# peabody124/PosePipeline

Measured on AMD Instinct MI355X. Metric: frames/sec (whole node), detect->2D->3D cascade on 1080p; MPJPE vs reference, higher is better.
Workload: dtype f32; eligible float32 convolutions are evaluated as 2-term float16 splits (22 significand bits under per-channel / per-sample power-of-two scales, 3 products per term) on the 16-bit matrix cores with float32 accumulation (float32-accurate at any input magnitude, not bit-identical: tests/test_gpu_spl

## Files before the change

posepipeline_amd/csrc/api_core.hip:

```cpp
#include <dlfcn.h>

#include <algorithm>
#include <memory>

#include "pp_internal.h"
#include "pp_amax.h"

#include <atomic>
extern std::atomic<int> g_decode_generic, g_split_gemm_epi;

static thread_local std::string g_last_error;

void pp_set_error(const char* fmt, ...) {
    char buf[1024];
    va_list ap;
    va_start(ap, fmt);
    vsnprintf(buf, sizeof(buf), fmt, ap);
    va_end(ap);
    g_last_error = buf;
}

namespace {
struct Roctx {
    int (*push)(const char*) = nullptr;
// ... 83 lines not shown
    PP_HIP_CHECK(hipStreamCreateWithFlags(&c->copy_stream, hipStreamNonBlocking));
    PP_HIP_CHECK(hipEventCreateWithFlags(&c->ev_upload, hipEventDisableTiming));
    PP_HIP_CHECK(hipEventCreateWithFlags(&c->ev_consumed, hipEventDisableTiming));
    *out = c.release();
    return PP_OK;
}

void pp_ctx_destroy(pp_ctx* ctx) {
    if (!ctx) return;
    (void)hipSetDevice(ctx->device);
    if (ctx->stream) (void)hipStreamSynchronize(ctx->stream);
    if (ctx->scratch) (void)hipFree(ctx->scratch);
    if (ctx->ev_start) (void)hipEventDestroy(ctx->ev_start);
    if (ctx->ev_stop) (void)hipEventDestroy(ctx->ev_stop);
    if (ctx->copy_stream) {
        (void)hipStreamSynchronize(ctx->copy_stream);
        (void)hipStreamDestroy(ctx->copy_stream);
    }
    if (ctx->ev_upload) (void)hipEventDestroy(ctx->ev_upload);
    if (ctx->ev_consumed) (void)hipEventDestroy(ctx->ev_consumed);
    if (ctx->own_stream && ctx->stream) (void)hipStreamDestroy(ctx->stream);
    delete ctx;
}

int pp_ctx_set_stream(pp_ctx* ctx, void* hip_stream) {
    PP_REQUIRE(ctx, "pp_ctx_set_stream: ctx is NULL");
    PP_HIP_CHECK(hipStreamSynchronize(ctx->stream));
    if (ctx->own_stream && ctx->stream) PP_HIP_CHECK(hipStreamDestroy(ctx->stream));
    ctx->stream = static_cast<hipStream_t>(hip_stream);
    ctx->own_stream = false;
    return PP_OK;
}

int pp_ctx_synchronize(pp_ctx* ctx) {
    PP_REQUIRE(ctx, "pp_ctx_synchronize: ctx is NULL");
    PP_HIP_CHECK(hipStreamSynchronize(ctx->stream));
    return PP_OK;
}

int pp_timer_start(pp_ctx* ctx) {
    PP_REQUIRE(ctx, "pp_timer_start: ctx is NULL");
    PP_HIP_CHECK(hipEventRecord(ctx->ev_start, ctx->stream));
    return PP_OK;
}

int pp_timer_stop(pp_ctx* ctx, float* elapsed_ms) {
    PP_REQUIRE(ctx && elapsed_ms, "pp_timer_stop: NULL argument");
    PP_HIP_CHECK(hipEventRecord(ctx->ev_stop, ctx->stream));
    PP_HIP_CHECK(hipEventSynchronize(ctx->ev_stop));
    PP_HIP_CHECK(hipEventElapsedTime(elapsed_ms, ctx->ev_start, ctx->ev_stop));
    return PP_OK;
}

int pp_malloc(pp_ctx* ctx, size_t bytes, void** dptr) {
    PP_REQUIRE(ctx && dptr, "pp_malloc: NULL argument");
    PP_HIP_CHECK(hipSetDevice(ctx->device));
    PP_HIP_CHECK(hipMalloc(dptr, bytes ? bytes : 1));
    return PP_OK;
}

int pp_free(pp_ctx* ctx, void* dptr) {
    PP_REQUIRE(ctx, "pp_free: ctx is NULL");
    if (!dptr) return PP_OK;
    PP_HIP_CHECK(hipStreamSynchronize(ctx->stream));
    PP_HIP_CHECK(hipFree(dptr));
    return PP_OK;
}

int pp_memcpy_h2d(pp_ctx* ctx, void* dst, const void* src, size_t bytes) {
    PP_REQUIRE(ctx && (bytes == 0 || (dst && src)), "pp_memcpy_h2d: NULL argument");
    PP_HIP_CHECK(hipMemcpyAsync(dst, src, bytes, hipMemcpyHostToDevice, ctx->stream));
    PP_HIP_CHECK(hipStreamSynchronize(ctx->stream));
    return PP_OK;
}

int pp_host_alloc(pp_ctx* ctx, size_t bytes, void** out) {
    PP_REQUIRE(ctx && out, "pp_host_alloc: NULL argument");
    *out = nullptr;
    PP_HIP_CHECK(hipSetDevice(ctx->device));
    PP_HIP_CHECK(hipHostMalloc(out, bytes ? bytes : 1, hipHostMallocDefault));
    return PP_OK;
}

int pp_host_free(pp_ctx* ctx, void* p) {
    PP_REQUIRE(ctx != nullptr, "pp_host_free: ctx is NULL");
    if (p) PP_HIP_CHECK(hipHostFree(p));
    return PP_OK;
}

int pp_upload_begin(pp_ctx* ctx, void* dst, const void* src, size_t bytes) {
    PP_REQUIRE(ctx && (bytes == 0 || (dst && src)), "pp_upload_begin: NULL argument");
    PP_HIP_CHECK(hipStreamWaitEvent(ctx->copy_stream, ctx->ev_consumed, 0));
    PP_HIP_CHECK(hipMemcpyAsync(dst, src, bytes, hipMemcpyHostToDevice, ctx->copy_stream));
    PP_HIP_CHECK(hipEventRecord(ctx->ev_upload, ctx->copy_stream));
    return PP_OK;
}

int pp_upload_begin_nv12(pp_ctx* ctx, void* dst_bgr, void* tmp_nv12, const void* src_host, int frames, int height, int width) {
    PP_REQUIRE(ctx && (frames == 0 || (dst_bgr && tmp_nv12 && src_host)), "pp_upload_begin_nv12: NULL argument");
    PP_REQUIRE(frames >= 0 && height > 0 && width > 0, "pp_upload_begin_nv12: bad shape");
    PP_HIP_CHECK(hipStreamWaitEvent(ctx->copy_stream, ctx->ev_consumed, 0));
    const size_t bytes = (size_t)frames * height * width * 3 / 2;
    if (bytes) PP_HIP_CHECK(hipMemcpyAsync(tmp_nv12, src_host, bytes, hipMemcpyHostToDevice, ctx->copy_stream));
    const int r = pp_launch_nv12_to_bgr((const unsigned char*)tmp_nv12, (unsigned char*)dst_bgr, frames, height, width, ctx->copy_stream);
    if (r != PP_OK) return r;
    PP_HIP_CHECK(hipEventRecord(ctx->ev_upload, ctx->copy_stream));
    return PP_OK;
}

int pp_nv12_to_bgr(pp_ctx* ctx, const uint8_t* nv12, int frames, int height, int width, uint8_t* bgr) {
    PP_REQUIRE(ctx && (frames == 0 || (nv12 && bgr)), "pp_nv12_to_bgr: NULL argument");
    return pp_launch_nv12_to_bgr(nv12, bgr, frames, height, width, ctx->stream);
}

int pp_upload_wait(pp_ctx* ctx, int host_sync) {
    PP_REQUIRE(ctx != nullptr, "pp_upload_wait: ctx is NULL");
    PP_HIP_CHECK(hipStreamWaitEvent(ctx->stream, ctx->ev_upload, 0));
    if (host_sync) PP_HIP_CHECK(hipEventSynchronize(ctx->ev_upload));
    return PP_OK;
}

int pp_upload_release(pp_ctx* ctx) {
    PP_REQUIRE(ctx != nullptr, "pp_upload_release: ctx is NULL");
    PP_HIP_CHECK(hipEventRecord(ctx->ev_consumed, ctx->stream));
    return PP_OK;
}

int pp_memcpy_d2h(pp_ctx* ctx, void* dst, const void* src, size_t bytes) {
    PP_REQUIRE(ctx && (bytes == 0 || (dst && src)), "pp_memcpy_d2h: NULL argument");
    PP_HIP_CHECK(hipMemcpyAsync(dst, src, bytes, hipMemcpyDeviceToHost, ctx->stream));
    PP_HIP_CHECK(hipStreamSynchronize(ctx->stream));
    return PP_OK;
}

int pp_memcpy_d2d(pp_ctx* ctx, void* dst, const void* src, size_t bytes) {
    PP_REQUIRE(ctx && (bytes == 0 || (dst && src)), "pp_memcpy_d2d: NULL argument");
    PP_HIP_CHECK(hipMemcpyAsync(dst, src, bytes, hipMemcpyDeviceToDevice, ctx->stream));
    return PP_OK;
}

}


struct pp_net {
    pp_ctx* ctx = nullptr;
    std::vector<pp_op> ops;
    std::vector<pp_buf> bufs;
    std::vector<size_t> buf_off;
    std::vector<size_t> buf_elems;
    float* weights = nullptr;
    size_t n_weights = 0;
    unsigned char* wsplit = nullptr;
    std::vector<SplitPlan> split_plan;
    int numerics = PP_NET_NUMERICS_EXACT;
    int split_f16 = 0;
    unsigned* amax = nullptr;
    std::vector<int> op_x_slot, op_y_slot, op_post_slot, slot_owner;
    std::vector<int> slot_first, slot_last;
    struct ExtAmax { int buf, slot, first_reader, last_reader; bool provided; };
    std::vector<ExtAmax> ext;
    float* arena = nullptr;
    size_t arena_floats = 0;
    int max_batch = 0;
    hipGraphExec_t graph_exec = nullptr;
    int graph_batch = 0;
    bool use_lanes = true;
    std::vector<hipStream_t> lanes;
    std::vector<int> op_lane;
    std::vector<std::vector<int>> op_waits;
    std::vector<char> op_needs_event;
    std::vector<hipEvent_t> op_done;
    hipEvent_t fork_ev = nullptr;
    std::vector<hipEvent_t> join_ev;
    std::vector<pp_vit_encoder*> vits;
    std::vector<pp_deconv_bf16*> deconvs;

    float* buf_ptr(int b) const { return arena + buf_off[b]; }
    unsigned* amax_slot(int slot) const { return slot >= 0 ? amax + (size_t)slot * max_batch : nullptr; }
};

static ConvArgs net_conv_args(pp_net* net, const pp_op& op, int batch);
static int net_make_lanes(pp_net* net, int n_lanes);

static void net_plan_amax(pp_net* net) {
    const int n = (int)net->ops.size(), nb = (int)net->bufs.size();
    net->op_x_slot.assign(n, -1);
    net->op_y_slot.assign(n, -1);
    net->op_post_slot.assign(n, -1);
    net->slot_owner.clear();
    net->ext.clear();
    if (net->numerics != PP_NET_NUMERICS_SPLIT || !net->split_f16) return;
    auto is_h = [&](int i) { return net->ops[i].type == PP_OP_CONV && net->split_plan[i].kernel != SPLIT_NONE; };
    auto tracks = [&](int i) {
        const pp_op& op = net->ops[i];
        if (op.type == PP_OP_UPSAMPLE_ADD) return true;
        return op.type == PP_OP_CONV && pp_conv_tracks_amax(net_conv_args(net, op, 1), is_h(i));
    };
    {
        std::vector<char> written(nb, 0);
        for (int i = 0; i < n; ++i) {
            const pp_op& op = net->ops[i];
            if (is_h(i) && !written[op.in]) {
                pp_net::ExtAmax* e = nullptr;
                for (auto& x : net->ext)
                    if (x.buf == op.in) e = &x;
                if (!e) {
                    net->ext.push_back({op.in, (int)net->slot_owner.size(), i, i, false});
                    net->slot_owner.push_back(-1);
                    e = &net->ext.back();
                }
                e->last_reader = i;
                net->op_x_slot[i] = e->slot;
            }
            written[op.out] = 1;
        }
    }
    struct Tensor { int slot; std::vector<int> producers; bool wanted; };
    std::vector<Tensor> tensors;
    std::vector<int> cur(nb, -1);
    std::vector<char> read_since(nb, 1);
    std::vector<std::pair<int, int>> readers;
    for (int i = 0; i < n; ++i) {
        const pp_op& op = net->ops[i];
        if (is_h(i) && cur[op.in] >= 0) {
            tensors[cur[op.in]].wanted = true;
            readers.push_back({i, cur[op.in]});
        }
        for (int b : {op.in, op.res1, op.res2, op.in2, op.in3})
            if (b >= 0) read_since[b] = 1;
        if (cur[op.out] < 0 || read_since[op.out]) {
            cur[op.out] = (int)tensors.size();
            tensors.push_back({(int)net->slot_owner.size(), {}, false});
            net->slot_owner.push_back(i);
        }
        tensors[cur[op.out]].producers.push_back(i);
        read_since[op.out] = 0;
    }
    net->slot_first.assign(net->slot_owner.size(), -1);
    net->slot_last.assign(net->slot_owner.size(), -1);
    for (const Tensor& t : tensors) {
        if (!t.wanted) continue;
        net->slot_first[t.slot] = t.producers.front();
        net->slot_last[t.slot] = t.producers.back();
        bool fused = true;
        for (int p : t.producers) fused = fused && tracks(p);
        {
            int covered = 0;
            const int out_b = net->ops[t.producers.front()].out;
            for (int p : t.producers) covered += net->ops[p].type == PP_OP_CONV ? net->ops[p].cout : net->bufs[out_b].c;
            if (covered < net->bufs[out_b].c) fused = false;
        }
        if (fused)
            for (int p : t.producers) net->op_y_slot[p] = t.slot;
        else
            net->op_post_slot[t.producers.back()] = t.slot;
    }
    for (const auto& r : readers) net->op_x_slot[r.first] = tensors[r.second].slot;
}

static int net_reset_amax(pp_net* net, int first, int last, int batch, hipStream_t s) {
    if (!net->amax) return PP_OK;
    int s0 = -1, s1 = -1;
    for (int k = 0; k < (int)net->slot_first.size(); ++k) {
        const int a = net->slot_first[k], b = net->slot_last[k];
        if (a < 0 || b < first || a >= last) continue;
        PP_REQUIRE(a >= first && b < last, "pp_net_run: op range [%d, %d) splits the producers (ops %d .. %d) of a tensor whose per-sample maxima are tracked",
                   first, last, a, b);
    }
    for (int k = 0; k < (int)net->slot_owner.size(); ++k)
        if (net->slot_owner[k] >= first && net->slot_owner[k] < last) {
            if (s0 < 0) s0 = k;
            s1 = k + 1;
        }
    if (s0 >= 0) PP_HIP_CHECK(hipMemsetAsync(net->amax_slot(s0), 0, (size_t)(s1 - s0) * net->max_batch * sizeof(unsigned), s));
    for (auto& e : net->ext) {
        if (e.last_reader < first || e.first_reader >= last) continue;
        if (e.provided) {
            e.provided = false;
            continue;
        }
        PP_HIP_CHECK(hipMemsetAsync(net->amax_slot(e.slot), 0, (size_t)batch * sizeof(unsigned), s));
        int rc = pp_launch_amax(net->buf_ptr(e.buf), batch, net->buf_elems[e.buf], net->amax_slot(e.slot), s);
        if (rc != PP_OK) return rc;
    }
    return PP_OK;
}

static void net_plan_lanes(pp_net* net, int n_lanes) {
    const int n = (int)net->ops.size(), nb = (int)net->bufs.size();
    net->op_lane.assign(n, 0);
    net->op_waits.assign(n, {});
    net->op_needs_event.assign(n, 0);
    std::vector<int> last_writer(nb, -1);
    std::vector<std::vector<int>> readers(nb);
    std::vector<int> lane_tail(n_lanes, -1);
    for (int i = 0; i < n; ++i) {
        const pp_op& op = net->ops[i];
        std::vector<int> deps;
        auto add = [&](int d) {
            if (d >= 0 && std::find(deps.begin(), deps.end(), d) == deps.end()) deps.push_back(d);
        };
        for (int b : {op.in, op.res1, op.res2, op.in2, op.in3})
            if (b >= 0) add(last_writer[b]);
        add(last_writer[op.out]);
        for (int r : readers[op.out]) add(r);
        int lane = -1, best = -1;
        for (int l = 0; l < n_lanes; ++l)
            if (lane_tail[l] >= 0 && lane_tail[l] > best && std::find(deps.begin(), deps.end(), lane_tail[l]) != deps.end()) {
                best = lane_tail[l];
                lane = l;
            }
        if (lane < 0) {
            lane = 0;
            for (int l = 1; l < n_lanes; ++l)
                if (lane_tail[l] < lane_tail[lane]) lane = l;
        }
        net->op_lane[i] = lane;
        for (int d : deps)
            if (net->op_lane[d] != lane) {
                net->op_waits[i].push_back(d);
                net->op_needs_event[d] = 1;
            }
        lane_tail[lane] = i;
        for (int b : {op.in, op.res1, op.res2, op.in2, op.in3})
            if (b >= 0 && b != op.out) readers[b].push_back(i);
        last_writer[op.out] = i;
        readers[op.out].clear();
    }
}

static int net_check_op(const pp_net& net, const pp_op& op, int idx) {
    const int nb = (int)net.bufs.size();
    PP_REQUIRE(op.in >= 0 && op.in < nb && op.out >= 0 && op.out < nb, "op %d: buffer id out of range", idx);
    PP_REQUIRE(op.res1 < nb && op.res2 < nb, "op %d: residual buffer id out of range", idx);
    PP_REQUIRE(op.in2 < nb && op.in3 < nb && (op.type == PP_OP_UPSAMPLE_ADD || (op.in2 < 0 && op.in3 < 0)),
               "op %d: in2 / in3 are inputs of PP_OP_UPSAMPLE_ADD only (-1 elsewhere)", idx);
    const pp_buf& bi = net.bufs[op.in];
    const pp_buf& bo = net.bufs[op.out];
    const int eh = op.pad_end & 1, ew = (op.pad_end >> 1) & 1;
    PP_REQUIRE(op.out_c_off >= 0 && op.in_c_off >= 0 && (op.out_c_off & 3) == 0 && (op.in_c_off & 3) == 0,
               "op %d: channel offsets must be non-negative multiples of 4", idx);
    if (op.type != PP_OP_CONV) {
        for (int b : {op.in, op.out, op.res1, op.res2, op.in2, op.in3})
            PP_REQUIRE(b < 0 || net.bufs[b].pad == 0, "op %d: only convolutions may touch a buffer with a zero halo (buffer %d)", idx, b);
    } else {
        PP_REQUIRE(bo.pad == 0 || (!op.out_nchw && op.out_c_off == 0 && bo.c == op.cout && (op.cout & 3) == 0),
                   "op %d: a halo output buffer must be a plain NHWC tensor of the op's own channels", idx);
    }
    if (op.type == PP_OP_CONV) {
        PP_REQUIRE(bi.c == op.cin && op.in_c_off == 0, "op %d: in buffer has %d channels, op.cin=%d", idx, bi.c, op.cin);
        PP_REQUIRE(op.out_c_off + op.cout <= bo.c && (op.out_c_off == 0 ? true : !op.out_nchw),
                   "op %d: channels [%d, %d) do not fit the out buffer (%d channels)", idx, op.out_c_off,
                   op.out_c_off + op.cout, bo.c);
        PP_REQUIRE(bo.c == op.cout || ((bo.c & 3) == 0 && !op.out_nchw), "op %d: a sliced out buffer needs c %% 4 == 0", idx);
        PP_REQUIRE(op.relu >= PP_RELU_NONE && op.relu <= PP_ACT_SWISH, "op %d: unknown activation %d", idx, op.relu);
        const int ho = pp_conv_out_dim(bi.h + eh, op.kh, op.stride, op.pad_h, op.dil_h) - ((op.pad_end >> 2) & 1);
        const int wo = pp_conv_out_dim(bi.w + ew, op.kw, op.stride, op.pad_w, op.dil_w) - ((op.pad_end >> 3) & 1);
        PP_REQUIRE((ho << op.up_log2) == bo.h && (wo << op.up_log2) == bo.w,
                   "op %d: conv output %dx%d (<<%d) does not match out buffer %dx%d", idx, ho, wo, op.up_log2,
                   bo.h, bo.w);
        const size_t kpad = ((size_t)op.kh * op.kw * op.cin + 31) / 32 * 32;
        const size_t cpad = ((size_t)op.cout + 15) / 16 * 16;
        PP_REQUIRE(op.w_off >= 0 && (size_t)op.w_off + kpad * cpad <= net.n_weights, "op %d: weights out of blob", idx);
        PP_REQUIRE(op.b_off >= 0 && (size_t)op.b_off + cpad <= net.n_weights, "op %d: bias out of blob", idx);
        PP_REQUIRE((op.w_off % 4) == 0 && (op.b_off % 4) == 0, "op %d: blob offsets must be 16-byte aligned", idx);
        if (op.res1 >= 0) PP_REQUIRE(net.bufs[op.res1].c == op.cout, "op %d: res1 channel mismatch", idx);
        if (op.res2 >= 0)
            PP_REQUIRE(net.bufs[op.res2].c == op.cout && net.bufs[op.res2].h == bo.h && net.bufs[op.res2].w == bo.w,
                       "op %d: res2 shape mismatch", idx);
    } else if (op.type == PP_OP_MAXPOOL) {
        PP_REQUIRE(op.cin == op.cout && (op.cin & 3) == 0 && op.in_c_off + op.cin <= bi.c && op.out_c_off + op.cout <= bo.c &&
                       (bi.c & 3) == 0 && (bo.c & 3) == 0,
                   "op %d: maxpool channel slices do not fit", idx);
        PP_REQUIRE(pp_conv_out_dim(bi.h + eh, op.kh, op.stride, op.pad_h, 1) == bo.h &&
                       pp_conv_out_dim(bi.w + ew, op.kw, op.stride, op.pad_w, 1) == bo.w,
                   "op %d: maxpool output dims mismatch", idx);
    } else if (op.type == PP_OP_AVGPOOL) {
        PP_REQUIRE(op.cin == op.cout && (op.cin & 3) == 0 && bi.c == op.cin && bo.c == op.cin && op.in != op.out && op.kh > 0 &&
                       op.kw > 0 && op.stride > 0 && bi.h >= op.kh && bi.w >= op.kw && (bi.h - op.kh) / op.stride + 1 == bo.h &&
                       (bi.w - op.kw) / op.stride + 1 == bo.w,
                   "op %d: avgpool needs in [h][w][c] and out [(h - kh) / s + 1][(w - kw) / s + 1][c], c %% 4 == 0", idx);
    } else if (op.type == PP_OP_COPY) {
        PP_REQUIRE(bi.c == bo.c && bi.h == bo.h && bi.w == bo.w, "op %d: copy shape mismatch", idx);
    } else if (op.type == PP_OP_DEPTH_TO_SPACE) {
        PP_REQUIRE(op.cout > 0 && (op.cout & 3) == 0 && bi.c == 4 * op.cout && bo.c == op.cout && bo.h == 2 * bi.h && bo.w == 2 * bi.w,
                   "op %d: depth_to_space needs in [h][w][4*cout] and out [2h][2w][cout]", idx);
    } else if (op.type == PP_OP_DECONV_BF16) {
        PP_REQUIRE(bi.c == op.cin && bo.c == op.cout && bo.h == 2 * bi.h && bo.w == 2 * bi.w && op.in != op.out,
                   "op %d: deconv_bf16 needs in [h][w][cin] and out [2h][2w][cout]", idx);
        PP_REQUIRE(op.cin % 64 == 0 && (op.cout & 7) == 0, "op %d: deconv_bf16 needs cin %% 64 == 0 and cout %% 8 == 0", idx);
        PP_REQUIRE(op.relu == PP_RELU_NONE || op.relu == PP_RELU_LAST, "op %d: deconv_bf16 supports PP_RELU_NONE / PP_RELU_LAST", idx);
        PP_REQUIRE(op.w_off >= 0 && (op.w_off % 4) == 0 && (size_t)op.w_off + (size_t)16 * op.cout * op.cin <= net.n_weights &&
                       op.b_off >= 0 && (op.b_off % 4) == 0 && (size_t)op.b_off + op.cout <= net.n_weights,
                   "op %d: deconv_bf16 parameters out of blob", idx);
    } else if (op.type == PP_OP_UPSAMPLE_ADD) {
        PP_REQUIRE(op.cin == op.cout && (op.cout & 3) == 0 && bi.c == op.cout && bo.c == op.cout && op.up_log2 >= 0 &&
                       (bi.h << op.up_log2) == bo.h && (bi.w << op.up_log2) == bo.w && op.in != op.out,
                   "op %d: upsample_add needs in [h][w][c] and out [h << up][w << up][c]", idx);
        PP_REQUIRE(op.relu == PP_RELU_NONE || op.relu == PP_RELU_LAST, "op %d: upsample_add supports PP_RELU_NONE / PP_RELU_LAST", idx);
        for (int r : {op.res1, op.res2})
            if (r >= 0)
                PP_REQUIRE(net.bufs[r].c == bo.c && net.bufs[r].h == bo.h && net.bufs[r].w == bo.w, "op %d: residual shape mismatch", idx);
        PP_REQUIRE(op.in3 < 0 || op.in2 >= 0, "op %d: in3 without in2", idx);
        for (int k = 0; k < 2; ++k) {
            const int b = k ? op.in3 : op.in2, u = k ? op.up3_log2 : op.up2_log2;
            if (b >= 0)
                PP_REQUIRE(u >= 0 && u <= 5 && net.bufs[b].c == bo.c && (net.bufs[b].h << u) == bo.h && (net.bufs[b].w << u) == bo.w &&
                               b != op.out, "op %d: in%d must be [h >> up][w >> up][c] of the out buffer", idx, k + 2);
        }
    } else if (op.type == PP_OP_VIT_ENCODER) {
        PP_REQUIRE(op.cin == op.cout && bi.c == op.cin && bo.c == op.cin && bi.h == bo.h && bi.w == bo.w && op.in != op.out,
                   "op %d: vit encoder needs distinct in / out buffers of [h][w][dim]", idx);
        PP_REQUIRE(op.kh > 0 && op.kw > 0 && op.stride > 0, "op %d: vit encoder needs depth (kh), heads (kw), mlp ratio (stride)", idx);
        PP_REQUIRE(op.w_off >= 0 && (op.w_off % 4) == 0 &&
                       (size_t)op.w_off + pp_vit_param_floats(bi.h * bi.w, op.cin, op.kh, op.cin * op.stride) <= net.n_weights,
                   "op %d: vit encoder parameters out of blob", idx);
    } else {
        pp_set_error("op %d: unsupported op type %d", idx, op.type);
        return PP_ERR_UNSUPPORTED;
    }
    return PP_OK;
}

static ConvArgs net_conv_args(pp_net* net, const pp_op& op, int batch) {
    const pp_buf& bi = net->bufs[op.in];
    const pp_buf& bo = net->bufs[op.out];
    ConvArgs a{};
    a.x = net->buf_ptr(op.in);
    a.y = net->buf_ptr(op.out);
    a.w = net->weights + op.w_off;
    a.bias = net->weights + op.b_off;
    a.res1 = op.res1 >= 0 ? net->buf_ptr(op.res1) : nullptr;
    a.res2 = op.res2 >= 0 ? net->buf_ptr(op.res2) : nullptr;
    a.N = batch; a.Hin = bi.h; a.Win = bi.w; a.Cin = op.cin;
    a.Hout = bo.h >> op.up_log2; a.Wout = bo.w >> op.up_log2;
    a.Cout = op.cout; a.CoutPad = (op.cout + 15) / 16 * 16;
    a.KH = op.kh; a.KW = op.kw; a.stride = op.stride; a.pad_h = op.pad_h; a.pad_w = op.pad_w;
    a.dil_h = op.dil_h; a.dil_w = op.dil_w;
    a.K = op.kh * op.kw * op.cin; a.Kpad = (a.K + 31) / 32 * 32;
    a.HWout = a.Hout * a.Wout; a.M = batch * a.HWout;
    a.relu = op.relu; a.up_log2 = op.up_log2; a.out_nchw = op.out_nchw;
    a.res1_shift = op.res1_shift; a.res1_off_w = op.res1_off_w;
    a.res1_H = op.res1 >= 0 ? net->bufs[op.res1].h : 0;
    a.res1_W = op.res1 >= 0 ? net->bufs[op.res1].w : 0;
    a.y_stride = bo.c; a.y_coff = op.out_c_off;
    a.x_pad = bi.pad; a.y_pad = bo.pad;
    a.r1_pad = op.res1 >= 0 ? net->bufs[op.res1].pad : 0;
    a.r2_pad = op.res2 >= 0 ? net->bufs[op.res2].pad : 0;
    const size_t idx = &op - net->ops.data();
    a.wsplit = (net->wsplit && idx < net->split_plan.size() && net->split_plan[idx].off >= 0) ? net->wsplit + net->split_plan[idx].off : nullptr;
    a.numerics = net->numerics;
    a.split_f16 = net->split_f16;
    if (idx < net->op_x_slot.size()) {
        a.x_amax = net->amax_slot(net->op_x_slot[idx]);
        a.y_amax = net->amax_slot(net->op_y_slot[idx]);
    }
    return a;
}

static int net_launch_op_body(pp_net* net, const pp_op& op, int batch, hipStream_t s);

static int net_launch_op(pp_net* net, const pp_op& op, int batch, hipStream_t s) {
    const size_t idx = &op - net->ops.data();
    int rc = net_launch_op_body(net, op, batch, s);
    if (rc == PP_OK && net->amax && net->op_post_slot[idx] >= 0)
        rc = pp_launch_amax(net->buf_ptr(op.out), batch, net->buf_elems[op.out], net->amax_slot(net->op_post_slot[idx]), s);
    return rc;
}

static int net_launch_op_body(pp_net* net, const pp_op& op, int batch, hipStream_t s) {
    const pp_buf& bi = net->bufs[op.in];
    const pp_buf& bo = net->bufs[op.out];
    if (op.type == PP_OP_CONV) {
        const ConvArgs a = net_conv_args(net, op, batch);
        return pp_launch_conv(a, &net->split_plan[&op - net->ops.data()], s);
    } else if (op.type == PP_OP_MAXPOOL) {
        PoolArgs p{};
        p.x = net->buf_ptr(op.in); p.y = net->buf_ptr(op.out);
        p.N = batch; p.Hin = bi.h; p.Win = bi.w; p.C = op.cin; p.Hout = bo.h; p.Wout = bo.w;
        p.x_stride = bi.c; p.x_coff = op.in_c_off; p.y_stride = bo.c; p.y_coff = op.out_c_off;
        p.KH = op.kh; p.KW = op.kw; p.stride = op.stride; p.pad_h = op.pad_h; p.pad_w = op.pad_w;
        return pp_launch_maxpool(p, s);
    } else if (op.type == PP_OP_AVGPOOL) {
        return pp_launch_avgpool(net->buf_ptr(op.in), net->buf_ptr(op.out), batch, bi.h, bi.w, op.cin, op.kh, op.kw, op.stride, s);
    } else if (op.type == PP_OP_COPY) {
        PP_HIP_CHECK(hipMemcpyAsync(net->buf_ptr(op.out), net->buf_ptr(op.in),
                                    (size_t)batch * net->buf_elems[op.in] * sizeof(float),
                                    hipMemcpyDeviceToDevice, s));
        return PP_OK;
    } else if (op.type == PP_OP_DEPTH_TO_SPACE) {
        return pp_launch_depth_to_space(net->buf_ptr(op.in), net->buf_ptr(op.out), batch, bi.h, bi.w, op.cout, s);
    } else if (op.type == PP_OP_DECONV_BF16) {
        return pp_deconv_bf16_run(net->deconvs[&op - net->ops.data()], net->buf_ptr(op.in), net->buf_ptr(op.out), batch,
                                  op.relu == PP_RELU_LAST, s);
    } else if (op.type == PP_OP_UPSAMPLE_ADD) {
        return pp_launch_upsample_add(net->buf_ptr(op.in), op.res1 >= 0 ? net->buf_ptr(op.res1) : nullptr,
                                      op.res2 >= 0 ? net->buf_ptr(op.res2) : nullptr, net->buf_ptr(op.out), batch, bo.h, bo.w,
                                      bo.c, op.up_log2, op.relu == PP_RELU_LAST, s, op.in2 >= 0 ? net->buf_ptr(op.in2) : nullptr,
                                      op.up2_log2, op.in3 >= 0 ? net->buf_ptr(op.in3) : nullptr, op.up3_log2,
                                      net->amax && net->op_y_slot[&op - net->ops.data()] >= 0 ? net->amax_slot(net->op_y_slot[&op - net->ops.data()]) : nullptr);
    } else if (op.type == PP_OP_VIT_ENCODER) {
        pp_vit_encoder* enc = net->vits[&op - net->ops.data()];
        return pp_vit_encoder_run(enc, net->buf_ptr(op.in), net->buf_ptr(op.out), batch, s);
    }
    return PP_ERR_UNSUPPORTED;
}

int pp_net_dims(pp_net* net, int buf, int* h, int* w, int* c) {
    if (!net || buf < 0 || buf >= (int)net->bufs.size()) return PP_ERR_ARG;
    *h = net->bufs[buf].h; *w = net->bufs[buf].w; *c = net->bufs[buf].c;
    return PP_OK;
}
int pp_net_max_batch(pp_net* net) { return net ? net->max_batch : 0; }
pp_ctx* pp_net_ctx(pp_net* net) { return net ? net->ctx : nullptr; }

void pp_net_void_input_amax(pp_net* net, int buf) {
    if (!net) return;
    for (auto& e : net->ext)
        if (e.buf == buf) e.provided = false;
}

unsigned* pp_net_input_amax_slot(pp_net* net, int buf) {
    if (!net || !net->amax) return nullptr;
    for (auto& e : net->ext)
        if (e.buf == buf) return net->amax_slot(e.slot);
    return nullptr;
}

extern "C" {

int pp_net_create(pp_ctx* ctx, const pp_op* ops, int n_ops, const pp_buf* bufs, int n_bufs,
                  const float* weights, size_t n_weights, int max_batch, pp_net** out) {
    return pp_net_create_mem(ctx, ops, n_ops, bufs, n_bufs, weights, n_weights, PP_MEM_HOST, max_batch, out);
}

int pp_net_create_mem(pp_ctx* ctx, const pp_op* ops, int n_ops, const pp_buf* bufs, int n_bufs,
                      const float* weights, size_t n_weights, int weights_mem, int max_batch, pp_net** out) {
    return pp_net_create_ex(ctx, ops, n_ops, bufs, n_bufs, weights, n_weights, weights_mem, max_batch, PP_NET_NUMERICS_DEFAULT, out);
}

int pp_net_numerics(pp_net* net) { return net ? net->numerics : PP_ERR_ARG; }
int pp_net_split_kind(pp_net* net) {
    if (!net) return PP_ERR_ARG;
    return net->numerics != PP_NET_NUMERICS_SPLIT ? PP_NET_NUMERICS_EXACT : net->split_f16 ? PP_NET_NUMERICS_SPLIT_F16 : PP_NET_NUMERICS_SPLIT_BF16;
}

int pp_net_create_ex(pp_ctx* ctx, const pp_op* ops, int n_ops, const pp_buf* bufs, int n_bufs,
                     const float* weights, size_t n_weights, int weights_mem, int max_batch, int numerics, pp_net** out) {
    PP_REQUIRE(ctx && ops && bufs && weights && out, "pp_net_create: NULL argument");
    PP_REQUIRE(numerics >= PP_NET_NUMERICS_DEFAULT && numerics <= PP_NET_NUMERICS_SPLIT_F16, "pp_net_create_ex: bad numerics %d", numerics);
    PP_REQUIRE(weights_mem == PP_MEM_HOST || weights_mem == PP_MEM_DEVICE, "pp_net_create: bad weights_mem %d", weights_mem);
    PP_REQUIRE(n_ops > 0 && n_bufs > 0 && max_batch > 0, "pp_net_create: empty program");
    *out = nullptr;
    std::unique_ptr<pp_net> net(new pp_net());
    net->ctx = ctx;
    net->ops.assign(ops, ops + n_ops);
    net->bufs.assign(bufs, bufs + n_bufs);
    net->max_batch = max_batch;
    net->n_weights = n_weights;
    net->numerics = numerics != PP_NET_NUMERICS_DEFAULT ? numerics : (pp_conv_split_enabled() ? PP_NET_NUMERICS_SPLIT : PP_NET_NUMERICS_EXACT);
    if (net->numerics >= PP_NET_NUMERICS_SPLIT) {
        net->split_f16 = net->numerics == PP_NET_NUMERICS_SPLIT ? pp_conv_split_f16_default() : net->numerics == PP_NET_NUMERICS_SPLIT_F16;
        net->numerics = PP_NET_NUMERICS_SPLIT;
    }
    size_t off = 0;
    for (int b = 0; b < n_bufs; ++b) {
        PP_REQUIRE(bufs[b].h > 0 && bufs[b].w > 0 && bufs[b].c > 0 && bufs[b].pad >= 0 && bufs[b].pad <= 8, "buffer %d has an empty dim / bad halo", b);
        const size_t e = (size_t)(bufs[b].h + bufs[b].pad) * (bufs[b].w + bufs[b].pad) * bufs[b].c;
        net->buf_elems.push_back(e);
        net->buf_off.push_back(off);
        off += (e * max_batch + 63) / 64 * 64;
    }
    net->arena_floats = off;
    for (int i = 0; i < n_ops; ++i) {
        int rc = net_check_op(*net, net->ops[i], i);
        if (rc != PP_OK) return rc;
    }
    PP_HIP_CHECK(hipSetDevice(ctx->device));
    PP_HIP_CHECK(hipMalloc((void**)&net->weights, n_weights * sizeof(float)));
    PP_HIP_CHECK(hipMemcpyAsync(net->weights, weights, n_weights * sizeof(float),
                                weights_mem == PP_MEM_HOST ? hipMemcpyHostToDevice : hipMemcpyDeviceToDevice, ctx->stream));
    PP_HIP_CHECK(hipMalloc((void**)&net->arena, net->arena_floats * sizeof(float)));
    PP_HIP_CHECK(hipMemsetAsync(net->arena, 0, net->arena_floats * sizeof(float), ctx->stream));
    net->vits.assign(n_ops, nullptr);
    net->deconvs.assign(n_ops, nullptr);
    for (int i = 0; i < n_ops; ++i) {
        const pp_op& op = net->ops[i];
        if (op.type == PP_OP_DECONV_BF16) {
            const pp_buf& bi = net->bufs[op.in];
            int rc = pp_deconv_bf16_create(net->weights + op.w_off, net->weights + op.b_off, bi.h, bi.w, op.cin, op.cout,
                                           max_batch, ctx->stream, &net->deconvs[i]);
            if (rc != PP_OK) {
                pp_net_destroy(net.release());
                return rc;
            }
        }
        if (op.type != PP_OP_VIT_ENCODER) continue;
        const pp_buf& bi = net->bufs[op.in];
        int rc = pp_vit_encoder_create(net->weights + op.w_off, bi.h * bi.w, op.cin, op.kh, op.kw, op.cin * op.stride,
                                       max_batch, ctx->stream, &net->vits[i]);
        if (rc != PP_OK) {
            pp_net_destroy(net.release());
            return rc;
        }
    }
    net->split_plan.assign(n_ops, SplitPlan());
    if (net->numerics == PP_NET_NUMERICS_SPLIT) {
        size_t bytes = 0;
        for (int i = 0; i < n_ops; ++i) {
            if (net->ops[i].type != PP_OP_CONV) continue;
            SplitPlan p = pp_conv_split_plan(net_conv_args(net.get(), net->ops[i], 1));
            if (p.kernel == SPLIT_NONE) continue;
            p.off = (long long)bytes;
            bytes += (p.bytes + 255) / 256 * 256;
            net->split_plan[i] = p;
        }
        net_plan_amax(net.get());
        if (!net->slot_owner.empty()) {
            const size_t ab = net->slot_owner.size() * (size_t)max_batch * sizeof(unsigned);
            PP_HIP_CHECK(hipMalloc((void**)&net->amax, ab));
            PP_HIP_CHECK(hipMemsetAsync(net->amax, 0, ab, ctx->stream));
        }
        if (bytes) {
            PP_HIP_CHECK(hipMalloc((void**)&net->wsplit, bytes));
            for (int i = 0; i < n_ops; ++i) {
                const SplitPlan& p = net->split_plan[i];
                if (p.kernel == SPLIT_NONE) continue;
                int rc = pp_conv_split_weights(p, net_conv_args(net.get(), net->ops[i], 1), net->wsplit + p.off, ctx->stream);
                if (rc != PP_OK) return rc;
            }
        }
    }
    PP_HIP_CHECK(hipStreamSynchronize(ctx->stream));
    for (int i = 0; i < n_ops; ++i)
        if (net->ops[i].type == PP_OP_CONV) {
            int rc = pp_conv_prepare(net_conv_args(net.get(), net->ops[i], 1));
            if (rc != PP_OK) return rc;
        }
    const char* env_lanes = getenv("POSEPIPE_NET_LANES");
    const int n_lanes = env_lanes ? atoi(env_lanes) : 4;
    int rc_l = net_make_lanes(net.get(), n_lanes);
    if (rc_l != PP_OK) return rc_l;
    *out = net.release();
    return PP_OK;
}

static int net_make_lanes(pp_net* net, int n_lanes) {
    for (auto l : net->lanes) (void)hipStreamDestroy(l);
    net->lanes.clear();
    for (auto e : net->op_done)
        if (e) (void)hipEventDestroy(e);
    net->op_done.clear();
    for (auto e : net->join_ev)
        if (e) (void)hipEventDestroy(e);
    net->join_ev.clear();
    if (net->fork_ev) (void)hipEventDestroy(net->fork_ev);
    net->fork_ev = nullptr;
    const int n_ops = (int)net->ops.size();
    if (n_lanes > 1 && n_ops >= 8) {
        net_plan_lanes(net, n_lanes);
        net->lanes.resize(n_lanes);
        for (auto& l : net->lanes) PP_HIP_CHECK(hipStreamCreateWithFlags(&l, hipStreamNonBlocking));
        net->op_done.assign(n_ops, nullptr);
        for (int i = 0; i < n_ops; ++i)
            if (net->op_needs_event[i]) PP_HIP_CHECK(hipEventCreateWithFlags(&net->op_done[i], hipEventDisableTiming));
        PP_HIP_CHECK(hipEventCreateWithFlags(&net->fork_ev, hipEventDisableTiming));
        net->join_ev.resize(n_lanes);
        for (auto& e : net->join_ev) PP_HIP_CHECK(hipEventCreateWithFlags(&e, hipEventDisableTiming));
    }
    return PP_OK;
}

int pp_net_input_amax(pp_net* net, int buf, void** dptr) {
    PP_REQUIRE(net && dptr && buf >= 0 && buf < (int)net->bufs.size(), "pp_net_input_amax: bad argument");
    *dptr = nullptr;
    for (auto& e : net->ext)
        if (e.buf == buf && net->amax) {
            e.provided = true;
            *dptr = net->amax_slot(e.slot);
        }
    return PP_OK;
}

int pp_net_conv_kinds(pp_net* net, int* kinds) {
    PP_REQUIRE(net && kinds, "pp_net_conv_kinds: NULL argument");
    for (size_t i = 0; i < net->ops.size(); ++i) {
        if (net->ops[i].type != PP_OP_CONV) {
            kinds[i] = 0;
            continue;
        }
        kinds[i] = net->split_plan[i].kernel != SPLIT_NONE ? 2 : 1;
    }
    return PP_OK;
}

void pp_net_destroy(pp_net* net) {
    if (!net) return;
    if (net->ctx && net->ctx->stream) (void)hipStreamSynchronize(net->ctx->stream);
    for (auto l : net->lanes) {
        (void)hipStreamSynchronize(l);
        (void)hipStreamDestroy(l);
    }
    for (auto e : net->op_done)
        if (e) (void)hipEventDestroy(e);
    for (auto e : net->join_ev)
        if (e) (void)hipEventDestroy(e);
    if (net->fork_ev) (void)hipEventDestroy(net->fork_ev);
    if (net->graph_exec) (void)hipGraphExecDestroy(net->graph_exec);
    for (auto* v : net->vits) pp_vit_encoder_destroy(v);
    for (auto* d : net->deconvs) pp_deconv_bf16_destroy(d);
    if (net->weights) (void)hipFree(net->weights);
    if (net->wsplit) (void)hipFree(net->wsplit);
    if (net->amax) (void)hipFree(net->amax);
    if (net->arena) (void)hipFree(net->arena);
    delete net;
}

int pp_net_buffer(pp_net* net, int buf, void** dptr, size_t* bytes_per_sample) {
    PP_REQUIRE(net && buf >= 0 && buf < (int)net->bufs.size(), "pp_net_buffer: bad buffer id");
    PP_REQUIRE(net->bufs[buf].pad == 0, "pp_net_buffer: buffer %d has a zero halo (conv-internal layout); expose dense buffers only", buf);
    if (dptr) *dptr = net->buf_ptr(buf);
    if (bytes_per_sample) *bytes_per_sample = net->buf_elems[buf] * sizeof(float);
    return PP_OK;
}

int pp_net_run(pp_net* net, int batch, int first_op, int last_op) {
    PP_REQUIRE(net, "pp_net_run: net is NULL");
    PP_REQUIRE(batch > 0 && batch <= net->max_batch, "pp_net_run: batch %d not in (0,%d]", batch, net->max_batch);
    if (last_op < 0) last_op = (int)net->ops.size();
    PP_REQUIRE(first_op >= 0 && last_op <= (int)net->ops.size() && first_op <= last_op, "pp_net_run: bad op range");
    if (net->graph_exec && batch == net->graph_batch && first_op == 0 && last_op == (int)net->ops.size()) {
        PP_HIP_CHECK(hipGraphLaunch(net->graph_exec, net->ctx->stream));
        return PP_OK;
    }
    hipStream_t main = net->ctx->stream;
    PpRange range("pp_net_run");
    {
        int rc = net_reset_amax(net, first_op, last_op, batch, main);
        if (rc != PP_OK) return rc;
    }
    if (net->lanes.empty() || !net->use_lanes || last_op - first_op < 8) {
        for (int i = first_op; i < last_op; ++i) {
            int rc = net_launch_op(net, net->ops[i], batch, main);
            if (rc != PP_OK) return rc;
        }
        return PP_OK;
    }
    PP_HIP_CHECK(hipEventRecord(net->fork_ev, main));
    for (hipStream_t l : net->lanes) PP_HIP_CHECK(hipStreamWaitEvent(l, net->fork_ev, 0));
    for (int i = first_op; i < last_op; ++i) {
        hipStream_t s = net->lanes[net->op_lane[i]];
        for (int d : net->op_waits[i])
            if (d >= first_op) PP_HIP_CHECK(hipStreamWaitEvent(s, net->op_done[d], 0));
        int rc = net_launch_op(net, net->ops[i], batch, s);
        if (rc != PP_OK) return rc;
        if (net->op_needs_event[i]) PP_HIP_CHECK(hipEventRecord(net->op_done[i], s));
    }
    for (size_t l = 0; l < net->lanes.size(); ++l) {
        PP_HIP_CHECK(hipEventRecord(net->join_ev[l], net->lanes[l]));
        PP_HIP_CHECK(hipStreamWaitEvent(main, net->join_ev[l], 0));
    }
    return PP_OK;
}

int pp_net_vit_timing(pp_net* net, int enable, float* ms3, int* n_gemm) {
    PP_REQUIRE(net, "pp_net_vit_timing: net is NULL");
    for (auto* v : net->vits) {
        if (!v) continue;
        if (ms3) {
            PP_HIP_CHECK(hipStreamSynchronize(net->ctx->stream));
            int rc = pp_vit_encoder_get_timing(v, ms3, n_gemm);
            if (rc != PP_OK) return rc;
        }
        pp_vit_encoder_set_timing(v, enable);
        return PP_OK;
    }
    pp_set_error("pp_net_vit_timing: the program has no PP_OP_VIT_ENCODER");
    return PP_ERR_STATE;
}

int pp_net_set_lane_count(pp_net* net, int n_lanes) {
    PP_REQUIRE(net && n_lanes >= 1 && n_lanes <= 16, "pp_net_set_lane_count: net is NULL or n_lanes not in [1, 16]");
    PP_HIP_CHECK(hipStreamSynchronize(net->ctx->stream));
    for (auto l : net->lanes) PP_HIP_CHECK(hipStreamSynchronize(l));
    if (net->graph_exec) {
        PP_HIP_CHECK(hipGraphExecDestroy(net->graph_exec));
        net->graph_exec = nullptr;
    }
    return net_make_lanes(net, n_lanes);
}

int pp_net_set_lanes(pp_net* net, int enable) {
    PP_REQUIRE(net, "pp_net_set_lanes: net is NULL");
    PP_HIP_CHECK(hipStreamSynchronize(net->ctx->stream));
    net->use_lanes = enable != 0;
    return PP_OK;
}

int pp_net_capture(pp_net* net, int batch) {
    PP_REQUIRE(net, "pp_net_capture: net is NULL");
    PP_REQUIRE(batch > 0 && batch <= net->max_batch, "pp_net_capture: bad batch");
    if (net->graph_exec) {
        PP_HIP_CHECK(hipGraphExecDestroy(net->graph_exec));
        net->graph_exec = nullptr;
    }
    hipStream_t s = net->ctx->stream;
    PP_HIP_CHECK(hipStreamSynchronize(s));
    hipGraph_t graph = nullptr;
    PP_HIP_CHECK(hipStreamBeginCapture(s, hipStreamCaptureModeThreadLocal));
    int rc = net_reset_amax(net, 0, (int)net->ops.size(), batch, s);
    for (size_t i = 0; i < net->ops.size() && rc == PP_OK; ++i) rc = net_launch_op(net, net->ops[i], batch, s);
    hipError_t e = hipStreamEndCapture(s, &graph);
    if (rc != PP_OK) {
        if (graph) (void)hipGraphDestroy(graph);
        return rc;
    }
    PP_HIP_CHECK(e);
    PP_HIP_CHECK(hipGraphInstantiate(&net->graph_exec, graph, nullptr, nullptr, 0));
    PP_HIP_CHECK(hipGraphDestroy(graph));
    net->graph_batch = batch;
    return PP_OK;
}

int pp_net_forward(pp_net* net, int batch, int in_buf, const float* in, int out_buf, float* out, int mem) {
    PP_REQUIRE(net && in && out, "pp_net_forward: NULL argument");
    PP_REQUIRE(in_buf >= 0 && in_buf < (int)net->bufs.size() && out_buf >= 0 && out_buf < (int)net->bufs.size(),
               "pp_net_forward: bad buffer id");
    PP_REQUIRE(batch > 0 && batch <= net->max_batch, "pp_net_forward: batch %d not in (0,%d]", batch, net->max_batch);
    PP_REQUIRE(net->bufs[in_buf].pad == 0 && net->bufs[out_buf].pad == 0, "pp_net_forward: input / output buffers must be dense (pad 0)");
    hipStream_t s = net->ctx->stream;
    const hipMemcpyKind kin = mem == PP_MEM_HOST ? hipMemcpyHostToDevice : hipMemcpyDeviceToDevice;
    const hipMemcpyKind kout = mem == PP_MEM_HOST ? hipMemcpyDeviceToHost : hipMemcpyDeviceToDevice;
    PP_HIP_CHECK(hipMemcpyAsync(net->buf_ptr(in_buf), in, (size_t)batch * net->buf_elems[in_buf] * sizeof(float), kin, s));
    pp_net_void_input_amax(net, in_buf);
    int rc = pp_net_run(net, batch, 0, (int)net->ops.size());
    if (rc != PP_OK) return rc;
    PP_HIP_CHECK(hipMemcpyAsync(out, net->buf_ptr(out_buf), (size_t)batch * net->buf_elems[out_buf] * sizeof(float), kout, s));
    PP_HIP_CHECK(hipStreamSynchronize(s));
    return PP_OK;
}

int pp_net_profile(pp_net* net, int batch, float* ms_per_op) {
    PP_REQUIRE(net, "pp_net_profile: net is NULL");
    PP_REQUIRE(batch > 0 && batch <= net->max_batch, "pp_net_profile: bad batch");
    hipStream_t s = net->ctx->stream;
    const size_t n = net->ops.size();
    std::vector<hipEvent_t> ev(n + 1);
    for (auto& e : ev) PP_HIP_CHECK(hipEventCreate(&e));
    int rc = net_reset_amax(net, 0, (int)n, batch, s);
    PP_HIP_CHECK(hipEventRecord(ev[0], s));
    for (size_t i = 0; i < n && rc == PP_OK; ++i) {
        rc = net_launch_op(net, net->ops[i], batch, s);
        if (rc == PP_OK && hipEventRecord(ev[i + 1], s) != hipSuccess) rc = PP_ERR_HIP;
    }
    if (rc == PP_OK && hipStreamSynchronize(s) != hipSuccess) rc = PP_ERR_HIP;
    if (rc == PP_OK && ms_per_op) {
        for (size_t i = 0; i < n; ++i) {
            float ms = 0.f;
            (void)hipEventElapsedTime(&ms, ev[i], ev[i + 1]);
            ms_per_op[i] = ms;
        }
    }
    for (auto& e : ev) (void)hipEventDestroy(e);
    return rc;
}

int pp_conv2d(pp_ctx* ctx, const pp_op* op, int n, int hin, int win, const float* x, const float* w,
              const float* bias, const float* res1, const float* res2, float* y, int res1_h, int res1_w,
              int mem) {
    PP_REQUIRE(ctx && op && x && w && bias && y, "pp_conv2d: NULL argument");
    PP_REQUIRE(op->type == PP_OP_CONV, "pp_conv2d: op is not a conv");
    PP_REQUIRE(n > 0 && hin > 0 && win > 0, "pp_conv2d: empty input");
    ConvArgs a{};
    a.N = n; a.Hin = hin; a.Win = win; a.Cin = op->cin;
    a.Hout = pp_conv_out_dim(hin + (op->pad_end & 1), op->kh, op->stride, op->pad_h, op->dil_h) - ((op->pad_end >> 2) & 1);
    a.Wout = pp_conv_out_dim(win + ((op->pad_end >> 1) & 1), op->kw, op->stride, op->pad_w, op->dil_w) - ((op->pad_end >> 3) & 1);
    PP_REQUIRE(a.Hout > 0 && a.Wout > 0, "pp_conv2d: empty output");
    a.Cout = op->cout; a.CoutPad = (op->cout + 15) / 16 * 16;
    a.KH = op->kh; a.KW = op->kw; a.stride = op->stride; a.pad_h = op->pad_h; a.pad_w = op->pad_w;
    a.dil_h = op->dil_h; a.dil_w = op->dil_w;
    a.K = op->kh * op->kw * op->cin; a.Kpad = (a.K + 31) / 32 * 32;
    a.HWout = a.Hout * a.Wout; a.M = n * a.HWout;
    a.relu = op->relu; a.up_log2 = op->up_log2; a.out_nchw = op->out_nchw;
    a.res1_shift = op->res1_shift; a.res1_off_w = op->res1_off_w;
    const int Ho2 = a.Hout << op->up_log2, Wo2 = a.Wout << op->up_log2;
    a.res1_H = res1 ? (res1_h > 0 ? res1_h : Ho2) : 0;
    a.res1_W = res1 ? (res1_w > 0 ? res1_w : Wo2) : 0;
    a.y_stride = op->cout; a.y_coff = 0;
    PP_REQUIRE(op->out_c_off == 0 && op->in_c_off == 0, "pp_conv2d: channel slices need a layer program");
    const size_t x_e = (size_t)n * hin * win * op->cin;
    const size_t w_e = (size_t)a.Kpad * a.CoutPad;
    const size_t b_e = a.CoutPad;
    const size_t y_e = (size_t)n * Ho2 * Wo2 * op->cout;
    const size_t r1_e = res1 ? (size_t)n * a.res1_H * a.res1_W * op->cout : 0;
    const size_t r2_e = res2 ? y_e : 0;
    if (mem == PP_MEM_DEVICE) {
        a.x = x; a.w = w; a.bias = bias; a.res1 = res1; a.res2 = res2; a.y = y;
        return pp_launch_conv(a, nullptr, ctx->stream);
    }
    size_t total = 0;
    for (size_t e : {x_e, w_e, b_e, y_e, r1_e, r2_e}) total += ScratchCursor::align(e * sizeof(float));
    int rc = ctx->ensure_scratch(total);
    if (rc != PP_OK) return rc;
    ScratchCursor cur(ctx);
    float* dx = cur.take<float>(x_e);
    float* dw = cur.take<float>(w_e);
    float* db = cur.take<float>(b_e);
    float* dy = cur.take<float>(y_e);
    float* dr1 = cur.take<float>(r1_e);
    float* dr2 = cur.take<float>(r2_e);
    hipStream_t s = ctx->stream;
    PP_HIP_CHECK(hipMemcpyAsync(dx, x, x_e * 4, hipMemcpyHostToDevice, s));
    PP_HIP_CHECK(hipMemcpyAsync(dw, w, w_e * 4, hipMemcpyHostToDevice, s));
    PP_HIP_CHECK(hipMemcpyAsync(db, bias, b_e * 4, hipMemcpyHostToDevice, s));
    if (res1) PP_HIP_CHECK(hipMemcpyAsync(dr1, res1, r1_e * 4, hipMemcpyHostToDevice, s));
    if (res2) PP_HIP_CHECK(hipMemcpyAsync(dr2, res2, r2_e * 4, hipMemcpyHostToDevice, s));
    a.x = dx; a.w = dw; a.bias = db; a.res1 = res1 ? dr1 : nullptr; a.res2 = res2 ? dr2 : nullptr; a.y = dy;
    rc = pp_launch_conv(a, nullptr, s);
    if (rc != PP_OK) return rc;
    PP_HIP_CHECK(hipMemcpyAsync(y, dy, y_e * 4, hipMemcpyDeviceToHost, s));
    PP_HIP_CHECK(hipStreamSynchronize(s));
    return PP_OK;
}

}
```

posepipeline_amd/csrc/conv_igemm.hip:

```cpp
#include <dlfcn.h>

#include <algorithm>
#include <atomic>
#include <cstdlib>
#include <map>
#include <mutex>
#include <vector>

#include "pp_internal.h"
#include "pp_amax.h"

typedef float f32x4 __attribute__((ext_vector_type(4)));

namespace {

constexpr int BK = 32;

__device__ __forceinline__ int swz(int j) {
    return ((j >> 1) & 1) | ((j & 1) << 1) | ((((j >> 1) ^ (j >> 2)) & 1) << 2);
}

__device__ __forceinline__ unsigned udiv(unsigned n, unsigned m, unsigned s1, unsigned s2) {
    const unsigned t = __umulhi(m, n);
    return (t + ((n - t) >> s1)) >> s2;
// ... 466 lines not shown
};
struct TapKey {
    int dev, cin, kh, kw, dil_h, dil_w, win, k;
    bool operator<(const TapKey& o) const { return memcmp(this, &o, sizeof(TapKey)) < 0; }
};
std::mutex g_tap_mutex;
std::map<TapKey, uint2*> g_tap_tables;

const uint2* tap_table_for(const ConvArgs& a, bool create) {
    TapKey key;
    memset(&key, 0, sizeof(key));
    if (hipGetDevice(&key.dev) != hipSuccess) return nullptr;
    const int pitch = a.Win + a.x_pad;
    key.cin = a.Cin; key.kh = a.KH; key.kw = a.KW; key.dil_h = a.dil_h; key.dil_w = a.dil_w; key.win = pitch; key.k = a.K;
    std::lock_guard<std::mutex> lock(g_tap_mutex);
    auto it = g_tap_tables.find(key);
    if (it != g_tap_tables.end()) return it->second;
    if (!create) return nullptr;
    const int nsteps = (a.K + 15) / 16;
    std::vector<uint2> h((size_t)(nsteps + 1) * 4);
    for (int s = 0; s <= nsteps; ++s)
        for (int q = 0; q < 4; ++q) {
            const int k = 16 * s + 4 * q;
            uint2 e = make_uint2(0x7fff7fffu, 0x80000000u);
            if (k < a.K) {
                const int tap = k / a.Cin, c = k - tap * a.Cin;
                const int kh = tap / a.KW, kw = tap - kh * a.KW;
                e.x = ((unsigned)(kh * a.dil_h) << 16) | (unsigned)(kw * a.dil_w);
                e.y = (unsigned)(((kh * a.dil_h * pitch + kw * a.dil_w) * a.Cin + c) * 4);
            }
            h[(size_t)s * 4 + q] = e;
        }
    uint2* d = nullptr;
    if (hipMalloc((void**)&d, h.size() * sizeof(uint2)) != hipSuccess) return nullptr;
    if (hipMemcpy(d, h.data(), h.size() * sizeof(uint2), hipMemcpyHostToDevice) != hipSuccess) {
        (void)hipFree(d);
        return nullptr;
    }
    g_tap_tables[key] = d;
    return d;
}

int g_force_ct = 0, g_force_pt = 0;
int g_variant = -1;

}

extern "C" int pp_conv_variant(int variant) {
    if (variant < -1 || variant > 4) {
        pp_set_error("pp_conv_variant: -1 (default), 0 (two-barrier kernel), 1 (three-stage pipelined kernel), 3 (pipelined + tap table: "
                     "the bit-exact default) or 4 (bf16-split kernel where eligible)");
        return PP_ERR_ARG;
    }
    g_variant = variant;
    return PP_OK;
}

extern "C" int pp_conv_force(int ct, int pt) {
    if (ct < 0 || ct > 4 || (pt != 0 && pt != 1 && pt != 2)) {
        pp_set_error("pp_conv_force: ct in 0..4, pt in {0, 1, 2} (0 = automatic)");
        return PP_ERR_ARG;
    }
    g_force_ct = ct;
    g_force_pt = pt;
    return PP_OK;
}

int pp_conv_out_dim(int in, int k, int stride, int pad, int dil) {
    return (in + 2 * pad - dil * (k - 1) - 1) / stride + 1;
}

static void magic_u32(unsigned d, unsigned* m, unsigned* s1, unsigned* s2) {
    unsigned l = 0;
    while ((1ull << l) < d) ++l;
    *m = (unsigned)((((1ull << l) - d) << 32) / d + 1);
    *s1 = l < 1 ? l : 1;
    *s2 = l > 0 ? l - 1 : 0;
}

std::atomic<int> g_exact{-1};
bool pp_conv_split_enabled() {
    static const int env_exact = env_int("POSEPIPE_CONV_EXACT", 0);
    static const int env_variant = env_int("POSEPIPE_CONV_VARIANT", -1);
    const int v = g_variant >= 0 ? g_variant : env_variant;
    const int ge = g_exact.load(std::memory_order_relaxed);
    const int exact = ge >= 0 ? ge : env_exact;
    return v == 4 || (v < 0 && !exact);
}

std::atomic<int> g_split_f16{-1};
bool pp_conv_split_f16_default() {
    static const int env_f16 = env_int("POSEPIPE_SPLIT_F16", 1);
    const int g = g_split_f16.load(std::memory_order_relaxed);
    return (g >= 0 ? g : env_f16) != 0;
}

extern "C" int pp_conv_split_kind(int f16) {
    if (f16 < -1 || f16 > 1) {
        pp_set_error("pp_conv_split_kind: 1 (two float16 terms, three products), 0 (three bfloat16 terms, six products) or -1 (POSEPIPE_SPLIT_F16)");
        return PP_ERR_ARG;
    }
    g_split_f16.store(f16, std::memory_order_relaxed);
    return PP_OK;
}

extern "C" int pp_conv_exact(int exact) {
    if (exact < -1 || exact > 1) {
        pp_set_error("pp_conv_exact: 1 (bit-exact fp32 MFMA kernels), 0 (bf16-split kernels where eligible) or -1 (POSEPIPE_CONV_EXACT)");
        return PP_ERR_ARG;
    }
    g_exact.store(exact, std::memory_order_relaxed);
    return PP_OK;
}

bool pp_conv_tracks_amax(const ConvArgs& a, bool split) {
    if (a.HWout < 64) return false;
    if (split) return true;
    const int Ho2 = a.Hout << a.up_log2, Wo2 = a.Wout << a.up_log2;
    const bool res1_plain = a.res1_shift == 0 && a.res1_off_w == 0 && a.res1_H == Ho2 && a.res1_W == Wo2;
    return a.up_log2 == 0 && (a.Cout & 3) == 0 && !a.out_nchw && (!a.res1 || res1_plain) && a.relu <= PP_RELU_FIRST &&
           (a.y_stride == 0 || a.y_stride == a.Cout);
}

int pp_conv_prepare(const ConvArgs& a) {
    if (a.Cin % 4 != 0 || a.K <= 0) return PP_OK;
    return tap_table_for(a, true) ? PP_OK : PP_ERR_HIP;
}

int pp_launch_conv(const ConvArgs& a_in, const SplitPlan* plan, hipStream_t stream) {
    ConvArgs a = a_in;
    a.tap_table = nullptr;
    magic_u32((unsigned)a.HWout, &a.div_hw_m, &a.div_hw_s1, &a.div_hw_s2);
    magic_u32((unsigned)a.Wout, &a.div_w_m, &a.div_w_s1, &a.div_w_s2);
    magic_u32((unsigned)a.Cin, &a.div_c_m, &a.div_c_s1, &a.div_c_s2);
    magic_u32((unsigned)a.KW, &a.div_kw_m, &a.div_kw_s1, &a.div_kw_s2);
    static const int xcd_remap = env_int("POSEPIPE_CONV_XCD", 1);
    a.xcd_remap = xcd_remap;
    if (a.Cin % 4 != 0) {
        pp_set_error("conv: Cin=%d must be a multiple of 4 (pad the input channels)", a.Cin);
        return PP_ERR_ARG;
    }
    if (a.Hin + a.pad_h >= 32768 || a.Win + a.pad_w >= 32768) {
        pp_set_error("conv: spatial dims must be < 32768");
        return PP_ERR_ARG;
    }
    if (a.M <= 0) return PP_OK;
    const size_t img_bytes = (size_t)(a.Hin + a.x_pad) * (a.Win + a.x_pad) * a.Cin * sizeof(float);
    static const size_t max_bytes_env = (size_t)env_int("POSEPIPE_CONV_MAX_MB", 0) << 20;
    const size_t max_bytes = max_bytes_env ? max_bytes_env : 0xfffffff0u;
    if (img_bytes > max_bytes) {
        pp_set_error("conv: one input image of %zu bytes exceeds the 4 GiB buffer range", img_bytes);
        return PP_ERR_ARG;
    }
    if ((size_t)a.N * img_bytes > max_bytes) {
        const int per = (int)(max_bytes / img_bytes);
        const size_t y_img = (size_t)((a.Hout << a.up_log2) + a.y_pad) * ((a.Wout << a.up_log2) + a.y_pad) * (a.y_stride ? a.y_stride : a.Cout);
        const size_t r1_img = (size_t)(a.res1_H + a.r1_pad) * (a.res1_W + a.r1_pad) * a.Cout;
        const size_t r2_img = (size_t)((a.Hout << a.up_log2) + a.r2_pad) * ((a.Wout << a.up_log2) + a.r2_pad) * a.Cout;
        for (int n0 = 0; n0 < a.N; n0 += per) {
            ConvArgs p = a_in;
            p.N = std::min(per, a.N - n0);
            p.M = p.N * a.HWout;
            p.x = a.x + (size_t)n0 * (img_bytes / sizeof(float));
            p.y = a.y + (size_t)n0 * y_img;
            if (a.res1) p.res1 = a.res1 + (size_t)n0 * r1_img;
            if (a.res2) p.res2 = a.res2 + (size_t)n0 * r2_img;
            if (a.x_amax) p.x_amax = a.x_amax + n0;
            if (a.y_amax) p.y_amax = a.y_amax + n0;
            const int rc = pp_launch_conv(p, plan, stream);
            if (rc != PP_OK) return rc;
        }
        return PP_OK;
    }
    a.x_bytes = (unsigned)((size_t)a.N * img_bytes);
    if (a.y_stride == 0) a.y_stride = a.Cout;
    if (plan && plan->kernel != SPLIT_NONE) return pp_launch_conv_split(*plan, a, stream);
    if (!plan && a.numerics == 0 && pp_conv_split_enabled()) {
        a.split_f16 = pp_conv_split_f16_default();
        const SplitPlan p = pp_conv_split_plan(a);
        if (p.kernel != SPLIT_NONE) {
            void* tmp = nullptr;
            const size_t wbytes = (p.bytes + 255) / 256 * 256;
            PP_HIP_CHECK(hipMalloc(&tmp, wbytes + (p.f16 ? (size_t)a.N * sizeof(unsigned) : 0)));
            a.wsplit = tmp;
            int rc = pp_conv_split_weights(p, a, tmp, stream);
            if (rc == PP_OK && p.f16) {
                unsigned* am = reinterpret_cast<unsigned*>(static_cast<unsigned char*>(tmp) + wbytes);
                if (hipMemsetAsync(am, 0, (size_t)a.N * sizeof(unsigned), stream) != hipSuccess) rc = PP_ERR_HIP;
                if (rc == PP_OK) rc = pp_launch_amax(a.x, a.N, img_bytes / sizeof(float), am, stream);
                a.x_amax = am;
            }
            if (rc == PP_OK) rc = pp_launch_conv_split(p, a, stream);
            (void)hipStreamSynchronize(stream);
            (void)hipFree(tmp);
            return rc;
        }
    }
    if (a.y_amax && !pp_conv_tracks_amax(a, false)) {
        pp_set_error("conv: this layer's epilogue does not track the output maximum (ConvArgs::y_amax; see pp_conv_tracks_amax)");
        return PP_ERR_STATE;
    }
    static const int force_ct = env_int("POSEPIPE_CONV_CT", 0), force_pt = env_int("POSEPIPE_CONV_PT", 0),
                     min_blocks = env_int("POSEPIPE_CONV_MIN_BLOCKS", 512);
    const int tiles = a.CoutPad / 16;
    int best_ct = 1, best_waste = 1 << 30;
    for (int ct = 4; ct >= 1; --ct) {
        const int waste = ((tiles + ct - 1) / ct) * ct - tiles;
        if (waste < best_waste) {
            best_waste = waste;
            best_ct = ct;
        }
    }
    static const TuneTable tuning;
    static const int env_variant = env_int("POSEPIPE_CONV_VARIANT", -1);
    int tuned_pt = 0, variant = 0;
    if (!tuning.best.empty()) {
        TuneKey k;
        memset(&k, 0, sizeof(k));
        k.cin = a.Cin; k.cout = a.Cout; k.kh = a.KH; k.kw = a.KW; k.stride = a.stride; k.dil_h = a.dil_h; k.dil_w = a.dil_w;
        if (const TuneTable::Choice* c = tuning.find(k, a.M)) {
            best_ct = c->ct;
            tuned_pt = c->pt;
            if (c->variant >= 0) variant = c->variant;
        }
    }
    if (env_variant >= 0) variant = env_variant;
    if (g_variant >= 0) variant = g_variant;
    if (variant == 4) variant = 0;
    if (force_ct) best_ct = force_ct;
    if (g_force_ct) best_ct = g_force_ct;
    const int cblocks = (tiles + best_ct - 1) / best_ct;
    int pt = 2;
    while (pt > 1 && (long)((a.M + 64 * pt - 1) / (64 * pt)) * cblocks < min_blocks) pt >>= 1;
    if (tuned_pt) pt = tuned_pt;
    if (force_pt) pt = force_pt;
    if (g_force_pt) pt = g_force_pt;
    {
        static const int pt_by_ct[5] = {0, env_int("POSEPIPE_CONV_PT_CT1", 0), env_int("POSEPIPE_CONV_PT_CT2", 0),
                                        env_int("POSEPIPE_CONV_PT_CT3", 0), env_int("POSEPIPE_CONV_PT_CT4", 0)};
        if (pt_by_ct[best_ct] && (long)((a.M + 64 * pt_by_ct[best_ct] - 1) / (64 * pt_by_ct[best_ct])) * cblocks >= min_blocks)
            pt = pt_by_ct[best_ct];
    }
    a.no_bounds = 0;
    const bool halo = (a.x_pad | a.y_pad | a.r1_pad | a.r2_pad) != 0;
    if (halo) variant = 3;
    if (variant == 3) {
        a.no_bounds = a.pad_h <= a.x_pad && a.pad_w <= a.x_pad &&
                      (a.Hout - 1) * a.stride - a.pad_h + (a.KH - 1) * a.dil_h <= a.Hin - 1 + a.x_pad &&
                      (a.Wout - 1) * a.stride - a.pad_w + (a.KW - 1) * a.dil_w <= a.Win - 1 + a.x_pad && a.x_bytes < 0x7fffff00u;
        a.tap_table = tap_table_for(a, true);
        if (!a.tap_table) {
            pp_set_error("conv: could not build the tap table");
            return PP_ERR_HIP;
        }
    }
    if (variant >= 1) return pp_launch_conv_p3(a, best_ct, pt, stream, variant == 2);
    switch (best_ct) {
        case 4: return launch_ct<4>(a, pt, stream);
        case 3: return launch_ct<3>(a, pt, stream);
        case 2: return launch_ct<2>(a, pt, stream);
        default: return launch_ct<1>(a, pt, stream);
    }
}

int pp_launch_maxpool(const PoolArgs& a, hipStream_t stream) {
    if (a.C % 4 != 0) {
        pp_set_error("maxpool: C=%d must be a multiple of 4", a.C);
        return PP_ERR_ARG;
    }
    const size_t total = (size_t)a.N * a.Hout * a.Wout * (a.C / 4);
    if (total == 0) return PP_OK;
    const int blocks = (int)std::min<size_t>((total + 255) / 256, 256 * 8);
    hipLaunchKernelGGL(maxpool_kernel, dim3(blocks), dim3(256), 0, stream, a);
    hipError_t e = hipGetLastError();
    if (e != hipSuccess) {
        pp_set_error("maxpool launch failed: %s", hipGetErrorString(e));
        return PP_ERR_HIP;
    }
    return PP_OK;
}
```

posepipeline_amd/csrc/conv_split.hip:

```cpp
#include <algorithm>
#include <atomic>
#include <map>
#include <mutex>
#include <type_traits>
#include <vector>
#include <cstring>
#include <cstdio>

#include "pp_internal.h"
#include "pp_amax.h"

#ifndef PP_SPLIT_ABLATE
#define PP_SPLIT_ABLATE 0
#endif

typedef __attribute__((ext_vector_type(8))) __bf16 bf16x8;
typedef __attribute__((ext_vector_type(8))) _Float16 f16x8;
typedef __attribute__((ext_vector_type(16))) float f32x16;

std::atomic<int> g_split_gemm_epi{-1};

namespace {


struct SplitArgs {
    const float* x;
    const uint4* w;
    const float* bias;
    const float* res1;
    const float* res2;
    float* y;
    int N, H, W, Cin, Cout, ncb;
    int xp_h, xp_w;
    int y_pad, r1_pad, r2_pad, relu;
    int nchunks;
    int tiles_x, tiles_y, TH, TW, bw_log2, gx_log2;
    int PWp;
    int NP, NPp;
    int mode, stride;
    int r1_shift, r1_H, r1_W;
    int ktaps, KW, pad, Hin, Win;
    long long S;
    unsigned x_bytes;
    int xcd_remap;
    int SP;
    int gx, gy;
    int col_major;
    int epi_lds;
    unsigned dv_per[2], dv_row[2];
    unsigned dv_tx[2], dv_ty[2], dv_pw[2];
    unsigned dv_ncol[2], dv_run0[2], dv_run1[2];
    unsigned dv_ktaps[2], dv_kw[2];
    const float* wscale;
    const unsigned* x_amax;
    unsigned* y_amax;
#ifdef PP_SPLIT_TIMELINE
    unsigned long long* dbg;
#endif
};

#ifdef PP_SPLIT_TIMELINE
#define PP_TL_DECL unsigned long long tl_t[10] = {0, 0, 0, 0, 0, 0, 0, 0, 0, 0}
#define PP_TL_MARK(i) do { if (a.dbg) tl_t[i] = __builtin_amdgcn_s_memtime(); } while (0)
#define PP_TL_FLUSH()                                                                                                    \
    do {                                                                                                                 \
        if (a.dbg && threadIdx.x == 0) {                                                                                 \
            unsigned hw, xcc;                                                                                            \
            asm volatile("s_getreg_b32 %0, hwreg(HW_REG_HW_ID)" : "=s"(hw));                                            \
            asm volatile("s_getreg_b32 %0, hwreg(HW_REG_XCC_ID)" : "=s"(xcc));                                          \
            unsigned long long* r = a.dbg + (size_t)blockIdx.x * 16;                                                     \
            r[0] = blockIdx.x; r[1] = ((unsigned long long)xcc << 32) | hw;                                              \
            r[2] = tl_t[0]; r[3] = tl_t[1]; r[4] = tl_t[2]; r[5] = tl_t[3]; r[6] = L; r[7] = col;                       \
            for (int i_ = 4; i_ < 10; ++i_) r[4 + i_] = tl_t[i_];                                                        \
        }                                                                                                                \
    } while (0)
#else
#define PP_TL_DECL
#define PP_TL_MARK(i)
#define PP_TL_FLUSH()
#endif

__device__ __forceinline__ unsigned pp_udiv(unsigned n, const unsigned (&dv)[2]) {
    const unsigned t = __umulhi(n, dv[0]);
    const unsigned q = (t + ((n - t) >> 1)) >> (dv[1] & 31u);
    return dv[1] >= 32u ? n : q;
}

__device__ __forceinline__ bool xcd_tile_column(unsigned L, const SplitArgs& a, unsigned& tile, unsigned& col) {
    const unsigned ntiles = (unsigned)a.gx, ncol = (unsigned)a.gy;
    const unsigned xcd = L & 7u, j = L >> 3;
    const unsigned q = ntiles >> 3, r = ntiles & 7u;
    const unsigned run = xcd < r ? q + 1 : q;
    unsigned tj;
    if (a.col_major) {
        if (run == 0) return false;
        col = xcd < r ? pp_udiv(j, a.dv_run1) : pp_udiv(j, a.dv_run0);
        tj = j - col * run;
        if (col >= ncol) return false;
    } else {
        tj = pp_udiv(j, a.dv_ncol);
        col = j - tj * ncol;
        if (tj >= run) return false;
    }
    tile = (xcd < r ? xcd * (q + 1) : r * (q + 1) + (xcd - r) * q) + tj;
    return true;
}

typedef __attribute__((ext_vector_type(2))) __bf16 bf16x2_t;
typedef __attribute__((ext_vector_type(2))) float f32x2_t;
__device__ __forceinline__ void split4(const float4 v, uint2& p0, uint2& p1, uint2& p2) {
    const f32x2_t a = {v.x, v.y}, b = {v.z, v.w};
    const bf16x2_t a0 = __builtin_convertvector(a, bf16x2_t), b0 = __builtin_convertvector(b, bf16x2_t);
    const f32x2_t ra = a - __builtin_convertvector(a0, f32x2_t), rb = b - __builtin_convertvector(b0, f32x2_t);
    const bf16x2_t a1 = __builtin_convertvector(ra, bf16x2_t), b1 = __builtin_convertvector(rb, bf16x2_t);
    const f32x2_t sa = ra - __builtin_convertvector(a1, f32x2_t), sb = rb - __builtin_convertvector(b1, f32x2_t);
    const bf16x2_t a2 = __builtin_convertvector(sa, bf16x2_t), b2 = __builtin_convertvector(sb, bf16x2_t);
    p0 = make_uint2(__builtin_bit_cast(unsigned, a0), __builtin_bit_cast(unsigned, b0));
    p1 = make_uint2(__builtin_bit_cast(unsigned, a1), __builtin_bit_cast(unsigned, b1));
    p2 = make_uint2(__builtin_bit_cast(unsigned, a2), __builtin_bit_cast(unsigned, b2));
}

typedef __attribute__((ext_vector_type(2))) _Float16 f16x2_t;
__device__ __forceinline__ void split2h(const float x0, const float x1, const float s, unsigned& h0, unsigned& h1) {
    unsigned d, e;
    asm("v_fma_mixlo_f16 %0, %1, %2, 0" : "=v"(d) : "v"(x0), "v"(s));
    asm("v_fma_mixhi_f16 %0, %1, %2, 0" : "+v"(d) : "v"(x1), "v"(s));
    asm("v_fma_mixlo_f16 %0, %1, %2, -%3 op_sel_hi:[0,0,1]" : "=v"(e) : "v"(x0), "v"(s), "v"(d));
    asm("v_fma_mixhi_f16 %0, %1, %2, -%3 op_sel:[0,0,1] op_sel_hi:[0,0,1]" : "+v"(e) : "v"(x1), "v"(s), "v"(d));
    h0 = d;
    h1 = e;
}
__device__ __forceinline__ void split4h(const float4 v, const float s, uint2& p0, uint2& p1) {
    split2h(v.x, v.y, s, p0.x, p1.x);
    split2h(v.z, v.w, s, p0.y, p1.y);
}

__device__ __forceinline__ float split_activate(float x, int act) {
    if (act == PP_ACT_LEAKY) return x >= 0.f ? x : 0.1f * x;
    if (act == PP_ACT_MISH) {
        if (x > 20.f) return x;
        const double n = exp((double)x);
        const double t = n * (n + 2.0);
        return x * (float)(t / (t + 2.0));
    }
    if (act == PP_ACT_ELU) return x > 0.f ? x : (float)expm1((double)x);
    if (act == PP_ACT_SWISH) return x * (float)(1.0 / (1.0 + exp(-(double)x)));
    return x;
}

__device__ __forceinline__ int lane_q(int r) {
    const int g1 = ((r >= 4 && r < 12) || (r >= 16 && r < 20) || r >= 28) ? 1 : 0;
    int idx;
    if (!g1) idx = r < 4 ? r : r < 16 ? r - 8 : r - 12;
    else idx = r < 12 ? r - 4 : r < 20 ? r - 8 : r - 16;
    return g1 * 16 + idx;
}
__device__ __forceinline__ void block_pixel(int r, int bw_log2, int& iy, int& ix) {
    if (bw_log2 == 0) {
        iy = 0;
        ix = r;
        return;
    }
    const int q = lane_q(r);
    if (bw_log2 == 1) {
        iy = q >> 4;
        ix = q & 15;
    } else {
        iy = ((q >> 3) & 1) * 2 + (q >> 4);
        ix = q & 7;
    }
}

enum { MODE_TILE = 0, MODE_STREAM = 1, MODE_GEMM = 2 };

template <int T, int NSLOT, int COB, int PXB = 2, int NW = 4, bool RING4 = false, bool H = false, bool S2 = false>
__global__ __launch_bounds__(64 * NW, NW == 4 ? 2 : 1) void conv_split_kernel(SplitArgs a) {
    static_assert(!S2 || (T == 9 && RING4 && H && PXB == 1), "S2 is the 4-wave fp16 ring form with one pixel block per wave");
    constexpr int NT = 64 * NW;
    constexpr int XP = H ? 2 : 3;
    constexpr int WPL = H ? 2 : 3;
    constexpr bool WLDS = NW == 8 || RING4;
    static_assert(!RING4 || (NW == 4 && T == 9), "RING4 is the 4-wave 3x3 form");
    extern __shared__ __attribute__((aligned(16))) unsigned char smem[];
    const int tid = threadIdx.x;
    const int lane = tid & 63;
    const int wave = tid >> 6;
    unsigned L = blockIdx.x, col = blockIdx.y;
    PP_TL_DECL;
    PP_TL_MARK(0);
    if (a.xcd_remap) {
        if (!xcd_tile_column(blockIdx.x, a, L, col)) return;
    }
    const int cb0 = (int)col * COB;
    const int plane_bytes = 2 * a.NPp * 16;
    const int buf_bytes = XP * plane_bytes;

    int n = 0, x0 = 0, y0 = 0;
    unsigned s0 = 0;
    if (a.mode == MODE_TILE) {
        const unsigned L2 = pp_udiv(L, a.dv_tx);
        const int tx = (int)(L - L2 * (unsigned)a.tiles_x);
        n = (int)pp_udiv(L2, a.dv_ty);
        const int ty = (int)(L2 - (unsigned)n * (unsigned)a.tiles_y);
        x0 = tx * a.TW;
        y0 = ty * a.TH;
    } else {
        s0 = L * (unsigned)(32 * PXB * NW);
    }
// ... 833 lines not shown
    }
    size_t ypix[SB], r1pix[SB], r2pix[SB];
    bool ook[SB];
    int onn[SB];
    float xinv[H ? SB : 1];
#pragma unroll
    for (int sb = 0; sb < SB; ++sb) {
        int aof_, on_, oy_, ox_;
        sub_block(sb, aof_, on_, oy_, ox_, ook[sb]);
        onn[sb] = on_;
        if constexpr (H) xinv[sb] = pp_act_unscale(oam[sb]);
        const int n_ = ook[sb] ? on_ : 0, y_ = ook[sb] ? oy_ : 0, x_ = ook[sb] ? ox_ : 0;
        ypix[sb] = ((size_t)n_ * (a.H + a.y_pad) + y_) * (a.W + a.y_pad) + x_;
        r1pix[sb] = ((size_t)n_ * (a.r1_H + a.r1_pad) + (y_ >> a.r1_shift)) * (a.r1_W + a.r1_pad) + (x_ >> a.r1_shift);
        r2pix[sb] = ((size_t)n_ * (a.H + a.r2_pad) + y_) * (a.W + a.r2_pad) + x_;
    }
    float4 rv[SB][CB];
    if (a.res1) {
#pragma unroll
        for (int sb = 0; sb < SB; ++sb)
#pragma unroll
            for (int cb = 0; cb < CB; ++cb) rv[sb][cb] = *reinterpret_cast<const float4*>(a.res1 + r1pix[sb] * a.Cout + cos[cb]);
    }
#pragma unroll
    for (int sb = 0; sb < SB; ++sb)
#pragma unroll
        for (int cb = 0; cb < CB; ++cb) {
            const f32x4 cc = acc[cb][sb];
            const float4 b = b4[cb];
            float4 v;
            if constexpr (H) v = make_float4(__builtin_fmaf(cc[0], sc4[cb].x * xinv[sb], b.x), __builtin_fmaf(cc[1], sc4[cb].y * xinv[sb], b.y),
                                             __builtin_fmaf(cc[2], sc4[cb].z * xinv[sb], b.z), __builtin_fmaf(cc[3], sc4[cb].w * xinv[sb], b.w));
            else v = make_float4(cc[0] + b.x, cc[1] + b.y, cc[2] + b.z, cc[3] + b.w);
            if (a.relu == PP_RELU_FIRST) { v.x = fmaxf(v.x, 0.f); v.y = fmaxf(v.y, 0.f); v.z = fmaxf(v.z, 0.f); v.w = fmaxf(v.w, 0.f); }
            else if (a.relu >= PP_ACT_LEAKY) { v.x = split_activate(v.x, a.relu); v.y = split_activate(v.y, a.relu); v.z = split_activate(v.z, a.relu); v.w = split_activate(v.w, a.relu); }
            if (a.res1) { v.x += rv[sb][cb].x; v.y += rv[sb][cb].y; v.z += rv[sb][cb].z; v.w += rv[sb][cb].w; }
            rv[sb][cb] = v;
        }
    PP_TL_MARK(6);
    if (a.res2) {
#pragma unroll
        for (int sb = 0; sb < SB; ++sb)
#pragma unroll
            for (int cb = 0; cb < CB; ++cb) {
                const float4 r = *reinterpret_cast<const float4*>(a.res2 + r2pix[sb] * a.Cout + cos[cb]);
                rv[sb][cb].x += r.x; rv[sb][cb].y += r.y; rv[sb][cb].z += r.z; rv[sb][cb].w += r.w;
            }
    }
    float ymax[SB];
#pragma unroll
    for (int sb = 0; sb < SB; ++sb) {
        ymax[sb] = 0.f;
#pragma unroll
        for (int cb = 0; cb < CB; ++cb) {
            float4 v = rv[sb][cb];
            if (a.relu == PP_RELU_LAST) { v.x = fmaxf(v.x, 0.f); v.y = fmaxf(v.y, 0.f); v.z = fmaxf(v.z, 0.f); v.w = fmaxf(v.w, 0.f); }
            if (ook[sb] && cok[cb]) {
                *reinterpret_cast<float4*>(a.y + ypix[sb] * a.Cout + cos[cb]) = v;
                ymax[sb] = fmaxf(ymax[sb], pp_abs4max(v));
            }
        }
    }
    if (a.y_amax) {
        int wg_first = n, wg_last = n;
        if (a.mode != MODE_TILE) {
            const unsigned last = (unsigned)min((long long)s0 + 255, a.S - 1);
            wg_first = (int)pp_udiv(min(s0, last), a.dv_per);
            wg_last = (int)pp_udiv(last, a.dv_per);
        }
        pp_amax_commit_wg<4, SB>(a.y_amax, onn, ymax, wg_first, wg_last, reinterpret_cast<float*>(smem));
    }
    PP_TL_MARK(3);
#ifdef PP_SPLIT_TIMELINE
    asm volatile("s_waitcnt vmcnt(0)" ::: "memory");
    PP_TL_MARK(7);
#endif
    PP_TL_FLUSH();
}

__device__ __forceinline__ float channel_scale(float cmax) {
    if (!(cmax > 0.f) || !(cmax < 3.0e38f)) return 1.f;
    int e;
    (void)frexpf(cmax, &e);
    return ldexpf(1.f, 15 - e);
}
__device__ __forceinline__ void split_weight_h(float v, float c, unsigned short& q0, unsigned short& q1, unsigned short& q2) {
    const float vs = v * c;
    const _Float16 g0 = (_Float16)vs;
    const float r = vs - (float)g0;
    const _Float16 g1 = (_Float16)r;
    q0 = __builtin_bit_cast(unsigned short, g0);
    q1 = __builtin_bit_cast(unsigned short, g1);
    q2 = 0;
}
__global__ __launch_bounds__(64) void weight_channel_max_kernel(const float* w, int kchunks, int CoutPad, int nout, float* cmax, float* inv_scale) {
    const int cout = blockIdx.x, lane = threadIdx.x;
    float m = 0.f;
    if (cout < CoutPad)
        for (int c = lane >> 5; c < kchunks; c += 2) m = fmaxf(m, fabsf(w[((size_t)c * CoutPad + cout) * 32 + (lane & 31)]));
#pragma unroll
    for (int o = 32; o > 0; o >>= 1) m = fmaxf(m, __shfl_xor(m, o));
    if (lane == 0 && cout < nout) {
        cmax[cout] = m;
        inv_scale[cout] = 1.f / channel_scale(m);
    }
}

template <bool H>
__global__ __launch_bounds__(256) void split_weights48_kernel(const float* w, uint4* out, int Cin, int CoutPad, int ncb16, size_t total, const float* cmax) {
    const size_t i = blockIdx.x * (size_t)256 + threadIdx.x;
    if (i >= total) return;
    const int lane = (int)(i & 63);
    size_t r = i >> 6;
    const int cb = (int)(r % ncb16);
    r /= ncb16;
    const int pair = (int)(r % 5);
    const int c = (int)(r / 5);
    const int g = lane >> 4;
    const int t = 2 * pair + (g >> 1);
    const int cout = cb * 16 + (lane & 15);
    unsigned short h[3][8];
#pragma unroll
    for (int j = 0; j < 8; ++j) {
        const int cin = c * 16 + (g & 1) * 8 + j;
        const int k = t * Cin + cin;
        float v = 0.f;
        if (t < 9 && cout < CoutPad) v = w[((size_t)(k >> 5) * CoutPad + cout) * 32 + 8 * (k & 3) + ((k & 31) >> 2)];
        if constexpr (H) {
            split_weight_h(v, channel_scale(cmax[cout]), h[0][j], h[1][j], h[2][j]);
            continue;
        }
        const __bf16 q0 = (__bf16)v;
        const float r1 = v - (float)q0;
        const __bf16 q1 = (__bf16)r1;
        const float r2 = r1 - (float)q1;
        const __bf16 q2 = (__bf16)r2;
        h[0][j] = __builtin_bit_cast(unsigned short, q0);
        h[1][j] = __builtin_bit_cast(unsigned short, q1);
        h[2][j] = __builtin_bit_cast(unsigned short, q2);
    }
    constexpr int WPL = H ? 2 : 3;
    const size_t frag = (i >> 6) * WPL;
#pragma unroll
    for (int pl = 0; pl < WPL; ++pl) {
        uint4 o;
        o.x = h[pl][0] | ((unsigned)h[pl][1] << 16);
        o.y = h[pl][2] | ((unsigned)h[pl][3] << 16);
        o.z = h[pl][4] | ((unsigned)h[pl][5] << 16);
        o.w = h[pl][6] | ((unsigned)h[pl][7] << 16);
        out[(frag + pl) * 64 + lane] = o;
    }
}

template <int WM, int WN, bool H = false>
__global__ __launch_bounds__(64 * WM * WN, 512 / (64 * WM * WN)) void conv_split_gemm_kernel(SplitArgs a) {
    constexpr int XP = H ? 2 : 3;
    constexpr int WPL = H ? 2 : 3;
    constexpr int NT = 64 * WM * WN, NWAVE = WM * WN;
    constexpr int BM = 128 * WM, BN = 64 * WN;
    constexpr int XS = BM * 4 / NT;
    constexpr int WU = BN * 2 * WPL;
    constexpr int NPp = BM + 4;
    constexpr int XPLANE = 2 * NPp * 16;
    constexpr int XBYTES = XP * XPLANE, STAGE = XBYTES + WU * 16;
    extern __shared__ __attribute__((aligned(16))) unsigned char smem[];
    const int tid = threadIdx.x;
    const int lane = tid & 63;
    const int wave = tid >> 6;
    const int wm = wave / WN, wn = wave % WN;
    unsigned bx = blockIdx.x, by = blockIdx.y;
    PP_TL_DECL;
    PP_TL_MARK(0);
    if (a.xcd_remap) {
        if (!xcd_tile_column(blockIdx.x, a, bx, by)) return;
    }
    const unsigned L = bx, col = by;
    (void)L; (void)col;
    const long long m0 = (long long)bx * BM;
    const int cbB = by * (BN / 32);
    const int cb0 = cbB + wn * 2;

    const unsigned mfirst = (unsigned)min(m0 + wm * 128, a.S - 1), mlast = (unsigned)min(m0 + wm * 128 + 127, a.S - 1);
    const int img_first = __builtin_amdgcn_readfirstlane((int)pp_udiv(mfirst, a.dv_per)), img_last = __builtin_amdgcn_readfirstlane((int)pp_udiv(mlast, a.dv_per));
    unsigned oam_first = 0;
    if constexpr (H) oam_first = a.x_amax[img_first];
    const unsigned lds_base0 = (unsigned)(size_t)(__attribute__((address_space(3))) unsigned char*)smem;
    const size_t wstep0 = (size_t)a.ncb * (WPL * 64);
    f32x16 acc[2][4];
    if constexpr (H) {
    constexpr int XR = 3, XSTG = BM * 64, WR = 3, WBYTES = WU * 16;
    constexpr int NXD = BM / 16 / NWAVE;
    constexpr int NWD = WU / 64 / NWAVE;
    static_assert(BM / 16 % NWAVE == 0 && WU / 64 % NWAVE == 0, "every wave issues the same number of DMAs (vmcnt arithmetic)");
    unsigned gx[NXD];
#pragma unroll
    for (int i = 0; i < NXD; ++i) {
        const int pl = (wave + NWAVE * i) * 16 + (lane >> 2);
        const unsigned m = (unsigned)min(m0 + pl, a.S - 1);
        const int img = (int)pp_udiv(m, a.dv_per), rem = (int)(m - (unsigned)img * (unsigned)(a.H * a.W));
        const int ho = (int)pp_udiv((unsigned)rem, a.dv_row), wo = rem - ho * a.W;
        gx[i] = (unsigned)(((img * a.xp_h + ho * a.stride) * a.xp_w + wo * a.stride) * a.Cin) * 4u + (unsigned)(((lane & 3) ^ ((pl >> 1) & 3)) * 16);
    }
    float xsc[4];
#pragma unroll
    for (int pb = 0; pb < 4; ++pb) xsc[pb] = pp_act_scale(oam_first);
    if (img_first != img_last) {
#pragma unroll
        for (int pb = 0; pb < 4; ++pb) {
            const unsigned mp = (unsigned)min(m0 + wm * 128 + pb * 32 + (lane & 31), a.S - 1);
            xsc[pb] = pp_act_scale(a.x_amax[pp_udiv(mp, a.dv_per)]);
        }
    }
    asm volatile("s_waitcnt vmcnt(0)" ::: "memory");
    const unsigned wlane16 = (unsigned)lane * 16u;
    auto issue = [&](int c) {
        const uint4* wsrc = a.w + (size_t)c * wstep0 + (size_t)cbB * (WPL * 64);
#pragma unroll
        for (int i = 0; i < NWD; ++i) {
            const int slab = i * NWAVE + wave;
            const unsigned dst = __builtin_amdgcn_readfirstlane(lds_base0 + (unsigned)(XR * XSTG + (c % WR) * WBYTES + slab * 1024));
            asm volatile("s_mov_b32 m0, %2\n\ts_nop 0\n\tglobal_load_lds_dwordx4 %0, %1" ::"v"(wlane16 + (unsigned)(slab * 1024)), "s"(wsrc), "s"(dst) : "memory", "m0");
        }
        const float* xsrc = a.x + (size_t)c * 16;
#pragma unroll
        for (int i = 0; i < NXD; ++i) {
            const unsigned dst = __builtin_amdgcn_readfirstlane(lds_base0 + (unsigned)((c % XR) * XSTG + (wave + NWAVE * i) * 1024));
            asm volatile("s_mov_b32 m0, %2\n\ts_nop 0\n\tglobal_load_lds_dwordx4 %0, %1" ::"v"(gx[i]), "s"(xsrc), "s"(dst) : "memory", "m0");
        }
    };
    const int fofs = (wm * 128 + (lane & 31)) * 64 + ((((lane >> 5) * 2) ^ ((lane >> 1) & 3)) * 16);
    const int wofs = XR * XSTG + ((wn * 2) * (WPL * 64) + lane) * 16;
    auto frag = [&](const unsigned char* sx_, int pb, uint4 (&h)[2]) {
        const float4 q0 = *reinterpret_cast<const float4*>(sx_ + (fofs + pb * 2048));
        const float4 q1 = *reinterpret_cast<const float4*>(sx_ + ((fofs + pb * 2048) ^ 16));
        const float sc = xsc[pb];
        unsigned a_[4], b_[4];
        split2h(q0.x, q0.y, sc, a_[0], b_[0]);
        split2h(q0.z, q0.w, sc, a_[1], b_[1]);
        split2h(q1.x, q1.y, sc, a_[2], b_[2]);
        split2h(q1.z, q1.w, sc, a_[3], b_[3]);
        h[0] = make_uint4(a_[0], a_[1], a_[2], a_[3]);
        h[1] = make_uint4(b_[0], b_[1], b_[2], b_[3]);
    };
    PP_TL_MARK(4);
    issue(0);
    if (a.nchunks > 1) issue(1);
    PP_TL_MARK(5);
    if (a.nchunks > 1) asm volatile("s_waitcnt vmcnt(%0)" ::"n"(NXD + NWD) : "memory");
    else asm volatile("s_waitcnt vmcnt(0)" ::: "memory");
    __builtin_amdgcn_s_barrier();
    PP_TL_MARK(1);
#pragma unroll
    for (int cb = 0; cb < 2; ++cb)
#pragma unroll
        for (int pb = 0; pb < 4; ++pb)
#pragma unroll
            for (int i = 0; i < 16; ++i) acc[cb][pb][i] = 0.f;
    for (int c = 0; c < a.nchunks; ++c) {
        const unsigned char* sxp = smem + (c % XR) * XSTG;
        const unsigned char* sw = smem + (c % WR) * WBYTES;
        uint4 wf[2][WPL], xh[2][2];
#pragma unroll
        for (int cb = 0; cb < 2; ++cb)
#pragma unroll
            for (int pl = 0; pl < WPL; ++pl) wf[cb][pl] = *reinterpret_cast<const uint4*>(sw + wofs + (cb * WPL + pl) * 1024);
        frag(sxp, 0, xh[0]);
        if (c + 2 < a.nchunks) issue(c + 2);
#pragma unroll
        for (int pb = 0; pb < 4; ++pb) {
            __builtin_amdgcn_sched_barrier(0);
            constexpr int WI[3] = {1, 0, 0}, XI[3] = {0, 1, 0};
#pragma unroll
            for (int p = 0; p < 3; ++p)
#pragma unroll
                for (int cb = 0; cb < 2; ++cb)
                    acc[cb][pb] = __builtin_amdgcn_mfma_f32_32x32x16_f16(__builtin_bit_cast(f16x8, wf[cb][WI[p]]),
                                                                         __builtin_bit_cast(f16x8, xh[pb & 1][XI[p]]), acc[cb][pb], 0, 0, 0);
            if (pb < 3) frag(sxp, pb + 1, xh[(pb + 1) & 1]);
            __builtin_amdgcn_sched_barrier(0);
        }
        if (c + 2 < a.nchunks) asm volatile("s_waitcnt vmcnt(%0) lgkmcnt(0)" ::"n"(NXD + NWD) : "memory");
        else asm volatile("s_waitcnt vmcnt(0) lgkmcnt(0)" ::: "memory");
        __builtin_amdgcn_s_barrier();
    }
    } else {
    unsigned goff[XS];
    int simg[H ? XS : 1];
#pragma unroll
    for (int j = 0; j < XS; ++j) {
        const int u = tid + NT * j;
        const long long m = m0 + (u >> 2);
        unsigned off = 0xffffffffu;
        if constexpr (H) simg[j] = 0;
        if (m < a.S) {
            const int img = (int)pp_udiv((unsigned)m, a.dv_per), rem = (int)((unsigned)m - (unsigned)img * (unsigned)(a.H * a.W));
            if constexpr (H) simg[j] = img;
            const int ho = (int)pp_udiv((unsigned)rem, a.dv_row), wo = rem - ho * a.W;
            off = (unsigned)(((img * a.xp_h + ho * a.stride) * a.xp_w + wo * a.stride) * a.Cin) * 4u + (unsigned)(u & 3) * 16u;
        }
        goff[j] = off;
    }
    const int woff0 = ((((tid & 3) >> 1) * NPp + (tid >> 2)) * 16 + (tid & 1) * 8);
    const __amdgpu_buffer_rsrc_t xrsrc = __builtin_amdgcn_make_buffer_rsrc((void*)a.x, 0, (int)a.x_bytes, 0x00020000);
    const size_t wstep = (size_t)a.ncb * (WPL * 64);
    float4 xr[XS];
    auto load_x = [&](int c) {
#pragma unroll
        for (int j = 0; j < XS; ++j) {
            const unsigned off = goff[j] == 0xffffffffu ? 0xffffffffu : goff[j] + (unsigned)c * 64u;
            xr[j] = __builtin_bit_cast(float4, __builtin_amdgcn_raw_buffer_load_b128(xrsrc, (int)off, 0, 0));
        }
    };
    float sx[H ? XS : 1];
    auto store_x = [&](int buf) {
        unsigned char* base = smem + buf * STAGE;
#pragma unroll
        for (int j = 0; j < XS; ++j) {
            uint2 p0, p1, p2;
            if constexpr (H) split4h(xr[j], sx[j], p0, p1);
            else split4(xr[j], p0, p1, p2);
            unsigned char* d = base + woff0 + (NT / 4) * 16 * j;
            *reinterpret_cast<uint2*>(d) = p0;
            *reinterpret_cast<uint2*>(d + XPLANE) = p1;
            if constexpr (!H) *reinterpret_cast<uint2*>(d + 2 * XPLANE) = p2;
        }
    };
    constexpr int NSLAB = WU / 64;
    const unsigned lds_base = (unsigned)(size_t)(__attribute__((address_space(3))) unsigned char*)smem;
    auto issue_w = [&](int c, int buf) {
        const uint4* src = a.w + (size_t)c * wstep + (size_t)cbB * (WPL * 64) + lane;
#pragma unroll
        for (int i = 0; i < (NSLAB + NWAVE - 1) / NWAVE; ++i) {
            const int slab = i * NWAVE + wave;
            if (NSLAB % NWAVE == 0 || slab < NSLAB)
            {
                const unsigned dst = __builtin_amdgcn_readfirstlane(lds_base + (unsigned)(buf * STAGE + XBYTES + slab * 1024));
                const uint4* g = src + slab * 64;
                asm volatile("s_mov_b32 m0, %1\n\ts_nop 0\n\tglobal_load_lds_dwordx4 %0, off" ::"v"(g), "s"(dst) : "memory", "m0");
            }
        }
    };

    const int xofs = ((lane >> 5) * NPp + wm * 128 + (lane & 31)) * 16;
    const int wofs = XBYTES + ((wn * 2) * (WPL * 64) + lane) * 16;


    PP_TL_MARK(4);
    issue_w(0, 0);
    load_x(0);
    store_x(0);
    PP_TL_MARK(5);
    if (a.nchunks > 1) load_x(1);
    asm volatile("s_waitcnt vmcnt(%0) lgkmcnt(0)" ::"n"(XS) : "memory");
    if (a.nchunks <= 1) asm volatile("s_waitcnt vmcnt(0)" ::: "memory");
    __builtin_amdgcn_s_barrier();
    PP_TL_MARK(1);

#pragma unroll
    for (int cb = 0; cb < 2; ++cb)
#pragma unroll
        for (int pb = 0; pb < 4; ++pb)
#pragma unroll
            for (int i = 0; i < 16; ++i) acc[cb][pb][i] = 0.f;
    for (int c = 0; c < a.nchunks; ++c) {
        const unsigned char* sb = smem + (c & 1) * STAGE;
        uint4 wf[2][WPL], xf[2][XP];
#pragma unroll
        for (int cb = 0; cb < 2; ++cb)
#pragma unroll
            for (int pl = 0; pl < WPL; ++pl) wf[cb][pl] = *reinterpret_cast<const uint4*>(sb + wofs + (cb * WPL + pl) * 1024);
#pragma unroll
        for (int pl = 0; pl < XP; ++pl) xf[0][pl] = *reinterpret_cast<const uint4*>(sb + xofs + pl * XPLANE);
#pragma unroll
        for (int pb = 0; pb < 4; ++pb) {
            if (pb < 3) {
#pragma unroll
                for (int pl = 0; pl < XP; ++pl) xf[(pb + 1) & 1][pl] = *reinterpret_cast<const uint4*>(sb + xofs + pl * XPLANE + (pb + 1) * 512);
            }
            __builtin_amdgcn_sched_barrier(0);
            if (pb == 1 && c + 1 < a.nchunks) {
                store_x((c + 1) & 1);
                issue_w(c + 1, (c + 1) & 1);
                if (c + 2 < a.nchunks) load_x(c + 2);
            }
            if constexpr (H) {
                constexpr int WI[3] = {1, 0, 0}, XI[3] = {0, 1, 0};
#pragma unroll
                for (int p = 0; p < 3; ++p)
#pragma unroll
                    for (int cb = 0; cb < 2; ++cb)
                        acc[cb][pb] = __builtin_amdgcn_mfma_f32_32x32x16_f16(__builtin_bit_cast(f16x8, wf[cb][WI[p]]),
                                                                             __builtin_bit_cast(f16x8, xf[pb & 1][XI[p]]), acc[cb][pb], 0, 0, 0);
            } else {
            constexpr int WI[6] = {2, 1, 0, 1, 0, 0}, XI[6] = {0, 1, 2, 0, 1, 0};
#pragma unroll
            for (int p = 0; p < 6; ++p)
#pragma unroll
                for (int cb = 0; cb < 2; ++cb)
                    acc[cb][pb] = __builtin_amdgcn_mfma_f32_32x32x16_bf16(__builtin_bit_cast(bf16x8, wf[cb][WI[p]]),
                                                                          __builtin_bit_cast(bf16x8, xf[pb & 1][XI[p]]), acc[cb][pb], 0, 0, 0);
            }
            __builtin_amdgcn_sched_barrier(0);
        }
        if (c + 2 < a.nchunks)
            asm volatile("s_waitcnt vmcnt(%0) lgkmcnt(0)" ::"n"(XS) : "memory");
        else
            asm volatile("s_waitcnt vmcnt(0) lgkmcnt(0)" ::: "memory");
        __builtin_amdgcn_s_barrier();
    }

    }

    PP_TL_MARK(2);
    PP_TL_MARK(6);
    if (a.epi_lds) {
        unsigned char* stg = smem + wave * (16384 + 2048);
        uint4* tab = reinterpret_cast<uint4*>(stg + 16384);
#pragma unroll
        for (int i = 0; i < 2; ++i) {
            const int p = lane + 64 * i;
            const long long m = m0 + wm * 128 + p;
            uint4 t = make_uint4(0u, 0u, 0u, 0u);
            if (m < a.S) {
                const int img = (int)pp_udiv((unsigned)m, a.dv_per), rem = (int)((unsigned)m - (unsigned)img * (unsigned)(a.H * a.W));
                const int oy = (int)pp_udiv((unsigned)rem, a.dv_row), ox = rem - oy * a.W;
                t.x = (unsigned)(((size_t)img * (a.H + a.y_pad) + oy) * (a.W + a.y_pad) + ox);
                t.y = (unsigned)(((size_t)img * (a.r1_H + a.r1_pad) + (oy >> a.r1_shift)) * (a.r1_W + a.r1_pad) + (ox >> a.r1_shift));
                t.z = (unsigned)(((size_t)img * (a.H + a.r2_pad) + oy) * (a.W + a.r2_pad) + ox);
                t.w = (unsigned)img + 1u;
            }
            tab[p] = t;
        }
        const int rdrow = lane >> 3, rdpos = lane & 7, rdchunk = rdpos ^ rdrow;
        float xinv[H ? 4 : 1];
        if constexpr (H) {
#pragma unroll
            for (int pb = 0; pb < 4; ++pb) xinv[pb] = pp_act_unscale(oam_first);
            if (img_first != img_last) {
#pragma unroll
                for (int pb = 0; pb < 4; ++pb) {
                    const unsigned mp = (unsigned)min(m0 + wm * 128 + pb * 32 + (lane & 31), a.S - 1);
                    xinv[pb] = pp_act_unscale(a.x_amax[pp_udiv(mp, a.dv_per)]);
                }
            }
        }
        float ymax = 0.f, ymax1 = 0.f;
#pragma unroll
        for (int cb = 0; cb < 2; ++cb) {
#pragma unroll
            for (int pb = 0; pb < 4; ++pb)
#pragma unroll
                for (int g = 0; g < 4; ++g) {
                    const int co = (cb0 + cb) * 32 + 8 * g + 4 * (lane >> 5);
                    const float4 b4 = *reinterpret_cast<const float4*>(a.bias + co);
                    const f32x16 cc = acc[cb][pb];
                    float4 v;
                    if constexpr (H) {
                        const float4 sc = *reinterpret_cast<const float4*>(a.wscale + co);
                        const float xi = xinv[pb];
                        v = make_float4(__builtin_fmaf(cc[4 * g + 0], sc.x * xi, b4.x), __builtin_fmaf(cc[4 * g + 1], sc.y * xi, b4.y),
                                        __builtin_fmaf(cc[4 * g + 2], sc.z * xi, b4.z), __builtin_fmaf(cc[4 * g + 3], sc.w * xi, b4.w));
                    } else {
                        v = make_float4(cc[4 * g + 0] + b4.x, cc[4 * g + 1] + b4.y, cc[4 * g + 2] + b4.z, cc[4 * g + 3] + b4.w);
                    }
                    if (a.relu == PP_RELU_FIRST) { v.x = fmaxf(v.x, 0.f); v.y = fmaxf(v.y, 0.f); v.z = fmaxf(v.z, 0.f); v.w = fmaxf(v.w, 0.f); }
                    else if (a.relu >= PP_ACT_LEAKY) { v.x = split_activate(v.x, a.relu); v.y = split_activate(v.y, a.relu); v.z = split_activate(v.z, a.relu); v.w = split_activate(v.w, a.relu); }
                    *reinterpret_cast<float4*>(stg + (pb * 32 + (lane & 31)) * 128 + (((2 * g + (lane >> 5)) ^ (lane & 7)) << 4)) = v;
                }
            const int co = (cb0 + cb) * 32 + rdchunk * 4;
            const unsigned* tabw = reinterpret_cast<const unsigned*>(tab);
#pragma unroll
            for (int h8 = 0; h8 < 2; ++h8) {
            float4 vv[8];
#pragma unroll
            for (int i8 = 0; i8 < 8; ++i8) vv[i8] = *reinterpret_cast<const float4*>(stg + ((h8 * 8 + i8) * 8 + rdrow) * 128 + rdpos * 16);
            if (a.res1) {
                float4 rv[8];
#pragma unroll
                for (int i8 = 0; i8 < 8; ++i8) rv[i8] = *reinterpret_cast<const float4*>(a.res1 + (size_t)tabw[((h8 * 8 + i8) * 8 + rdrow) * 4 + 1] * a.Cout + co);
#pragma unroll
                for (int i8 = 0; i8 < 8; ++i8) { vv[i8].x += rv[i8].x; vv[i8].y += rv[i8].y; vv[i8].z += rv[i8].z; vv[i8].w += rv[i8].w; }
            }
            if (a.res2) {
                float4 rv[8];
#pragma unroll
                for (int i8 = 0; i8 < 8; ++i8) rv[i8] = *reinterpret_cast<const float4*>(a.res2 + (size_t)tabw[((h8 * 8 + i8) * 8 + rdrow) * 4 + 2] * a.Cout + co);
#pragma unroll
                for (int i8 = 0; i8 < 8; ++i8) { vv[i8].x += rv[i8].x; vv[i8].y += rv[i8].y; vv[i8].z += rv[i8].z; vv[i8].w += rv[i8].w; }
            }
#pragma unroll
            for (int i8 = 0; i8 < 8; ++i8) {
                const int it = h8 * 8 + i8;
                float4 v = vv[i8];
                if (a.relu == PP_RELU_LAST) { v.x = fmaxf(v.x, 0.f); v.y = fmaxf(v.y, 0.f); v.z = fmaxf(v.z, 0.f); v.w = fmaxf(v.w, 0.f); }
                const uint2 t = *reinterpret_cast<const uint2*>(tabw + (it * 8 + rdrow) * 4);
                const unsigned tw = tabw[(it * 8 + rdrow) * 4 + 3];
                if (tw) *reinterpret_cast<float4*>(a.y + (size_t)t.x * a.Cout + co) = v;
                if (a.y_amax) {
                    const float m = tw ? pp_abs4max(v) : 0.f;
                    if (img_last - img_first <= 1) {
                        if ((int)tw - 1 == img_first) ymax = fmaxf(ymax, m);
                        else ymax1 = fmaxf(ymax1, m);
                    } else {
                        float m8 = fmaxf(m, __shfl_xor(m, 1));
                        m8 = fmaxf(m8, __shfl_xor(m8, 2));
                        m8 = fmaxf(m8, __shfl_xor(m8, 4));
                        if (rdpos == 0 && m8 > 0.f) atomicMax(a.y_amax + (tw - 1u), __float_as_uint(m8));
                    }
                }
            }
            }
        }
        if (a.y_amax) {
            const unsigned wlast = (unsigned)min(m0 + BM - 1, a.S - 1);
            const int im[2] = {img_first, img_last};
            const float ym[2] = {ymax, ymax1};
            pp_amax_commit_wg<NWAVE, 2>(a.y_amax, im, ym, (int)pp_udiv((unsigned)min(m0, (long long)wlast), a.dv_per), (int)pp_udiv(wlast, a.dv_per),
                                        reinterpret_cast<float*>(smem));
        }
        PP_TL_MARK(3);
#ifdef PP_SPLIT_TIMELINE
        asm volatile("s_waitcnt vmcnt(0)" ::: "memory");
        PP_TL_MARK(7);
#endif
        PP_TL_FLUSH();
        return;
    }

    int rimg[4];
    float rmax[4];
#pragma unroll
    for (int pb = 0; pb < 4; ++pb) {
        const long long mt = m0 + wm * 128 + pb * 32 + (lane & 31);
        const bool pok = mt < a.S;
        const long long m = pok ? mt : a.S - 1;
        const int img = (int)pp_udiv((unsigned)m, a.dv_per), rem = (int)((unsigned)m - (unsigned)img * (unsigned)(a.H * a.W));
        float xi = 1.f, ymax = 0.f;
        if constexpr (H) xi = pp_act_unscale(a.x_amax[img]);
        rimg[pb] = img;
        const int oy = (int)pp_udiv((unsigned)rem, a.dv_row), ox = rem - oy * a.W;
        const size_t ypix = ((size_t)img * (a.H + a.y_pad) + oy) * (a.W + a.y_pad) + ox;
        const size_t r1pix = ((size_t)img * (a.r1_H + a.r1_pad) + (oy >> a.r1_shift)) * (a.r1_W + a.r1_pad) + (ox >> a.r1_shift);
        const size_t r2pix = ((size_t)img * (a.H + a.r2_pad) + oy) * (a.W + a.r2_pad) + ox;
#pragma unroll
        for (int cb = 0; cb < 2; ++cb) {
#pragma unroll
            for (int g = 0; g < 4; ++g) {
                const int co = (cb0 + cb) * 32 + 8 * g + 4 * (lane >> 5);
                if (co >= a.Cout || !pok) continue;
                const float4 b4 = *reinterpret_cast<const float4*>(a.bias + co);
                const f32x16 cc = acc[cb][pb];
                float4 v;
                if constexpr (H) {
                    const float4 sc = *reinterpret_cast<const float4*>(a.wscale + co);
                    v = make_float4(__builtin_fmaf(cc[4 * g + 0], sc.x * xi, b4.x), __builtin_fmaf(cc[4 * g + 1], sc.y * xi, b4.y),
                                    __builtin_fmaf(cc[4 * g + 2], sc.z * xi, b4.z), __builtin_fmaf(cc[4 * g + 3], sc.w * xi, b4.w));
                } else {
                    v = make_float4(cc[4 * g + 0] + b4.x, cc[4 * g + 1] + b4.y, cc[4 * g + 2] + b4.z, cc[4 * g + 3] + b4.w);
                }
                if (a.relu == PP_RELU_FIRST) { v.x = fmaxf(v.x, 0.f); v.y = fmaxf(v.y, 0.f); v.z = fmaxf(v.z, 0.f); v.w = fmaxf(v.w, 0.f); }
                else if (a.relu >= PP_ACT_LEAKY) { v.x = split_activate(v.x, a.relu); v.y = split_activate(v.y, a.relu); v.z = split_activate(v.z, a.relu); v.w = split_activate(v.w, a.relu); }
                if (a.res1) {
                    const float4 r = *reinterpret_cast<const float4*>(a.res1 + r1pix * a.Cout + co);
                    v.x += r.x; v.y += r.y; v.z += r.z; v.w += r.w;
                }
                if (a.res2) {
                    const float4 r = *reinterpret_cast<const float4*>(a.res2 + r2pix * a.Cout + co);
                    v.x += r.x; v.y += r.y; v.z += r.z; v.w += r.w;
                }
                if (a.relu == PP_RELU_LAST) { v.x = fmaxf(v.x, 0.f); v.y = fmaxf(v.y, 0.f); v.z = fmaxf(v.z, 0.f); v.w = fmaxf(v.w, 0.f); }
                *reinterpret_cast<float4*>(a.y + ypix * a.Cout + co) = v;
                ymax = fmaxf(ymax, pp_abs4max(v));
            }
        }
        rmax[pb] = ymax;
    }
    if (a.y_amax) {
        const unsigned wlast = (unsigned)min(m0 + BM - 1, a.S - 1);
        pp_amax_commit_wg<NWAVE, 4>(a.y_amax, rimg, rmax, (int)pp_udiv((unsigned)min(m0, (long long)wlast), a.dv_per), (int)pp_udiv(wlast, a.dv_per),
                                    reinterpret_cast<float*>(smem));
    }
}

template <bool H>
__global__ __launch_bounds__(256) void split_weights_kernel(const float* w, uint4* out, int Cin, int taps, int CoutPad, int ncb,
                                                            size_t total, const float* cmax) {
    const size_t i = blockIdx.x * (size_t)256 + threadIdx.x;
    if (i >= total) return;
    const int lane = (int)(i & 63);
    size_t r = i >> 6;
    const int cb = (int)(r % ncb);
    r /= ncb;
    const int t = (int)(r % taps);
    const int c = (int)(r / taps);
    const int cout = cb * 32 + (lane & 31);
    unsigned short h[3][8];
#pragma unroll
    for (int j = 0; j < 8; ++j) {
        const int cin = c * 16 + (lane >> 5) * 8 + j;
        const int k = t * Cin + cin;
        float v = 0.f;
        if (cout < CoutPad) v = w[((size_t)(k >> 5) * CoutPad + cout) * 32 + 8 * (k & 3) + ((k & 31) >> 2)];
        if constexpr (H) {
            split_weight_h(v, channel_scale(cmax[cout]), h[0][j], h[1][j], h[2][j]);
            continue;
        }
        const __bf16 q0 = (__bf16)v;
        const float r1 = v - (float)q0;
        const __bf16 q1 = (__bf16)r1;
        const float r2 = r1 - (float)q1;
        const __bf16 q2 = (__bf16)r2;
        h[0][j] = __builtin_bit_cast(unsigned short, q0);
        h[1][j] = __builtin_bit_cast(unsigned short, q1);
        h[2][j] = __builtin_bit_cast(unsigned short, q2);
    }
    constexpr int WPL = H ? 2 : 3;
    const size_t frag = (i >> 6) * WPL;
#pragma unroll
    for (int pl = 0; pl < WPL; ++pl) {
        uint4 o;
        o.x = h[pl][0] | ((unsigned)h[pl][1] << 16);
        o.y = h[pl][2] | ((unsigned)h[pl][3] << 16);
        o.z = h[pl][4] | ((unsigned)h[pl][5] << 16);
        o.w = h[pl][6] | ((unsigned)h[pl][7] << 16);
        out[(frag + pl) * 64 + lane] = o;
    }
}

void make_magic(unsigned d, unsigned (&dv)[2]) {
    if (d <= 1) { dv[0] = 0; dv[1] = 32; return; }
    unsigned k = 0;
    while ((1ull << k) < d) ++k;
    dv[0] = (unsigned)((((1ull << k) - d) << 32) / d + 1);
    dv[1] = k - 1;
}

int env_int(const char* name, int dflt) {
    const char* v = getenv(name);
    return v ? atoi(v) : dflt;
}

TileGeom pick_tile(int H, int W, int max_np, int pxb) {
    static const int force = env_int("POSEPIPE_SPLIT_TILE", -1);
    TileGeom best{};
    best.eff = -1.0;
    const int cand[4][2] = {{0, 0}, {0, 1}, {1, 0}, {2, 0}};
    const int nblk = 4 * pxb;
    for (int i = 0; i < 4; ++i) {
        if (force >= 0 && i != force) continue;
        TileGeom g{};
        g.bw_log2 = cand[i][0];
        g.gx_log2 = cand[i][1];
        const int BW = 32 >> g.bw_log2, BH = 1 << g.bw_log2, GX = 1 << g.gx_log2, GY = nblk / GX;
        g.TW = GX * BW;
        g.TH = GY * BH;
        g.PWp = g.TW + 2;
        if (g.bw_log2 == 2)
            while (g.PWp % 8 != 4) ++g.PWp;
        g.NP = (g.TH + 2) * g.PWp;
        g.NPp = g.NP;
        while (g.NPp % 8 != 4) ++g.NPp;
        g.tiles_x = (W + g.TW - 1) / g.TW;
        g.tiles_y = (H + g.TH - 1) / g.TH;
        if (g.NP > max_np) continue;
        g.eff = (double)H * W / ((double)g.tiles_x * g.tiles_y * 128.0 * pxb) - 1e-4 * g.NP / 256.0;
        if (g.eff > best.eff) best = g;
    }
    return best;
}

TileGeom pick_tile_s2(int H, int W, int max_np) {
    static const int force = env_int("POSEPIPE_SPLIT_TILE_S2", -1);
    TileGeom best{};
    best.eff = -1.0;
    const int cand[4][2] = {{0, 0}, {1, 0}, {2, 0}, {1, 1}};
    for (int i = 0; i < 4; ++i) {
        if (force >= 0 && i != force) continue;
        TileGeom g{};
        g.bw_log2 = cand[i][0];
        g.gx_log2 = cand[i][1];
        const int BW = 32 >> g.bw_log2, BH = 1 << g.bw_log2, GX = 1 << g.gx_log2, GY = 4 / GX;
        g.TW = GX * BW;
        g.TH = GY * BH;
        g.PWp = g.TW + 1;
        if (g.bw_log2 == 2)
            while (g.PWp % 8 != 4) ++g.PWp;
        g.NP = 4 * (g.TH + 1) * g.PWp;
        g.NPp = g.NP;
        while (g.NPp % 8 != 4) ++g.NPp;
        g.tiles_x = (W + g.TW - 1) / g.TW;
        g.tiles_y = (H + g.TH - 1) / g.TH;
// ... 180 lines not shown
    const int i = blockIdx.x * 256 + threadIdx.x;
    if (i >= STEM_STEPS * 2 * 64) return;
    const int lane = i & 63, cb = (i >> 6) & 1, s = i >> 7;
    const int cout = cb * 32 + (lane & 31);
    unsigned short h[2][8];
#pragma unroll
    for (int j = 0; j < 8; ++j) {
        const int dy = s >> 1, dx = 4 * (s & 1) + 2 * (lane >> 5) + (j >> 2), c = j & 3;
        float v = 0.f;
        if (dx < 7) {
            const int k = (dy * 7 + dx) * 4 + c;
            v = w[((size_t)(k >> 5) * CoutPad + cout) * 32 + 8 * (k & 3) + ((k & 31) >> 2)];
        }
        unsigned short q2;
        split_weight_h(v, channel_scale(cmax[cout]), h[0][j], h[1][j], q2);
    }
#pragma unroll
    for (int pn = 0; pn < 2; ++pn) {
        uint4 o;
        o.x = h[pn][0] | ((unsigned)h[pn][1] << 16);
        o.y = h[pn][2] | ((unsigned)h[pn][3] << 16);
        o.z = h[pn][4] | ((unsigned)h[pn][5] << 16);
        o.w = h[pn][6] | ((unsigned)h[pn][7] << 16);
        out[(size_t)(((s * 2 + cb) * 2 + pn) * 64 + lane)] = o;
    }
}

}


static TileGeom tap_tiling(const ConvArgs& a, int nw, int stream_env) {
    const int max_np = nw == 8 ? 768 : 512, xp_h = a.Hin + a.x_pad, xp_w = a.Win + a.x_pad;
    TileGeom g = pick_tile(a.Hout, a.Wout, max_np, nw / 2);
    g.mode = MODE_TILE;
    const int snp = 64 * nw + 2 + 2 * xp_w;
    const double stream_eff = (double)a.Hout * a.Wout / ((double)xp_h * xp_w);
    bool use_stream = a.x_pad >= 1 && snp <= max_np && (g.eff < 0 || stream_eff > g.eff + 0.02);
    if (stream_env == 0 && g.eff >= 0) use_stream = false;
    if (stream_env == 1 && a.x_pad >= 1 && snp <= max_np) use_stream = true;
    if (use_stream) {
        g.mode = MODE_STREAM;
        g.PWp = xp_w;
        g.NP = g.NPp = snp;
        while (g.NPp % 8 != 4) ++g.NPp;
    }
    return g;
}

SplitPlan pp_conv_split_plan(const ConvArgs& a) {
    static const int stem7_on = env_int("POSEPIPE_SPLIT_STEM7", 1);
    static const int s2_on = env_int("POSEPIPE_SPLIT_S2", 1), s2p_on = env_int("POSEPIPE_SPLIT_S2P", 1);
    static const int gemm8_on = env_int("POSEPIPE_SPLIT_GEMM8", 1), gemm4_min_c = env_int("POSEPIPE_SPLIT_GEMM4_MIN_C", 64);
    static const int gemm_min_cin = env_int("POSEPIPE_SPLIT_GEMM_MIN_CIN", 1024);
    static const int c48_on = env_int("POSEPIPE_SPLIT_C48", 1), c48_mult = env_int("POSEPIPE_SPLIT_C48_MULT", 0);
    static const int stream_env = env_int("POSEPIPE_SPLIT_STREAM", -1);
    const char* s2_env = getenv("POSEPIPE_SPLIT_S2_MIN_CIN");
    SplitPlan p;
    p.f16 = a.split_f16 != 0;
    const size_t wpl = p.f16 ? 2 : 3;
    p.ncb = (a.Cout + 31) / 32;
    p.nout = p.ncb * 32;
    if (stem7_on && p.f16 && a.KH == 7 && a.KW == 7 && a.stride == 2 && a.pad_h == 3 && a.pad_w == 3 && a.dil_h == 1 && a.dil_w == 1 &&
        a.Cin == 4 && a.Cout == 64 && a.CoutPad >= 64 && a.up_log2 == 0 && !a.out_nchw && !a.res1 && !a.res2 &&
        (a.relu == PP_RELU_NONE || a.relu == PP_RELU_FIRST || a.relu == PP_RELU_LAST) && (a.y_stride == 0 || a.y_stride == a.Cout) &&
        a.y_coff == 0 && a.Hout == (a.Hin - 1) / 2 + 1 && a.Wout == (a.Win - 1) / 2 + 1) {
        p.kernel = SPLIT_STEM7;
        p.cin = a.Cin;
        p.frag_bytes = STEM_WBYTES;
        p.bytes = p.frag_bytes + (size_t)2 * p.nout * sizeof(float);
        return p;
    }
    const bool k3 = a.KH == 3 && a.KW == 3 && a.stride == 1 && a.pad_h == 1 && a.pad_w == 1 && a.dil_h == 1 && a.dil_w == 1 &&
                    a.Hout == a.Hin && a.Wout == a.Win;
    const bool k1 = a.KH == 1 && a.KW == 1 && a.pad_h == 0 && a.pad_w == 0;
    const bool full = a.KH == a.Hin && a.KW == a.Win && a.pad_h == 0 && a.pad_w == 0 && a.dil_h == 1 && a.dil_w == 1 &&
                      a.x_pad == 0 && a.Hout == 1 && a.Wout == 1 && !k1;
    const bool s2_pick = s2_env ? a.Cin >= atoi(s2_env) : p.f16 ? (a.Cin >= 96 || (a.Cin >= 48 && p.ncb >= 6)) : (a.Cin >= 128 && (p.ncb & 1) == 0);
    const bool s2_shape = a.KH == 3 && a.KW == 3 && a.stride == 2 && a.pad_h == 1 && a.pad_w == 1 && a.dil_h == 1 && a.dil_w == 1 && !full;
    const bool s2p_map = a.Hout * a.Wout >= 1500 || (a.Hout * a.Wout >= 400 && a.Cout >= 96);
    const bool s2p = s2p_on && p.f16 && s2_shape && s2p_map;
    const bool k3s2 = s2_on && s2_shape && (s2_pick || s2p);
    if (!(k3 || k1 || full || k3s2)) return p;
    p.taps = (k3 || k3s2) ? 9 : 1;
    p.cin = full ? a.K : a.Cin;
    const bool product = gemm8_on && p.taps == 1 && p.cin >= gemm4_min_c && a.Cout % 128 == 0;
    const bool one_column = p.f16 && p.cin >= 256 && a.Cout > 32 && a.Cout <= 64 && a.HWout >= 4096;
    if (p.taps == 1 && p.cin < gemm_min_cin && !one_column && !product) return p;
    const bool res1_plain = !a.res1 || (a.res1_off_w == 0 && a.res1_shift >= 0 && a.res1_shift <= 4 &&
                                        ((a.Hout - 1) >> a.res1_shift) < a.res1_H && ((a.Wout - 1) >> a.res1_shift) < a.res1_W &&
                                        (a.res1_shift > 0 || (a.res1_H == a.Hout && a.res1_W == a.Wout)));
    if (!(p.cin % 16 == 0 && a.Cout % 4 == 0 && a.up_log2 == 0 && !a.out_nchw && res1_plain && a.relu <= PP_ACT_SWISH &&
          (a.y_stride == 0 || a.y_stride == a.Cout) && a.y_coff == 0))
        return p;
    const bool c48 = c48_on && k3 && ((a.Cout > 32 && a.Cout <= 48) || (c48_mult == 1 && a.Cout % 48 == 0) || (c48_mult == 2 && a.Cout == 192));
    size_t steps = (size_t)(p.cin / 16) * p.taps;
    if (product) {
        p.kernel = SPLIT_PRODUCT;
    } else if (!k3 && !s2p) {
        p.kernel = p.taps > 1 ? SPLIT_TAP_GATHER : SPLIT_ONE_TAP;
        p.tile[0].mode = MODE_GEMM;
        p.tile[0].NP = 256;
        p.tile[0].NPp = 260;
    } else if (s2p) {
        p.kernel = SPLIT_S2P;
        p.tile[0] = pick_tile_s2(a.Hout, a.Wout, 13 * 64);
        p.tile[0].mode = MODE_TILE;
    } else if (c48) {
        p.kernel = SPLIT_C48;
        p.ncb = (a.Cout + 47) / 48 * 3;
        p.nout = p.ncb * 16;
        steps = (size_t)(p.cin / 16) * 5;
        p.tile[0] = tap_tiling(a, 4, stream_env);
    } else {
        p.kernel = SPLIT_TAP3;
        p.tile[0] = tap_tiling(a, 4, stream_env);
        p.tile[1] = tap_tiling(a, 8, stream_env);
    }
    p.frag_bytes = (steps + 1) * p.ncb * wpl * 64 * sizeof(uint4);
    p.bytes = p.frag_bytes + (p.f16 ? (size_t)2 * p.nout * sizeof(float) : 0);
    return p;
}

int pp_conv_split_weights(const SplitPlan& p, const ConvArgs& a, void* out, hipStream_t stream) {
    float* cmax = nullptr;
    if (p.f16) {
        float* inv_scale = reinterpret_cast<float*>(static_cast<unsigned char*>(out) + p.frag_bytes);
        cmax = inv_scale + p.nout;
        hipLaunchKernelGGL(weight_channel_max_kernel, dim3((unsigned)p.nout), dim3(64), 0, stream, a.w, a.Kpad / 32, a.CoutPad, p.nout, cmax, inv_scale);
    }
    const char* what = "split_weights";
    if (p.kernel == SPLIT_STEM7) {
        what = "split_weights_stem7";
        hipLaunchKernelGGL(split_weights_stem7_kernel, dim3((STEM_STEPS * 2 * 64 + 255) / 256), dim3(256), 0, stream, a.w, (uint4*)out, a.CoutPad, cmax);
    } else if (p.kernel == SPLIT_C48) {
        what = "split_weights48";
        const size_t total = (size_t)(p.cin / 16) * 5 * p.ncb * 64;
        const dim3 grid((unsigned)((total + 255) / 256));
        if (p.f16) hipLaunchKernelGGL(split_weights48_kernel<true>, grid, dim3(256), 0, stream, a.w, (uint4*)out, p.cin, a.CoutPad, p.ncb, total, cmax);
        else hipLaunchKernelGGL(split_weights48_kernel<false>, grid, dim3(256), 0, stream, a.w, (uint4*)out, p.cin, a.CoutPad, p.ncb, total, cmax);
    } else {
        const size_t total = (size_t)(p.cin / 16) * p.taps * p.ncb * 64;
        const dim3 grid((unsigned)((total + 255) / 256));
        if (p.f16) hipLaunchKernelGGL(split_weights_kernel<true>, grid, dim3(256), 0, stream, a.w, (uint4*)out, p.cin, p.taps, a.CoutPad, p.ncb, total, cmax);
        else hipLaunchKernelGGL(split_weights_kernel<false>, grid, dim3(256), 0, stream, a.w, (uint4*)out, p.cin, p.taps, a.CoutPad, p.ncb, total, cmax);
    }
    hipError_t e = hipGetLastError();
    if (e != hipSuccess) {
        pp_set_error("%s launch failed: %s", what, hipGetErrorString(e));
        return PP_ERR_HIP;
    }
    return PP_OK;
}

__global__ __launch_bounds__(256) void amax_kernel(const float4* x, size_t quads, unsigned per, unsigned* amax) {
    const unsigned n = blockIdx.x / per, part = blockIdx.x - n * per;
    const float4* xs = x + (size_t)n * quads;
    float m = 0.f;
    for (size_t i = (size_t)part * 256 + threadIdx.x; i < quads; i += (size_t)per * 256) m = fmaxf(m, pp_abs4max(xs[i]));
    __shared__ float red[16];
    const int im[1] = {(int)n};
    const float mm[1] = {m};
    pp_amax_commit_wg<4, 1>(amax, im, mm, (int)n, (int)n, red);
}

int pp_launch_amax(const float* x, int n, size_t elems, unsigned* amax, hipStream_t stream) {
    if (n <= 0 || elems == 0) return PP_OK;
    if (elems % 4 != 0) {
        pp_set_error("amax: %zu floats per sample (a multiple of 4 is required)", elems);
        return PP_ERR_ARG;
    }
    const size_t quads = elems / 4;
    const unsigned per = (unsigned)std::min<size_t>(std::max<size_t>((quads + 1023) / 1024, 1), std::max<size_t>(2048 / (size_t)n, 1));
    hipLaunchKernelGGL(amax_kernel, dim3(per * (unsigned)n), dim3(256), 0, stream, (const float4*)x, quads, per, amax);
    hipError_t e = hipGetLastError();
    if (e != hipSuccess) {
        pp_set_error("amax launch failed: %s", hipGetErrorString(e));
        return PP_ERR_HIP;
    }
    return PP_OK;
}

#ifdef PP_SPLIT_TIMELINE
static unsigned long long* tl_buf = nullptr;
static const size_t TL_MAX_WG = 1 << 19;
static unsigned long long* tl_begin(const ConvArgs& a, hipStream_t stream) {
    static const char* path = getenv("POSEPIPE_SPLIT_TIMELINE");
    static const int only_cin = env_int("POSEPIPE_SPLIT_TIMELINE_CIN", 0);
    static const int max_launches = env_int("POSEPIPE_SPLIT_TIMELINE_MAX", 300);
    static int recorded = 0;
    if (!path || (only_cin && a.Cin != only_cin) || recorded >= max_launches) return nullptr;
    ++recorded;
    if (!tl_buf && hipMalloc(&tl_buf, TL_MAX_WG * 128) != hipSuccess) return nullptr;
    (void)hipMemsetAsync(tl_buf, 0, TL_MAX_WG * 128, stream);
    return tl_buf;
}
static void tl_end(const ConvArgs& a, const SplitArgs& s, const char* kernel, unsigned nwg, hipStream_t stream) {
    if (!s.dbg) return;
    (void)hipStreamSynchronize(stream);
    nwg = std::min<unsigned>(nwg, TL_MAX_WG);
    std::vector<unsigned long long> h((size_t)nwg * 16);
    (void)hipMemcpy(h.data(), tl_buf, h.size() * 8, hipMemcpyDeviceToHost);
    static int launch = 0;
    FILE* f = fopen(getenv("POSEPIPE_SPLIT_TIMELINE"), "ab");
    if (!f) return;
    long long hdr[16] = {0x54494d454c494e45ll, launch++, (long long)nwg, a.N, a.Hout, a.Wout, a.Cin, a.Cout, s.mode, s.nchunks, s.gx, s.gy,
                         a.res1 != nullptr, a.res2 != nullptr, 0, 0};
    memcpy(&hdr[14], kernel, std::min<size_t>(strlen(kernel), 15));
    fwrite(hdr, 8, 16, f);
    fwrite(h.data(), 8, h.size(), f);
    fclose(f);
}
#define PP_TL_BEGIN() s.dbg = tl_begin(a, stream)
#define PP_TL_END(name, nwg) tl_end(a, s, name, nwg, stream)
#else
#define PP_TL_BEGIN()
#define PP_TL_END(name, nwg)
#endif

static void fill_divisors(SplitArgs& s) {
    const bool stream_mode = s.mode == MODE_STREAM;
    make_magic(stream_mode ? (unsigned)(s.xp_h * s.PWp) : (unsigned)(s.H * s.W), s.dv_per);
    make_magic(stream_mode ? (unsigned)s.PWp : (unsigned)s.W, s.dv_row);
    make_magic((unsigned)std::max(s.tiles_x, 1), s.dv_tx);
    make_magic((unsigned)std::max(s.tiles_y, 1), s.dv_ty);
    make_magic((unsigned)std::max(s.PWp, 1), s.dv_pw);
    make_magic((unsigned)std::max(s.gy, 1), s.dv_ncol);
    make_magic((unsigned)std::max(s.gx >> 3, 1), s.dv_run0);
    make_magic((unsigned)((s.gx >> 3) + 1), s.dv_run1);
    make_magic((unsigned)std::max(s.ktaps, 1), s.dv_ktaps);
    make_magic((unsigned)std::max(s.KW, 1), s.dv_kw);
}

template <auto K, int MAX_LDS, class Args>
static void launch_split(dim3 grid, unsigned threads, size_t lds, hipStream_t stream, const Args& s) {
    static PpPerDeviceOnce once;
    once.run([] { (void)hipFuncSetAttribute((const void*)K, hipFuncAttributeMaxDynamicSharedMemorySize, MAX_LDS); });
    hipLaunchKernelGGL(K, grid, dim3(threads), lds, stream, s);
}

template <int NS, int... MORE, class F>
static void with_nslot(int nslot, F&& f) {
    if constexpr (sizeof...(MORE) == 0) f(std::integral_constant<int, NS>());
    else if (nslot <= NS) f(std::integral_constant<int, NS>());
    else with_nslot<MORE...>(nslot, f);
}

template <int T, int NW, bool R4, int NS>
static void launch_tap(int cob, bool f16, dim3 grid, size_t lds, hipStream_t stream, const SplitArgs& s) {
    constexpr int L = (NW == 8 ? 160 : 100) * 1024;
    if constexpr (R4) {
        if (cob == 3) return launch_split<conv_split_kernel<9, NS, 3, 2, 4, true, true>, L>(grid, 256, lds, stream, s);
        if (cob == 4) return launch_split<conv_split_kernel<9, NS, 4, 2, 4, true, true>, L>(grid, 256, lds, stream, s);
    }
    if (f16 && cob == 2) launch_split<conv_split_kernel<T, NS, 2, 2, NW, R4, true>, L>(grid, 64 * NW, lds, stream, s);
    else if (f16) launch_split<conv_split_kernel<T, NS, 1, 2, NW, R4, true>, L>(grid, 64 * NW, lds, stream, s);
    else if (cob == 2) launch_split<conv_split_kernel<T, NS, 2, 2, NW, R4, false>, L>(grid, 64 * NW, lds, stream, s);
    else launch_split<conv_split_kernel<T, NS, 1, 2, NW, R4, false>, L>(grid, 64 * NW, lds, stream, s);
}

static unsigned apply_tiling(SplitArgs& s, const TileGeom& g, const ConvArgs& a, int nw) {
    s.mode = g.mode;
    s.NP = g.NP;
    s.NPp = g.NPp;
    if (g.mode == MODE_GEMM) {
        s.S = (long long)a.M;
        return (unsigned)((a.M + 255) / 256);
    }
    s.PWp = g.PWp;
    if (g.mode == MODE_STREAM) {
        s.S = (long long)a.N * s.xp_h * s.xp_w;
        return (unsigned)((s.S + 64 * nw - 1) / (64 * nw));
    }
    s.tiles_x = g.tiles_x; s.tiles_y = g.tiles_y; s.TH = g.TH; s.TW = g.TW; s.bw_log2 = g.bw_log2; s.gx_log2 = g.gx_log2;
    return (unsigned)(g.tiles_x * g.tiles_y * a.N);
}

static int launch_stem7(const ConvArgs& a, hipStream_t stream) {
    if (!a.x_amax) {
        pp_set_error("conv_split: the fp16 form needs the per-sample maximum of its input (ConvArgs::x_amax)");
        return PP_ERR_STATE;
    }
    StemArgs s{};
    s.x = a.x; s.w = (const uint4*)a.wsplit; s.bias = a.bias; s.y = a.y;
    s.wscale = reinterpret_cast<const float*>(static_cast<const unsigned char*>(a.wsplit) + STEM_WBYTES);
    s.x_amax = a.x_amax; s.y_amax = a.y_amax;
    s.N = a.N; s.Hin = a.Hin; s.Win = a.Win; s.xp_h = a.Hin + a.x_pad; s.xp_w = a.Win + a.x_pad;
    s.Hout = a.Hout; s.Wout = a.Wout; s.y_pad = a.y_pad; s.relu = a.relu;
    s.tiles_x = (a.Wout + STEM_TW - 1) / STEM_TW;
    s.tiles_y = (a.Hout + STEM_TH - 1) / STEM_TH;
    s.ntiles = a.N * s.tiles_x * s.tiles_y;
    s.x_bytes = a.x_bytes;
    make_magic((unsigned)s.tiles_x, s.dv_tx);
    make_magic((unsigned)s.tiles_y, s.dv_ty);
    static const int ncu = [] {
        int dev = 0, n = 256;
        if (hipGetDevice(&dev) == hipSuccess) (void)hipDeviceGetAttribute(&n, hipDeviceAttributeMultiprocessorCount, dev);
        return n > 0 ? n : 256;
    }();
    launch_split<conv_split_stem7_kernel, STEM_LDS>(dim3((unsigned)std::min(s.ntiles, ncu)), 512, STEM_LDS, stream, s);
    hipError_t e = hipGetLastError();
    if (e != hipSuccess) {
        pp_set_error("conv_split_stem7 launch failed: %s", hipGetErrorString(e));
        return PP_ERR_HIP;
    }
    return PP_OK;
}

int pp_launch_conv_split(const SplitPlan& p, const ConvArgs& a, hipStream_t stream) {
    if (a.wsplit && p.kernel == SPLIT_STEM7) return launch_stem7(a, stream);
    if (!a.wsplit || p.kernel == SPLIT_NONE) {
        pp_set_error("conv_split: layer not eligible");
        return PP_ERR_ARG;
    }
    static const int colmaj_mb = env_int("POSEPIPE_SPLIT_COLMAJOR_MB", 256), gemm_remap = env_int("POSEPIPE_SPLIT_GEMM_REMAP", 1);
    static const int epi_env = env_int("POSEPIPE_SPLIT_GEMM_EPI", 1);
    static const int cob2_env = env_int("POSEPIPE_SPLIT_S2_COB", 0), cob_env = env_int("POSEPIPE_SPLIT_COB", 0);
    static const int nw8_f16 = env_int("POSEPIPE_SPLIT_NW8_F16", 0);
    static const int nw8_min_blocks = env_int("POSEPIPE_SPLIT_NW8_MIN_BLOCKS", 512), nw8_min_chunks = env_int("POSEPIPE_SPLIT_NW8_MIN_CHUNKS", 16);
    static const int ring4_env = env_int("POSEPIPE_SPLIT_RING4", 1), ring48_env = env_int("POSEPIPE_SPLIT_RING48", 1);
    const bool full = p.cin != a.Cin;
    SplitArgs s{};
    s.x = a.x; s.w = (const uint4*)a.wsplit; s.bias = a.bias; s.res1 = a.res1; s.res2 = a.res2; s.y = a.y;
    s.N = a.N; s.H = a.Hout; s.W = a.Wout; s.Cin = p.cin; s.Cout = a.Cout;
    s.ncb = p.ncb;
    s.xp_h = full ? 1 : a.Hin + a.x_pad;
    s.xp_w = full ? 1 : a.Win + a.x_pad;
    s.stride = a.stride;
    s.y_pad = a.y_pad; s.r1_pad = a.r1_pad; s.r2_pad = a.r2_pad; s.relu = a.relu;
    s.r1_shift = a.res1 ? a.res1_shift : 0;
    s.r1_H = a.res1 ? a.res1_H : a.Hout;
    s.r1_W = a.res1 ? a.res1_W : a.Wout;
    s.nchunks = p.cin / 16;
    s.ktaps = 1; s.KW = a.KW; s.pad = a.pad_h; s.Hin = a.Hin; s.Win = a.Win;
    if (p.kernel == SPLIT_TAP_GATHER) {
        s.ktaps = p.taps;
        s.nchunks = (p.cin / 16) * p.taps;
    }
    s.x_bytes = a.x_bytes;
    s.xcd_remap = a.xcd_remap;
    const bool f16 = p.f16 != 0;
    const int xp = f16 ? 2 : 3;
    const int wpl = f16 ? 2 : 3;
    s.wscale = f16 ? reinterpret_cast<const float*>(static_cast<const unsigned char*>(a.wsplit) + p.frag_bytes) : nullptr;
    s.x_amax = a.x_amax;
    s.y_amax = a.y_amax;
    if (f16 && !a.x_amax) {
        pp_set_error("conv_split: the fp16 form needs the per-sample maximum of its input (ConvArgs::x_amax)");
        return PP_ERR_STATE;
    }
    PP_TL_BEGIN();
    s.col_major = (size_t)a.x_bytes <= (size_t)colmaj_mb << 20;
    const char* tag;
    dim3 grid;
    if (p.kernel == SPLIT_PRODUCT) {
        s.mode = MODE_GEMM;
        s.S = (long long)a.M;
        s.col_major = 0;
        const int BM = 256, BN = 128;
        grid = dim3((unsigned)((a.M + BM - 1) / BM), (unsigned)(a.Cout / BN));
        s.gx = (int)grid.x; s.gy = (int)grid.y;
        s.xcd_remap = gemm_remap && s.gy > 1;
        if (s.xcd_remap) grid = dim3((unsigned)((s.gx + 7) / 8 * 8 * s.gy), 1);
        const int epi_knob = g_split_gemm_epi.load(std::memory_order_relaxed);
        s.epi_lds = epi_knob >= 0 ? epi_knob : epi_env;
        const int nwave = 4;
        fill_divisors(s);
        const size_t lds_loop = f16 ? (size_t)3 * BM * 64 + (size_t)3 * BN * 2 * wpl * 16 : (size_t)2 * (xp * 2 * (BM + 4) * 16 + BN * 2 * wpl * 16);
        const size_t lds = std::max<size_t>(lds_loop, s.epi_lds ? (size_t)nwave * (16384 + 2048) : 0);
        if (f16) launch_split<conv_split_gemm_kernel<2, 2, true>, 80 * 1024>(grid, 256, lds, stream, s);
        else launch_split<conv_split_gemm_kernel<2, 2, false>, 80 * 1024>(grid, 256, lds, stream, s);
        tag = "g256x128";
    } else if (p.kernel == SPLIT_S2P) {
        if (p.tile[0].eff < 0) {
            pp_set_error("conv_split: no strided-patch tile for a %dx%d map", a.Hout, a.Wout);
            return PP_ERR_STATE;
        }
        const unsigned gx = apply_tiling(s, p.tile[0], a, 4);
        s.SP = (s.TH + 1) * s.PWp;
        int cob = 1;
        for (int c : {4, 3, 2})
            if (s.ncb % c == 0 && (size_t)2 * 2 * s.NPp * 16 + (size_t)4 * c * 2 * 1024 <= 80 * 1024 && (cob2_env == 0 || cob2_env == c)) {
                cob = c;
                break;
            }
        grid = dim3(gx, (unsigned)(s.ncb / cob));
        s.gx = (int)grid.x; s.gy = (int)grid.y;
        if (s.xcd_remap) grid = dim3((unsigned)((s.gx + 7) / 8 * 8 * s.gy), 1);
        fill_divisors(s);
        make_magic((unsigned)s.SP, s.dv_row);
        const size_t lds = (size_t)2 * 2 * s.NPp * 16 + (size_t)4 * cob * 2 * 1024;
        with_nslot<10, 11, 13>((s.NP + 63) / 64, [&](auto ns) {
            constexpr int NS = decltype(ns)::value, L = 100 * 1024;
            if (cob == 4) launch_split<conv_split_kernel<9, NS, 4, 1, 4, true, true, true>, L>(grid, 256, lds, stream, s);
            else if (cob == 3) launch_split<conv_split_kernel<9, NS, 3, 1, 4, true, true, true>, L>(grid, 256, lds, stream, s);
            else if (cob == 2) launch_split<conv_split_kernel<9, NS, 2, 1, 4, true, true, true>, L>(grid, 256, lds, stream, s);
            else launch_split<conv_split_kernel<9, NS, 1, 1, 4, true, true, true>, L>(grid, 256, lds, stream, s);
        });
        tag = "s2p";
    } else if (p.kernel == SPLIT_C48) {
        const unsigned gx = apply_tiling(s, p.tile[0], a, 4);
        s.gx = (int)gx;
        s.gy = s.ncb / 3;
        grid = s.xcd_remap ? dim3((unsigned)((s.gx + 7) / 8 * 8 * s.gy), 1) : dim3(gx, (unsigned)s.gy);
        fill_divisors(s);
        const size_t patch48 = (size_t)2 * xp * 2 * s.NPp * 16;
        const bool ring48 = f16 && ring48_env && patch48 + (size_t)4 * 3 * wpl * 1024 <= 80 * 1024;
        const size_t lds = patch48 + (ring48 ? (size_t)4 * 3 * wpl * 1024 : 0);
        with_nslot<5, 6, 7, 8>((s.NP + 63) / 64, [&](auto ns) {
            constexpr int NS = decltype(ns)::value, L = 100 * 1024;
            if (ring48) launch_split<conv_split48_kernel<NS, true, true>, L>(grid, 256, lds, stream, s);
            else if (f16) launch_split<conv_split48_kernel<NS, true, false>, L>(grid, 256, lds, stream, s);
            else launch_split<conv_split48_kernel<NS, false, false>, L>(grid, 256, lds, stream, s);
        });
        tag = "c48";
    } else {
        const bool tap3 = p.kernel == SPLIT_TAP3;
        int cob = (s.ncb & 1) ? 1 : 2;
        if (tap3 && f16 && s.ncb % 3 == 0 && (cob_env == 0 || cob_env == 3)) cob = 3;
        else if (tap3 && f16 && s.ncb % 4 == 0 && (cob_env == 0 || cob_env == 4)) cob = 4;
        int nw = tap3 && (!f16 || nw8_f16) ? 8 : 4;
        unsigned gx = apply_tiling(s, p.tile[nw == 8], a, nw);
        if (nw == 8 && !((long)gx * (s.ncb / cob) >= nw8_min_blocks && s.nchunks >= nw8_min_chunks)) {
            nw = 4;
            gx = apply_tiling(s, p.tile[0], a, nw);
        }
        const int nslot = (s.NP + 16 * nw - 1) / (16 * nw);
        const auto ring_fits = [&](int c) {
            return ring4_env && nw == 4 && s.mode != MODE_GEMM && (size_t)xp * 2 * s.NPp * 16 + (size_t)4 * c * wpl * 1024 <= 80 * 1024;
        };
        if (cob >= 3 && !(ring_fits(cob) && (cob_env >= 3 || (long)gx * (s.ncb / cob) >= 400))) cob = (s.ncb & 1) ? 1 : 2;
        const bool ring = ring_fits(cob);
        grid = dim3(gx, (unsigned)(s.ncb / cob));
        s.gx = (int)grid.x; s.gy = (int)grid.y;
        if (s.xcd_remap) grid = dim3((unsigned)((s.gx + 7) / 8 * 8 * s.gy), 1);
        const size_t lds = (size_t)(ring ? 1 : 2) * xp * 2 * s.NPp * 16 + ((nw == 8 || ring) ? (size_t)4 * cob * wpl * 1024 : 0);
        fill_divisors(s);
        if (s.mode == MODE_GEMM) launch_tap<1, 4, false, 4>(cob, f16, grid, lds, stream, s);
        else if (nw == 8) with_nslot<5, 6>(nslot, [&](auto ns) { launch_tap<9, 8, false, decltype(ns)::value>(cob, f16, grid, lds, stream, s); });
        else if (ring) with_nslot<5, 6, 7, 8>(nslot, [&](auto ns) { launch_tap<9, 4, true, decltype(ns)::value>(cob, f16, grid, lds, stream, s); });
        else with_nslot<5, 6, 7, 8>(nslot, [&](auto ns) { launch_tap<9, 4, false, decltype(ns)::value>(cob, f16, grid, lds, stream, s); });
        tag = s.mode == MODE_GEMM ? "gemm4" : nw == 8 ? "nw8" : ring ? "ring4" : "nw4";
    }
    PP_TL_END(tag, grid.x * grid.y);
    hipError_t e = hipGetLastError();
    if (e != hipSuccess) {
        pp_set_error("conv_split (%s) launch failed: %s", tag, hipGetErrorString(e));
        return PP_ERR_HIP;
    }
    return PP_OK;
}
```

posepipeline_amd/csrc/pp_internal.h:

```cpp
#pragma once
#include <hip/hip_runtime.h>
#include <cstdarg>
#include <cstdio>
#include <cstring>
#include <string>
#include <vector>
#include <mutex>

#include "posepipe_hip.h"

void pp_set_error(const char* fmt, ...);

#define PP_HIP_CHECK(expr)                                                              \
    do {                                                                                \
        hipError_t _e = (expr);                                                         \
        if (_e != hipSuccess) {                                                         \
            pp_set_error("%s failed: %s (%s:%d)", #expr, hipGetErrorString(_e), __FILE__, \
                         __LINE__);                                                     \
            return PP_ERR_HIP;                                                          \
        }                                                                               \
    } while (0)

#define PP_REQUIRE(cond, ...)            \
    do {                                 \
        if (!(cond)) {                   \
            pp_set_error(__VA_ARGS__);   \
            return PP_ERR_ARG;           \
        }                                \
    } while (0)

struct PpPerDeviceOnce {
    std::mutex m;
    unsigned long long done = 0;
    template <class F> void run(F&& f) {
        int dev = 0;
        (void)hipGetDevice(&dev);
        std::lock_guard<std::mutex> g(m);
        if ((done >> (dev & 63)) & 1ull) return;
        f();
        done |= 1ull << (dev & 63);
    }
};

struct pp_ctx {
    int device = 0;
    hipStream_t stream = nullptr;
    bool own_stream = true;
    hipEvent_t ev_start = nullptr, ev_stop = nullptr;
    hipStream_t copy_stream = nullptr;
    hipEvent_t ev_upload = nullptr;
    hipEvent_t ev_consumed = nullptr;
    void* scratch = nullptr;
    size_t scratch_bytes = 0;
    int ensure_scratch(size_t bytes);
};

struct ScratchCursor {
    pp_ctx* ctx;
    size_t off = 0;
    explicit ScratchCursor(pp_ctx* c) : ctx(c) {}
    static size_t align(size_t b) { return (b + 255) & ~size_t(255); }
    template <class T>
    T* take(size_t count) {
        T* p = reinterpret_cast<T*>(static_cast<char*>(ctx->scratch) + off);
        off += align(count * sizeof(T));
        return p;
    }
};

void pp_range_push(const char* name);
void pp_range_pop();
struct PpRange {
    explicit PpRange(const char* name) { pp_range_push(name); }
    ~PpRange() { pp_range_pop(); }
    PpRange(const PpRange&) = delete;
    PpRange& operator=(const PpRange&) = delete;
};
struct PpStages {
    bool open = false;
    void next(const char* name) {
        if (open) pp_range_pop();
        open = name != nullptr;
        if (open) pp_range_push(name);
    }
    ~PpStages() { next(nullptr); }
};

struct ConvArgs {
    const float* x;
    const float* w;
    const float* bias;
    const float* res1;
    const float* res2;
    float* y;
    int N, Hin, Win, Cin, Hout, Wout, Cout, CoutPad;
    int KH, KW, stride, pad_h, pad_w, dil_h, dil_w;
    int K, Kpad, M, HWout;
    unsigned div_hw_m, div_hw_s1, div_hw_s2, div_w_m, div_w_s1, div_w_s2;
    unsigned div_c_m, div_c_s1, div_c_s2, div_kw_m, div_kw_s1, div_kw_s2;
    int xcd_remap;
    unsigned x_bytes;
    int relu, up_log2, out_nchw;
    int res1_shift, res1_off_w, res1_H, res1_W;
    int y_stride, y_coff;
    const uint2* tap_table;
    int x_pad, y_pad, r1_pad, r2_pad;
    int no_bounds;
    const void* wsplit;
    int numerics;
    int split_f16;
    const unsigned* x_amax;
    unsigned* y_amax;
};
struct TileGeom {
    int TH, TW, bw_log2, gx_log2, PWp, NP, NPp, tiles_x, tiles_y;
    double eff;
    int mode;
};
enum SplitKernel {
    SPLIT_NONE = 0,
    SPLIT_STEM7,
    SPLIT_PRODUCT,
    SPLIT_C48,
    SPLIT_TAP3,
    SPLIT_S2P,
    SPLIT_ONE_TAP,
    SPLIT_TAP_GATHER,
};
struct SplitPlan {
    int kernel = SPLIT_NONE;
    int f16 = 0;
    int taps = 1, cin = 0;
    int ncb = 0;
    int nout = 0;
    size_t frag_bytes = 0;
    size_t bytes = 0;
    TileGeom tile[2] = {};
    long long off = -1;
};
SplitPlan pp_conv_split_plan(const ConvArgs& a);
int pp_conv_split_weights(const SplitPlan& p, const ConvArgs& a, void* out, hipStream_t stream);
int pp_launch_conv_split(const SplitPlan& p, const ConvArgs& a, hipStream_t stream);
bool pp_conv_tracks_amax(const ConvArgs& a, bool split);
bool pp_conv_split_enabled();
bool pp_conv_split_f16_default();
int pp_conv_prepare(const ConvArgs& a);
int pp_conv_out_dim(int in, int k, int stride, int pad, int dil);
int pp_launch_conv(const ConvArgs& a, const SplitPlan* plan, hipStream_t stream);
int pp_launch_conv_p3(const ConvArgs& a, int ct, int pt, hipStream_t stream, bool fake_addresses = false);

struct PoolArgs {
    const float* x;
    float* y;
    int N, Hin, Win, C, Hout, Wout, KH, KW, stride, pad_h, pad_w;
    int x_stride, x_coff, y_stride, y_coff;
};
int pp_launch_maxpool(const PoolArgs& a, hipStream_t stream);
int pp_launch_avgpool(const float* x, float* y, int n, int hin, int win, int c, int kh, int kw, int stride, hipStream_t stream);

struct GemmArgs {
    const void* A;
    const void* B;
    const float* bias;
    const float* res;
    void* C;
    int M, N, K;
    int act;
    int out_bf16;
    int res_mod;
    int group_m;
    int qkv_tokens, qkv_hd;
};
int pp_launch_gemm_bf16(const GemmArgs& a, hipStream_t stream);
int pp_gemm_bf16_prepare();
struct pp_deconv_bf16;
int pp_deconv_bf16_create(const float* weights, const float* bias, int h, int w, int cin, int cout, int max_batch,
                          hipStream_t stream, pp_deconv_bf16** out);
void pp_deconv_bf16_destroy(pp_deconv_bf16* d);
int pp_deconv_bf16_run(pp_deconv_bf16* d, const float* x, float* out, int batch, int relu, hipStream_t stream);
int pp_launch_f32_to_bf16(const float* x, void* y, size_t n, hipStream_t stream);
int pp_launch_nv12_to_bgr(const unsigned char* nv12, unsigned char* bgr, int frames, int h, int w, hipStream_t stream);
int pp_launch_layernorm(const float* x, const float* pos, int pos_mod, float* x_out, const float* gamma,
                        const float* beta, int rows, int dim, float eps, void* y, int out_bf16, hipStream_t stream);
int pp_launch_attention(const void* qkv, int batch, int tokens, int heads, int head_dim, void* out, hipStream_t stream,
                        int head_major = 0);
int pp_launch_depth_to_space(const float* x, float* y, int n, int h, int w, int c, hipStream_t stream);
int pp_launch_upsample_add(const float* t, const float* res1, const float* res2, float* y, int n, int H, int W, int c,
                           int up_log2, int relu, hipStream_t stream, const float* t2 = nullptr, int up2 = 0,
                           const float* t3 = nullptr, int up3 = 0, unsigned* y_amax = nullptr);
struct pp_vit_encoder;
size_t pp_vit_param_floats(int tokens, int dim, int depth, int hidden);
int pp_vit_encoder_create(const float* params, int tokens, int dim, int depth, int heads, int hidden, int max_batch,
                          hipStream_t stream, pp_vit_encoder** out);
void pp_vit_encoder_destroy(pp_vit_encoder* e);
int pp_vit_encoder_run(pp_vit_encoder* e, const float* in, float* out, int batch, hipStream_t stream);
void pp_vit_encoder_set_timing(pp_vit_encoder* e, int enable);
int pp_vit_encoder_get_timing(pp_vit_encoder* e, float ms3[3], int* n_gemm);

struct PersonXform {
    double a00, a01, b0, a10, a11, b1;
    int frame;
    int valid;
};
bool pp_person_transform(const double* bbox_tlwh, int out_w, int out_h, float center_scale[4], PersonXform* t, int udp = 0);
int pp_enqueue_crop(hipStream_t s, const uint8_t* frames, int h, int w, const PersonXform* xf, int n_person,
                    int out_w, int out_h, const float* lut, const int32_t chan_map[3], int flip, float* out,
                    uint8_t* crop_u8);
int pp_enqueue_flip_w(hipStream_t s, const float* src, float* dst, int n, int h, int w);

struct DecodeParams {
    int n, k, h, w;
    int shift_heatmap, post, blur_kernel;
};
int pp_enqueue_decode(hipStream_t s, const DecodeParams& p, const float* hm, const float* hm_flip,
                      const int32_t* flip_perm, const float* center_scale, float* kpts, float* merged);
```

posepipeline_amd/program.py:

```python
from __future__ import annotations

import ctypes as C
from dataclasses import dataclass, field

import numpy as np

from . import _lib as L


def fold_bn(weight, conv_bias, gamma, beta, mean, var, eps=1e-5):
    scale = gamma.astype(np.float64) / np.sqrt(var.astype(np.float64) + eps)
    w = weight.astype(np.float64) * scale.reshape((-1,) + (1,) * (weight.ndim - 1))
    b0 = np.zeros_like(scale) if conv_bias is None else conv_bias.astype(np.float64)
    b = beta.astype(np.float64) + (b0 - mean.astype(np.float64)) * scale
    return w.astype(np.float32), b.astype(np.float32)


def pack_conv(weight, bias, cin_pad=None):
    w = np.asarray(weight, dtype=np.float32)
    if w.ndim == 3:
        w = w[:, :, None, :]
    cout, cin, kh, kw = w.shape
    cin_p = cin_pad if cin_pad is not None else (cin + 3) // 4 * 4
    assert cin_p % 4 == 0 and cin_p >= cin
# ... 71 lines not shown
        h, w, cin_buf = self.dims(x)
        wt = np.asarray(weight)
        if wt.ndim == 3:
            wt = wt[:, :, None, :]
        cout, cin, kh, kw = wt.shape
        assert cin <= cin_buf and cin_buf % 4 == 0, (cin, cin_buf)
        W, b = pack_conv(wt, bias, cin_pad=cin_buf)
        ho = (h + pad_end[0] + 2 * pad[0] - dil[0] * (kh - 1) - 1) // stride + 1 - front_only[0]
        wo = (w + pad_end[1] + 2 * pad[1] - dil[1] * (kw - 1) - 1) // stride + 1 - front_only[1]
        if out is None:
            assert out_c_off == 0
            out = self.buf(ho << up_log2, wo << up_log2, cout)
        else:
            oh, ow, oc = self.dims(out)
            assert (oh, ow) == (ho << up_log2, wo << up_log2) and out_c_off + cout <= oc and out_c_off % 4 == 0, \
                (self.dims(out), ho, wo, cout, out_c_off)
        w_off = self._add_blob(W)
        b_off = self._add_blob(b)
        self.vops.append(dict(type=L.PP_OP_CONV, in_=x, out=out, res1=res1, res2=res2, cin=cin_buf, cout=cout, kh=kh,
                              kw=kw, stride=stride, pad_h=pad[0], pad_w=pad[1], dil_h=dil[0], dil_w=dil[1], relu=relu,
                              up_log2=up_log2, out_nchw=int(out_nchw), res1_shift=res1_shift, res1_off_w=res1_off_w,
                              out_c_off=out_c_off, in_c_off=0,
                              pad_end=pad_end[0] | (pad_end[1] << 1) | (front_only[0] << 2) | (front_only[1] << 3),
                              w_off=w_off, b_off=b_off, name=name,
                              flops=2.0 * ho * wo * cout * cin * kh * kw))
        return out

    def maxpool(self, x, k, stride, pad, name="maxpool", out=None, out_c_off=0, in_c_off=0, c=None) -> int:
        h, w, cx = self.dims(x)
        c = cx if c is None else c
        assert in_c_off + c <= cx and c % 4 == 0 and in_c_off % 4 == 0
        ho = (h + 2 * pad - (k - 1) - 1) // stride + 1
        wo = (w + 2 * pad - (k - 1) - 1) // stride + 1
        if out is None:
            assert out_c_off == 0
            out = self.buf(ho, wo, c)
        else:
            oh, ow, oc = self.dims(out)
            assert (oh, ow) == (ho, wo) and out_c_off + c <= oc and out_c_off % 4 == 0
        self.vops.append(dict(type=L.PP_OP_MAXPOOL, in_=x, out=out, res1=-1, res2=-1, cin=c, cout=c, kh=k, kw=k,
                              stride=stride, pad_h=pad, pad_w=pad, dil_h=1, dil_w=1, relu=0, up_log2=0, out_nchw=0,
                              res1_shift=0, res1_off_w=0, out_c_off=out_c_off, in_c_off=in_c_off, pad_end=0,
                              w_off=0, b_off=0, name=name, flops=0.0))
        return out

    def avgpool(self, x, kh, kw, stride=1, name="avgpool") -> int:
        h, w, c = self.dims(x)
        out = self.buf((h - kh) // stride + 1, (w - kw) // stride + 1, c)
        return self._plain_op(L.PP_OP_AVGPOOL, x, out, cin=c, cout=c, kh=kh, kw=kw, stride=stride, name=name)

    def _plain_op(self, type_, x, out, *, cin, cout, kh=1, kw=1, stride=1, w_off=0, name="op", flops=0.0):
        self.vops.append(dict(type=type_, in_=x, out=out, res1=-1, res2=-1, cin=cin, cout=cout, kh=kh, kw=kw, stride=stride,
                              pad_h=0, pad_w=0, dil_h=1, dil_w=1, relu=0, up_log2=0, out_nchw=0, res1_shift=0,
                              res1_off_w=0, out_c_off=0, in_c_off=0, pad_end=0, w_off=w_off, b_off=0, name=name,
                              flops=flops))
        return out

    def vit_encoder(self, x, params, *, depth, heads, mlp_ratio, name="vit_encoder") -> int:
        h, w, dim = self.dims(x)
        t, hid = h * w, dim * mlp_ratio
        per_block = 2 * dim + 3 * dim * dim + 3 * dim + dim * dim + dim + 2 * dim + hid * dim + hid + dim * hid + dim
        params = np.asarray(params, dtype=np.float32).reshape(-1)
        assert params.size == t * dim + per_block * depth + 2 * dim, (params.size, t, dim, depth)
        out = self.buf(h, w, dim)
        macs = depth * (t * (4 * dim * dim + 2 * dim * hid) + 2 * t * t * dim)
        return self._plain_op(L.PP_OP_VIT_ENCODER, x, out, cin=dim, cout=dim, kh=depth, kw=heads, stride=mlp_ratio,
                              w_off=self._add_blob(params), name=name, flops=2.0 * macs)

    def upsample_add(self, t, *, up_log2, res1=-1, res2=-1, relu=L.PP_RELU_NONE, name="upsample_add", more=()) -> int:
        h, w, c = self.dims(t)
        out = self.buf(h << up_log2, w << up_log2, c)
        more = list(more)
        assert len(more) <= 2
        for tb, ub in more:
            assert self.dims(tb) == ((h << up_log2) >> ub, (w << up_log2) >> ub, c), (self.dims(tb), self.dims(out), ub)
        (in2, up2), (in3, up3) = (more + [(-1, 0), (-1, 0)])[:2]
        self.vops.append(dict(type=L.PP_OP_UPSAMPLE_ADD, in_=t, out=out, res1=res1, res2=res2, cin=c, cout=c, kh=1, kw=1,
                              stride=1, pad_h=0, pad_w=0, dil_h=1, dil_w=1, relu=relu, up_log2=up_log2, out_nchw=0,
                              res1_shift=0, res1_off_w=0, out_c_off=0, in_c_off=0, pad_end=0, w_off=0, b_off=0, name=name,
                              in2=in2, in3=in3, up2_log2=up2, up3_log2=up3, flops=0.0))
        return out

    def deconv4x4s2_bf16(self, x, weight, bias, *, relu=L.PP_RELU_NONE, name="deconv_bf16") -> int:
        h, w, cin_buf = self.dims(x)
        wt = np.asarray(weight, dtype=np.float32)
        cin, cout = wt.shape[:2]
        assert wt.shape[2:] == (4, 4) and cin == cin_buf and cin % 64 == 0 and cout % 8 == 0, (wt.shape, cin_buf)
        blocks = np.empty((2, 2, 2, 2, cout, cin), np.float32)
        for a in (0, 1):
            for b in (0, 1):
                for r in (0, 1):
                    for s in (0, 1):
                        blocks[a, b, r, s] = wt[:, :, 3 - a - 2 * r, 3 - b - 2 * s].T
        bb = np.zeros(cout, np.float32) if bias is None else np.asarray(bias, np.float32)
        out = self.buf(2 * h, 2 * w, cout)
        w_off = self._add_blob(blocks)
        b_off = self._add_blob(bb)
        self.vops.append(dict(type=L.PP_OP_DECONV_BF16, in_=x, out=out, res1=-1, res2=-1, cin=cin, cout=cout, kh=4, kw=4,
                              stride=2, pad_h=1, pad_w=1, dil_h=1, dil_w=1, relu=relu, up_log2=0, out_nchw=0, res1_shift=0,
                              res1_off_w=0, out_c_off=0, in_c_off=0, pad_end=0, w_off=w_off, b_off=b_off, name=name,
                              flops=2.0 * h * w * cin * cout * 16))
        return out

    def depth_to_space(self, x, name="depth_to_space") -> int:
        h, w, c4 = self.dims(x)
        assert c4 % 16 == 0
        out = self.buf(2 * h, 2 * w, c4 // 4)
        return self._plain_op(L.PP_OP_DEPTH_TO_SPACE, x, out, cin=c4, cout=c4 // 4, name=name)

    def deconv4x4s2(self, x, weight, bias, *, relu=L.PP_RELU_NONE, name="deconv") -> int:
        h, w, cin_buf = self.dims(x)
        wt = np.asarray(weight, dtype=np.float32)
        cin, cout = wt.shape[:2]
        assert wt.shape[2:] == (4, 4) and cout % 4 == 0
        wide = self.buf(h, w, 4 * cout)
        taps = {0: (3, 1), 1: (2, 0)}
        for a in (0, 1):
            for b in (0, 1):
                sub = wt[:, :, list(taps[a]), :][:, :, :, list(taps[b])]
                self.conv(x, np.transpose(sub, (1, 0, 2, 3)), bias, pad=(1 - a, 1 - b), pad_end=(a, b),
                          front_only=(1 - a, 1 - b), relu=relu, out=wide, out_c_off=(2 * a + b) * cout,
                          name=f"{name}.p{a}{b}")
        return self.depth_to_space(wide, name=name + ".d2s")

    def _halo_plan(self):
        import os
        n_v = len(self.vbufs)
        pad = [0] * n_v
        if os.environ.get("POSEPIPE_CONV_HALO", "1") == "0":
            return pad
        ok = [not b.pinned and b.c % 4 == 0 for b in self.vbufs]
        need = [0] * n_v
        for op in self.vops:
            conv = op["type"] == L.PP_OP_CONV
            for k in ("in_", "out", "res1", "res2", "in2", "in3"):
                v = op.get(k, -1)
                if v >= 0 and not conv:
                    ok[v] = False
            if not conv:
                continue
            o = op["out"]
            if op["out_nchw"] or op["out_c_off"] or self.vbufs[o].c != op["cout"]:
                ok[o] = False
            h, w, _ = self.dims(op["in_"])
            eh, ew = op["pad_end"] & 1, (op["pad_end"] >> 1) & 1
            ho = (h + eh + 2 * op["pad_h"] - op["dil_h"] * (op["kh"] - 1) - 1) // op["stride"] + 1 - ((op["pad_end"] >> 2) & 1)
            wo = (w + ew + 2 * op["pad_w"] - op["dil_w"] * (op["kw"] - 1) - 1) // op["stride"] + 1 - ((op["pad_end"] >> 3) & 1)
            over = max(op["pad_h"], op["pad_w"], (ho - 1) * op["stride"] - op["pad_h"] + (op["kh"] - 1) * op["dil_h"] - (h - 1),
                       (wo - 1) * op["stride"] - op["pad_w"] + (op["kw"] - 1) * op["dil_w"] - (w - 1))
            if over > 0:
                need[op["in_"]] = max(need[op["in_"]], over)
        return [need[v] if ok[v] and 0 < need[v] <= 2 else 0 for v in range(n_v)]

    def build(self) -> Program:
        n_v = len(self.vbufs)
        last_use = [-1] * n_v
        first_def = [None] * n_v
        for i, op in enumerate(self.vops):
            for key in ("in_", "res1", "res2", "in2", "in3", "out"):
                v = op.get(key, -1)
                if v >= 0:
                    last_use[v] = i
            if first_def[op["out"]] is None:
                first_def[op["out"]] = i
        vpad = self._halo_plan()
        phys_dims: list[tuple] = []
        phys_pad: list[int] = []
        free: dict[tuple, list[int]] = {}
        v2p = [-1] * n_v
        for v, b in enumerate(self.vbufs):
            if b.pinned:
                phys_dims.append((b.h, b.w, b.c))
                phys_pad.append(0)
                v2p[v] = len(phys_dims) - 1
        for i, op in enumerate(self.vops):
            v = op["out"]
            if v2p[v] < 0:
                key = self.dims(v) + (vpad[v],)
                pool = free.get(key, [])
                busy = {v2p[op[k]] for k in ("in_", "res1", "res2", "in2", "in3") if op.get(k, -1) >= 0}
                pick = next((p for p in pool if p not in busy), None)
                if pick is not None:
                    pool.remove(pick)
                    v2p[v] = pick
                else:
                    phys_dims.append(key[:3])
                    phys_pad.append(vpad[v])
                    v2p[v] = len(phys_dims) - 1
            for key in ("in_", "res1", "res2", "in2", "in3", "out"):
                u = op.get(key, -1)
                if u >= 0 and last_use[u] == i and not self.vbufs[u].pinned and v2p[u] >= 0:
                    lst = free.setdefault(self.dims(u) + (vpad[u],), [])
                    if v2p[u] not in lst:
                        lst.append(v2p[u])
        ops = []
        for op in self.vops:
            rec = L.pp_op()
            for k, val in op.items():
                if k in ("name", "flops"):
                    continue
                if k in ("in_", "out", "res1", "res2", "in2", "in3"):
                    val = v2p[val] if val >= 0 else -1
                setattr(rec, k, int(val))
            ops.append(rec)
        blob = np.concatenate(self.blob_parts) if self.blob_parts else np.zeros(4, np.float32)
        named = {k: v2p[v] for k, v in self.named.items()}
        return Program(ops=ops, bufs=phys_dims, buf_pad=phys_pad, blob=blob, named=named,
                       flops=float(sum(op["flops"] for op in self.vops)),
                       op_flops=[op["flops"] for op in self.vops], op_names=[op["name"] for op in self.vops])


class Net:

    def __init__(self, ctx: L.Context, prog: Program, max_batch: int, blob_dev=None, numerics=None):
        self.ctx = ctx
        self.prog = prog
        self.max_batch = int(max_batch)
        lib = ctx.lib
        n_ops = len(prog.ops)
        ops = (L.pp_op * n_ops)(*prog.ops)
        pads = prog.buf_pad or [0] * len(prog.bufs)
        bufs = (L.pp_buf * len(prog.bufs))(*[L.pp_buf(*d, p) for d, p in zip(prog.bufs, pads)])
        h = C.c_void_p()
        if blob_dev is not None:
            dptr, n_floats = blob_dev
            L.check(lib.pp_net_create_ex(ctx.handle, ops, n_ops, bufs, len(prog.bufs), C.c_void_p(int(dptr)), int(n_floats),
                                         L.PP_MEM_DEVICE, self.max_batch, L.NUMERICS[numerics], C.byref(h)), "pp_net_create_ex")
        else:
            blob = np.ascontiguousarray(prog.blob, dtype=np.float32)
            L.check(lib.pp_net_create_ex(ctx.handle, ops, n_ops, bufs, len(prog.bufs), L.ptr(blob), blob.size, L.PP_MEM_HOST,
                                         self.max_batch, L.NUMERICS[numerics], C.byref(h)), "pp_net_create_ex")
        self.handle = h
        self.numerics = "split" if lib.pp_net_numerics(h) == L.PP_NET_NUMERICS_SPLIT else "exact"
        self.split_kind = {L.PP_NET_NUMERICS_SPLIT_BF16: "split_bf16", L.PP_NET_NUMERICS_SPLIT_F16: "split_f16"}.get(lib.pp_net_split_kind(h), "exact")

    def close(self):
        if getattr(self, "handle", None):
            if getattr(self.ctx, "handle", None):
                self.ctx.lib.pp_net_destroy(self.handle)
            self.handle = None

    def __del__(self):
        try:
            self.close()
        except Exception:
            pass

    def buffer(self, name_or_id):
        pid = self.prog.named[name_or_id] if isinstance(name_or_id, str) else int(name_or_id)
        p = C.c_void_p()
        nb = C.c_size_t()
        L.check(self.ctx.lib.pp_net_buffer(self.handle, pid, C.byref(p), C.byref(nb)), "pp_net_buffer")
        return int(p.value), int(nb.value), self.prog.bufs[pid]

    def run(self, batch, first=0, last=None):
        last = len(self.prog.ops) if last is None else last
        L.check(self.ctx.lib.pp_net_run(self.handle, batch, first, last), "pp_net_run")

    def set_lanes(self, enable: bool):
        L.check(self.ctx.lib.pp_net_set_lanes(self.handle, int(bool(enable))), "pp_net_set_lanes")

    def set_lane_count(self, n_lanes: int):
        L.check(self.ctx.lib.pp_net_set_lane_count(self.handle, int(n_lanes)), "pp_net_set_lane_count")

    def capture(self, batch):
        L.check(self.ctx.lib.pp_net_capture(self.handle, batch), "pp_net_capture")

    def forward(self, x: np.ndarray, in_name="input", out_name="output") -> np.ndarray:
        x = np.ascontiguousarray(x, dtype=np.float32)
        n = x.shape[0]
        pin, pout = self.prog.named[in_name], self.prog.named[out_name]
        assert tuple(x.shape[1:]) == tuple(self.prog.bufs[pin]), (x.shape, self.prog.bufs[pin])
        oh, ow, oc = self.prog.bufs[pout]
        out = np.empty((n, oh, ow, oc), dtype=np.float32)
        L.check(self.ctx.lib.pp_net_forward(self.handle, n, pin, L.ptr(x), pout, L.ptr(out), L.PP_MEM_HOST),
                "pp_net_forward")
        return out

    def read(self, name_or_id, batch) -> np.ndarray:
        dptr, nb, (h, w, c) = self.buffer(name_or_id)
        out = np.empty((batch, h, w, c), dtype=np.float32)
        self.ctx.d2h(out, dptr)
        return out

    def conv_kinds(self) -> np.ndarray:
        kinds = np.zeros(len(self.prog.ops), dtype=np.int32)
        L.check(self.ctx.lib.pp_net_conv_kinds(self.handle, L.ptr(kinds)), "pp_net_conv_kinds")
        return kinds

    def profile(self, batch) -> np.ndarray:
        ms = np.zeros(len(self.prog.ops), dtype=np.float32)
        L.check(self.ctx.lib.pp_net_profile(self.handle, batch, L.ptr(ms)), "pp_net_profile")
        return ms
```

Baseline: 607.5.

## Fold 1x1 shortcut conv into residual-consuming 1x1 conv as second K segment

Detects a bias-only 1x1 projection conv whose output is read only as the residual of a later 1x1 conv. It concatenates the two weight sets into one split-fp16 GEMM with two K segments, so the shortcut is accumulated in the same kernel. The accumulators are rescaled between segments to reconcile the two activation scales. This removes one conv launch plus the write and read of the shortcut tensor. In exchange it keeps the shortcut's input alive longer, adds scheduling dependencies, and carries some precision risk from the scale clamp and rescale.

```diff
diff --git a/posepipeline_amd/csrc/api_core.hip b/posepipeline_amd/csrc/api_core.hip
--- a/posepipeline_amd/csrc/api_core.hip
+++ b/posepipeline_amd/csrc/api_core.hip
@@ -259,6 +259,8 @@
     size_t n_weights = 0;
     unsigned char* wsplit = nullptr;
     std::vector<SplitPlan> split_plan;
+    std::vector<int> fold_into, fold_from;
+    std::vector<SplitPlan> fold_plan;
     int numerics = PP_NET_NUMERICS_EXACT;
     int split_f16 = 0;
     unsigned* amax = nullptr;
@@ -288,6 +290,56 @@
 
 static ConvArgs net_conv_args(pp_net* net, const pp_op& op, int batch);
 static int net_make_lanes(pp_net* net, int n_lanes);
+
+static void net_plan_folds(pp_net* net, size_t& bytes) {
+    const int n = (int)net->ops.size();
+    net->fold_into.assign(n, -1);
+    net->fold_from.assign(n, -1);
+    net->fold_plan.assign(n, SplitPlan());
+    const char* env = getenv("POSEPIPE_SPLIT_FOLD_SHORTCUT");
+    if (net->numerics != PP_NET_NUMERICS_SPLIT || !net->split_f16 || (env && atoi(env) == 0)) return;
+    for (int ia = 0; ia < n; ++ia) {
+        const pp_op& A = net->ops[ia];
+        if (A.type != PP_OP_CONV || A.kh != 1 || A.kw != 1 || A.pad_h != 0 || A.pad_w != 0 || A.pad_end != 0 || A.relu != PP_RELU_NONE ||
+            A.res1 >= 0 || A.res2 >= 0 || A.up_log2 != 0 || A.out_nchw || A.out_c_off != 0 || net->bufs[A.out].c != A.cout || A.cin % 16 != 0 ||
+            A.in == A.out || net->split_plan[ia].kernel == SPLIT_NONE)
+            continue;
+        int ib = -1;
+        bool ok = true;
+        for (int j = ia + 1; j < n && ok; ++j) {
+            const pp_op& o = net->ops[j];
+            const bool reads = o.in == A.out || o.res2 == A.out || o.in2 == A.out || o.in3 == A.out;
+            if (reads || (o.res1 == A.out && ib >= 0)) ok = false;
+            else if (o.res1 == A.out) ib = j;
+            if (o.out == A.out) {
+                if (j == ib) ok = false;
+                break;
+            }
+        }
+        if (!ok || ib < 0) continue;
+        const pp_op& B = net->ops[ib];
+        if (B.type != PP_OP_CONV || B.kh != 1 || B.kw != 1 || B.res1_shift != 0 || B.res1_off_w != 0 || net->fold_from[ib] >= 0 ||
+            net->bufs[B.out].h != net->bufs[A.out].h || net->bufs[B.out].w != net->bufs[A.out].w || B.cout != A.cout)
+            continue;
+        for (int j = ia + 1; j <= ib && ok; ++j) ok = net->ops[j].out != A.in;
+        if (!ok) continue;
+        const ConvArgs a = net_conv_args(net, A, 1), b = net_conv_args(net, B, 1);
+        SplitPlan p = pp_conv_split_fold_plan(net->split_plan[ib], b, net->split_plan[ia], a);
+        if (p.kernel == SPLIT_NONE) continue;
+        p.off = (long long)bytes;
+        bytes += (p.bytes + 255) / 256 * 256;
+        net->fold_plan[ib] = p;
+        net->fold_from[ib] = ia;
+        net->fold_into[ia] = ib;
+    }
+}
+
+static int net_fold_role(const pp_net* net, int i, int first, int last) {
+    if (net->fold_into.empty()) return 0;
+    if (net->fold_into[i] >= 0 && net->fold_into[i] < last) return 1;
+    if (net->fold_from[i] >= 0 && net->fold_from[i] >= first) return 2;
+    return 0;
+}
 
 static void net_plan_amax(pp_net* net) {
     const int n = (int)net->ops.size(), nb = (int)net->bufs.size();
@@ -407,7 +459,8 @@
         auto add = [&](int d) {
             if (d >= 0 && std::find(deps.begin(), deps.end(), d) == deps.end()) deps.push_back(d);
         };
-        for (int b : {op.in, op.res1, op.res2, op.in2, op.in3})
+        const int fin = !net->fold_from.empty() && net->fold_from[i] >= 0 ? net->ops[net->fold_from[i]].in : -1;
+        for (int b : {op.in, op.res1, op.res2, op.in2, op.in3, fin})
             if (b >= 0) add(last_writer[b]);
         add(last_writer[op.out]);
         for (int r : readers[op.out]) add(r);
@@ -429,7 +482,7 @@
                 net->op_needs_event[d] = 1;
             }
         lane_tail[lane] = i;
-        for (int b : {op.in, op.res1, op.res2, op.in2, op.in3})
+        for (int b : {op.in, op.res1, op.res2, op.in2, op.in3, fin})
             if (b >= 0 && b != op.out) readers[b].push_back(i);
         last_writer[op.out] = i;
         readers[op.out].clear();
@@ -567,9 +620,26 @@
 
 static int net_launch_op_body(pp_net* net, const pp_op& op, int batch, hipStream_t s);
 
-static int net_launch_op(pp_net* net, const pp_op& op, int batch, hipStream_t s) {
+static int net_launch_fused(pp_net* net, int ib, int batch, hipStream_t s) {
+    const pp_op& A = net->ops[net->fold_from[ib]];
+    const SplitPlan& p = net->fold_plan[ib];
+    ConvArgs a = net_conv_args(net, net->ops[ib], batch);
+    const pp_buf& bx = net->bufs[A.in];
+    a.res1 = nullptr;
+    a.res1_H = a.res1_W = 0;
+    a.r1_pad = 0;
+    a.x2 = net->buf_ptr(A.in);
+    a.x2_amax = net->amax_slot(net->op_x_slot[net->fold_from[ib]]);
+    a.x2_Hin = bx.h; a.x2_Win = bx.w; a.x2_Cin = A.cin; a.x2_pad = bx.pad; a.x2_stride = A.stride;
+    a.wsplit = net->wsplit + p.off;
+    a.bias = reinterpret_cast<const float*>(net->wsplit + p.off + p.frag_bytes) + 2 * (size_t)p.nout;
+    return pp_launch_conv(a, &p, s);
+}
+
+static int net_launch_op(pp_net* net, const pp_op& op, int batch, hipStream_t s, int role = 0) {
     const size_t idx = &op - net->ops.data();
-    int rc = net_launch_op_body(net, op, batch, s);
+    if (role == 1) return PP_OK;
+    int rc = role == 2 ? net_launch_fused(net, (int)idx, batch, s) : net_launch_op_body(net, op, batch, s);
     if (rc == PP_OK && net->amax && net->op_post_slot[idx] >= 0)
         rc = pp_launch_amax(net->buf_ptr(op.out), batch, net->buf_elems[op.out], net->amax_slot(net->op_post_slot[idx]), s);
     return rc;
@@ -722,7 +792,13 @@
             bytes += (p.bytes + 255) / 256 * 256;
             net->split_plan[i] = p;
         }
+        net_plan_folds(net.get(), bytes);
         net_plan_amax(net.get());
+        for (int i = 0; i < n_ops; ++i)
+            if (net->fold_from[i] >= 0 && net->op_x_slot[net->fold_from[i]] < 0) {
+                net->fold_into[net->fold_from[i]] = -1;
+                net->fold_from[i] = -1;
+            }
         if (!net->slot_owner.empty()) {
             const size_t ab = net->slot_owner.size() * (size_t)max_batch * sizeof(unsigned);
             PP_HIP_CHECK(hipMalloc((void**)&net->amax, ab));
@@ -734,6 +810,14 @@
                 const SplitPlan& p = net->split_plan[i];
                 if (p.kernel == SPLIT_NONE) continue;
                 int rc = pp_conv_split_weights(p, net_conv_args(net.get(), net->ops[i], 1), net->wsplit + p.off, ctx->stream);
+                if (rc != PP_OK) return rc;
+            }
+            for (int i = 0; i < n_ops; ++i) {
+                const int ia = net->fold_from[i];
+                if (ia < 0) continue;
+                const SplitPlan &p = net->fold_plan[i], &pb = net->split_plan[i], &pa = net->split_plan[ia];
+                int rc = pp_conv_split_fold_weights(p, pb, net_conv_args(net.get(), net->ops[i], 1), net->wsplit + pb.off, pa,
+                                                    net_conv_args(net.get(), net->ops[ia], 1), net->wsplit + pa.off, net->wsplit + p.off, ctx->stream);
                 if (rc != PP_OK) return rc;
             }
         }
@@ -848,7 +932,7 @@
     }
     if (net->lanes.empty() || !net->use_lanes || last_op - first_op < 8) {
         for (int i = first_op; i < last_op; ++i) {
-            int rc = net_launch_op(net, net->ops[i], batch, main);
+            int rc = net_launch_op(net, net->ops[i], batch, main, net_fold_role(net, i, first_op, last_op));
             if (rc != PP_OK) return rc;
         }
         return PP_OK;
@@ -859,7 +943,7 @@
         hipStream_t s = net->lanes[net->op_lane[i]];
         for (int d : net->op_waits[i])
             if (d >= first_op) PP_HIP_CHECK(hipStreamWaitEvent(s, net->op_done[d], 0));
-        int rc = net_launch_op(net, net->ops[i], batch, s);
+        int rc = net_launch_op(net, net->ops[i], batch, s, net_fold_role(net, i, first_op, last_op));
         if (rc != PP_OK) return rc;
         if (net->op_needs_event[i]) PP_HIP_CHECK(hipEventRecord(net->op_done[i], s));
     }
@@ -916,7 +1000,8 @@
     hipGraph_t graph = nullptr;
     PP_HIP_CHECK(hipStreamBeginCapture(s, hipStreamCaptureModeThreadLocal));
     int rc = net_reset_amax(net, 0, (int)net->ops.size(), batch, s);
-    for (size_t i = 0; i < net->ops.size() && rc == PP_OK; ++i) rc = net_launch_op(net, net->ops[i], batch, s);
+    for (size_t i = 0; i < net->ops.size() && rc == PP_OK; ++i)
+        rc = net_launch_op(net, net->ops[i], batch, s, net_fold_role(net, (int)i, 0, (int)net->ops.size()));
     hipError_t e = hipStreamEndCapture(s, &graph);
     if (rc != PP_OK) {
         if (graph) (void)hipGraphDestroy(graph);
@@ -957,7 +1042,7 @@
     int rc = net_reset_amax(net, 0, (int)n, batch, s);
     PP_HIP_CHECK(hipEventRecord(ev[0], s));
     for (size_t i = 0; i < n && rc == PP_OK; ++i) {
-        rc = net_launch_op(net, net->ops[i], batch, s);
+        rc = net_launch_op(net, net->ops[i], batch, s, net_fold_role(net, (int)i, 0, (int)n));
         if (rc == PP_OK && hipEventRecord(ev[i + 1], s) != hipSuccess) rc = PP_ERR_HIP;
     }
     if (rc == PP_OK && hipStreamSynchronize(s) != hipSuccess) rc = PP_ERR_HIP;
diff --git a/posepipeline_amd/csrc/conv_igemm.hip b/posepipeline_amd/csrc/conv_igemm.hip
--- a/posepipeline_amd/csrc/conv_igemm.hip
+++ b/posepipeline_amd/csrc/conv_igemm.hip
@@ -642,8 +642,13 @@
         pp_set_error("conv: one input image of %zu bytes exceeds the 4 GiB buffer range", img_bytes);
         return PP_ERR_ARG;
     }
-    if ((size_t)a.N * img_bytes > max_bytes) {
-        const int per = (int)(max_bytes / img_bytes);
+    const size_t x2_img_bytes = a.x2 ? (size_t)(a.x2_Hin + a.x2_pad) * (a.x2_Win + a.x2_pad) * a.x2_Cin * sizeof(float) : 0;
+    if (x2_img_bytes > max_bytes) {
+        pp_set_error("conv: one image of the folded shortcut's input (%zu bytes) exceeds the 4 GiB buffer range", x2_img_bytes);
+        return PP_ERR_ARG;
+    }
+    if ((size_t)a.N * std::max(img_bytes, x2_img_bytes) > max_bytes) {
+        const int per = (int)(max_bytes / std::max(img_bytes, x2_img_bytes));
         const size_t y_img = (size_t)((a.Hout << a.up_log2) + a.y_pad) * ((a.Wout << a.up_log2) + a.y_pad) * (a.y_stride ? a.y_stride : a.Cout);
         const size_t r1_img = (size_t)(a.res1_H + a.r1_pad) * (a.res1_W + a.r1_pad) * a.Cout;
         const size_t r2_img = (size_t)((a.Hout << a.up_log2) + a.r2_pad) * ((a.Wout << a.up_log2) + a.r2_pad) * a.Cout;
@@ -656,6 +661,8 @@
             if (a.res1) p.res1 = a.res1 + (size_t)n0 * r1_img;
             if (a.res2) p.res2 = a.res2 + (size_t)n0 * r2_img;
             if (a.x_amax) p.x_amax = a.x_amax + n0;
+            if (a.x2) p.x2 = a.x2 + (size_t)n0 * (x2_img_bytes / sizeof(float));
+            if (a.x2_amax) p.x2_amax = a.x2_amax + n0;
             if (a.y_amax) p.y_amax = a.y_amax + n0;
             const int rc = pp_launch_conv(p, plan, stream);
             if (rc != PP_OK) return rc;
diff --git a/posepipeline_amd/csrc/conv_split.hip b/posepipeline_amd/csrc/conv_split.hip
--- a/posepipeline_amd/csrc/conv_split.hip
+++ b/posepipeline_amd/csrc/conv_split.hip
@@ -54,6 +54,9 @@
     const float* wscale;
     const unsigned* x_amax;
     unsigned* y_amax;
+    const float* x2;
+    const unsigned* x2_amax;
+    int nchunks1, x2p_h, x2p_w, Cin2, stride2;
 #ifdef PP_SPLIT_TIMELINE
     unsigned long long* dbg;
 #endif
@@ -1193,8 +1196,9 @@
     }
 }
 
-template <int WM, int WN, bool H = false>
+template <int WM, int WN, bool H = false, bool F = false>
 __global__ __launch_bounds__(64 * WM * WN, 512 / (64 * WM * WN)) void conv_split_gemm_kernel(SplitArgs a) {
+    static_assert(H || !F, "two K segments: the fp16 form only");
     constexpr int XP = H ? 2 : 3;
     constexpr int WPL = H ? 2 : 3;
     constexpr int NT = 64 * WM * WN, NWAVE = WM * WN;
@@ -1228,6 +1232,7 @@
     const unsigned lds_base0 = (unsigned)(size_t)(__attribute__((address_space(3))) unsigned char*)smem;
     const size_t wstep0 = (size_t)a.ncb * (WPL * 64);
     f32x16 acc[2][4];
+    float xfin[F ? 4 : 1];
     if constexpr (H) {
     constexpr int XR = 3, XSTG = BM * 64, WR = 3, WBYTES = WU * 16;
     constexpr int NXD = BM / 16 / NWAVE;
@@ -1252,6 +1257,33 @@
             xsc[pb] = pp_act_scale(a.x_amax[pp_udiv(mp, a.dv_per)]);
         }
     }
+    unsigned gx2[F ? NXD : 1];
+    float xsc2[F ? 4 : 1];
+    if constexpr (F) {
+#pragma unroll
+        for (int i = 0; i < NXD; ++i) {
+            const int pl = (wave + NWAVE * i) * 16 + (lane >> 2);
+            const unsigned m = (unsigned)min(m0 + pl, a.S - 1);
+            const int img = (int)pp_udiv(m, a.dv_per), rem = (int)(m - (unsigned)img * (unsigned)(a.H * a.W));
+            const int ho = (int)pp_udiv((unsigned)rem, a.dv_row), wo = rem - ho * a.W;
+            gx2[i] = (unsigned)(((img * a.x2p_h + ho * a.stride2) * a.x2p_w + wo * a.stride2) * a.Cin2) * 4u + (unsigned)(((lane & 3) ^ ((pl >> 1) & 3)) * 16);
+        }
+        const unsigned am2 = a.x2_amax[img_first];
+#pragma unroll
+        for (int pb = 0; pb < 4; ++pb) xsc2[pb] = pp_act_scale(am2);
+        if (img_first != img_last) {
+#pragma unroll
+            for (int pb = 0; pb < 4; ++pb) {
+                const unsigned mp = (unsigned)min(m0 + wm * 128 + pb * 32 + (lane & 31), a.S - 1);
+                xsc2[pb] = pp_act_scale(a.x2_amax[pp_udiv(mp, a.dv_per)]);
+            }
+        }
+#pragma unroll
+        for (int pb = 0; pb < 4; ++pb) {
+            const unsigned f1 = __float_as_uint(xsc[pb]) >> 23, f2 = __float_as_uint(xsc2[pb]) >> 23;
+            xsc2[pb] = __uint_as_float(min(f2, f1 + 40u) << 23);
+        }
+    }
     asm volatile("s_waitcnt vmcnt(0)" ::: "memory");
     const unsigned wlane16 = (unsigned)lane * 16u;
     auto issue = [&](int c) {
@@ -1262,11 +1294,13 @@
             const unsigned dst = __builtin_amdgcn_readfirstlane(lds_base0 + (unsigned)(XR * XSTG + (c % WR) * WBYTES + slab * 1024));
             asm volatile("s_mov_b32 m0, %2\n\ts_nop 0\n\tglobal_load_lds_dwordx4 %0, %1" ::"v"(wlane16 + (unsigned)(slab * 1024)), "s"(wsrc), "s"(dst) : "memory", "m0");
         }
-        const float* xsrc = a.x + (size_t)c * 16;
+        const bool seg2 = F && c >= a.nchunks1;
+        const float* xsrc = seg2 ? a.x2 + (size_t)(c - a.nchunks1) * 16 : a.x + (size_t)c * 16;
 #pragma unroll
         for (int i = 0; i < NXD; ++i) {
             const unsigned dst = __builtin_amdgcn_readfirstlane(lds_base0 + (unsigned)((c % XR) * XSTG + (wave + NWAVE * i) * 1024));
-            asm volatile("s_mov_b32 m0, %2\n\ts_nop 0\n\tglobal_load_lds_dwordx4 %0, %1" ::"v"(gx[i]), "s"(xsrc), "s"(dst) : "memory", "m0");
+            const unsigned go = seg2 ? gx2[F ? i : 0] : gx[i];
+            asm volatile("s_mov_b32 m0, %2\n\ts_nop 0\n\tglobal_load_lds_dwordx4 %0, %1" ::"v"(go), "s"(xsrc), "s"(dst) : "memory", "m0");
         }
     };
     const int fofs = (wm * 128 + (lane & 31)) * 64 + ((((lane >> 5) * 2) ^ ((lane >> 1) & 3)) * 16);
@@ -1301,6 +1335,20 @@
         const unsigned char* sxp = smem + (c % XR) * XSTG;
         const unsigned char* sw = smem + (c % WR) * WBYTES;
         uint4 wf[2][WPL], xh[2][2];
+        if constexpr (F) {
+            if (c == a.nchunks1) {
+#pragma unroll
+                for (int pb = 0; pb < 4; ++pb) {
+                    const int rf = 127 + (int)(__float_as_uint(xsc2[pb]) >> 23) - (int)(__float_as_uint(xsc[pb]) >> 23);
+                    const float ratio = rf > 0 ? __uint_as_float((unsigned)rf << 23) : 0.f;
+#pragma unroll
+                    for (int cb = 0; cb < 2; ++cb)
+#pragma unroll
+                        for (int i = 0; i < 16; ++i) acc[cb][pb][i] *= ratio;
+                    xsc[pb] = xsc2[pb];
+                }
+            }
+        }
 #pragma unroll
         for (int cb = 0; cb < 2; ++cb)
 #pragma unroll
@@ -1323,6 +1371,10 @@
         if (c + 2 < a.nchunks) asm volatile("s_waitcnt vmcnt(%0) lgkmcnt(0)" ::"n"(NXD + NWD) : "memory");
         else asm volatile("s_waitcnt vmcnt(0) lgkmcnt(0)" ::: "memory");
         __builtin_amdgcn_s_barrier();
+    }
+    if constexpr (F) {
+#pragma unroll
+        for (int pb = 0; pb < 4; ++pb) xfin[pb] = __uint_as_float((254u - (__float_as_uint(xsc[pb]) >> 23)) << 23);
     }
     } else {
     unsigned goff[XS];
@@ -1474,7 +1526,10 @@
         }
         const int rdrow = lane >> 3, rdpos = lane & 7, rdchunk = rdpos ^ rdrow;
         float xinv[H ? 4 : 1];
-        if constexpr (H) {
+        if constexpr (F) {
+#pragma unroll
+            for (int pb = 0; pb < 4; ++pb) xinv[pb] = xfin[pb];
+        } else if constexpr (H) {
 #pragma unroll
             for (int pb = 0; pb < 4; ++pb) xinv[pb] = pp_act_unscale(oam_first);
             if (img_first != img_last) {
@@ -1577,7 +1632,8 @@
         const long long m = pok ? mt : a.S - 1;
         const int img = (int)pp_udiv((unsigned)m, a.dv_per), rem = (int)((unsigned)m - (unsigned)img * (unsigned)(a.H * a.W));
         float xi = 1.f, ymax = 0.f;
-        if constexpr (H) xi = pp_act_unscale(a.x_amax[img]);
+        if constexpr (F) xi = xfin[pb];
+        else if constexpr (H) xi = pp_act_unscale(a.x_amax[img]);
         rimg[pb] = img;
         const int oy = (int)pp_udiv((unsigned)rem, a.dv_row), ox = rem - oy * a.W;
         const size_t ypix = ((size_t)img * (a.H + a.y_pad) + oy) * (a.W + a.y_pad) + ox;
@@ -2064,6 +2120,53 @@
     return PP_OK;
 }
 
+SplitPlan pp_conv_split_fold_plan(const SplitPlan& pb, const ConvArgs& b, const SplitPlan& pa, const ConvArgs& a) {
+    SplitPlan p;
+    if (!pb.f16 || !pa.f16 || pb.kernel != SPLIT_PRODUCT || pa.kernel == SPLIT_NONE || pb.taps != 1 || pb.cin != b.Cin) return p;
+    if (!(a.KH == 1 && a.KW == 1 && a.pad_h == 0 && a.pad_w == 0 && a.Cin % 16 == 0 && a.Cout == b.Cout && a.Hout == b.Hout && a.Wout == b.Wout &&
+          pa.nout == pb.nout && (b.relu == PP_RELU_NONE || b.relu == PP_RELU_LAST)))
+        return p;
+    p = pb;
+    p.off = -1;
+    p.cin2 = a.Cin;
+    const size_t steps = (size_t)(p.cin + p.cin2) / 16;
+    p.frag_bytes = (steps + 1) * p.ncb * 2 * 64 * sizeof(uint4);
+    p.bytes = p.frag_bytes + (size_t)3 * p.nout * sizeof(float);
+    return p;
+}
+
+__global__ __launch_bounds__(256) void fold_scale_bias_kernel(const float* cmax_b, const float* cmax_a, const float* bias_b, const float* bias_a,
+                                                              int nout, int cout, float* inv_scale, float* cmax, float* bias) {
+    const int i = blockIdx.x * 256 + threadIdx.x;
+    if (i >= nout) return;
+    const float m = fmaxf(cmax_b[i], cmax_a[i]);
+    cmax[i] = m;
+    inv_scale[i] = 1.f / channel_scale(m);
+    bias[i] = i < cout ? bias_b[i] + bias_a[i] : 0.f;
+}
+
+int pp_conv_split_fold_weights(const SplitPlan& p, const SplitPlan& pb, const ConvArgs& b, const void* wsplit_b, const SplitPlan& pa,
+                               const ConvArgs& a, const void* wsplit_a, void* out, hipStream_t stream) {
+    float* inv_scale = reinterpret_cast<float*>(static_cast<unsigned char*>(out) + p.frag_bytes);
+    float* cmax = inv_scale + p.nout;
+    float* bias = cmax + p.nout;
+    const float* cmax_b = reinterpret_cast<const float*>(static_cast<const unsigned char*>(wsplit_b) + pb.frag_bytes) + pb.nout;
+    const float* cmax_a = reinterpret_cast<const float*>(static_cast<const unsigned char*>(wsplit_a) + pa.frag_bytes) + pa.nout;
+    hipLaunchKernelGGL(fold_scale_bias_kernel, dim3((unsigned)((p.nout + 255) / 256)), dim3(256), 0, stream, cmax_b, cmax_a, b.bias, a.bias, p.nout,
+                       b.Cout, inv_scale, cmax, bias);
+    const size_t t1 = (size_t)(p.cin / 16) * p.ncb * 64, t2 = (size_t)(p.cin2 / 16) * p.ncb * 64;
+    hipLaunchKernelGGL(split_weights_kernel<true>, dim3((unsigned)((t1 + 255) / 256)), dim3(256), 0, stream, b.w, (uint4*)out, p.cin, 1, b.CoutPad,
+                       p.ncb, t1, cmax);
+    hipLaunchKernelGGL(split_weights_kernel<true>, dim3((unsigned)((t2 + 255) / 256)), dim3(256), 0, stream, a.w, (uint4*)out + t1 * 2, p.cin2, 1,
+                       a.CoutPad, p.ncb, t2, cmax);
+    hipError_t e = hipGetLastError();
+    if (e != hipSuccess) {
+        pp_set_error("split_weights (folded shortcut) launch failed: %s", hipGetErrorString(e));
+        return PP_ERR_HIP;
+    }
+    return PP_OK;
+}
+
 __global__ __launch_bounds__(256) void amax_kernel(const float4* x, size_t quads, unsigned per, unsigned* amax) {
     const unsigned n = blockIdx.x / per, part = blockIdx.x - n * per;
     const float4* xs = x + (size_t)n * quads;
@@ -2279,7 +2382,17 @@
         fill_divisors(s);
         const size_t lds_loop = f16 ? (size_t)3 * BM * 64 + (size_t)3 * BN * 2 * wpl * 16 : (size_t)2 * (xp * 2 * (BM + 4) * 16 + BN * 2 * wpl * 16);
         const size_t lds = std::max<size_t>(lds_loop, s.epi_lds ? (size_t)nwave * (16384 + 2048) : 0);
-        if (f16) launch_split<conv_split_gemm_kernel<2, 2, true>, 80 * 1024>(grid, 256, lds, stream, s);
+        if (p.cin2 > 0) {
+            if (!f16 || !a.x2 || !a.x2_amax || a.res1 || a.x2_Cin != p.cin2 || p.cin2 % 16 != 0) {
+                pp_set_error("conv_split: a folded shortcut needs the fp16 form, its second input with maxima and no res1");
+                return PP_ERR_STATE;
+            }
+            s.x2 = a.x2; s.x2_amax = a.x2_amax;
+            s.x2p_h = a.x2_Hin + a.x2_pad; s.x2p_w = a.x2_Win + a.x2_pad; s.Cin2 = a.x2_Cin; s.stride2 = a.x2_stride;
+            s.nchunks1 = p.cin / 16;
+            s.nchunks = (p.cin + p.cin2) / 16;
+            launch_split<conv_split_gemm_kernel<2, 2, true, true>, 80 * 1024>(grid, 256, lds, stream, s);
+        } else if (f16) launch_split<conv_split_gemm_kernel<2, 2, true>, 80 * 1024>(grid, 256, lds, stream, s);
         else launch_split<conv_split_gemm_kernel<2, 2, false>, 80 * 1024>(grid, 256, lds, stream, s);
         tag = "g256x128";
     } else if (p.kernel == SPLIT_S2P) {
diff --git a/posepipeline_amd/csrc/pp_internal.h b/posepipeline_amd/csrc/pp_internal.h
--- a/posepipeline_amd/csrc/pp_internal.h
+++ b/posepipeline_amd/csrc/pp_internal.h
@@ -111,6 +111,9 @@
     int split_f16;
     const unsigned* x_amax;
     unsigned* y_amax;
+    const float* x2;
+    const unsigned* x2_amax;
+    int x2_Hin, x2_Win, x2_Cin, x2_pad, x2_stride;
 };
 struct TileGeom {
     int TH, TW, bw_log2, gx_log2, PWp, NP, NPp, tiles_x, tiles_y;
@@ -131,6 +134,7 @@
     int kernel = SPLIT_NONE;
     int f16 = 0;
     int taps = 1, cin = 0;
+    int cin2 = 0;
     int ncb = 0;
     int nout = 0;
     size_t frag_bytes = 0;
@@ -141,6 +145,9 @@
 SplitPlan pp_conv_split_plan(const ConvArgs& a);
 int pp_conv_split_weights(const SplitPlan& p, const ConvArgs& a, void* out, hipStream_t stream);
 int pp_launch_conv_split(const SplitPlan& p, const ConvArgs& a, hipStream_t stream);
+SplitPlan pp_conv_split_fold_plan(const SplitPlan& pb, const ConvArgs& b, const SplitPlan& pa, const ConvArgs& a);
+int pp_conv_split_fold_weights(const SplitPlan& p, const SplitPlan& pb, const ConvArgs& b, const void* wsplit_b, const SplitPlan& pa,
+                               const ConvArgs& a, const void* wsplit_a, void* out, hipStream_t stream);
 bool pp_conv_tracks_amax(const ConvArgs& a, bool split);
 bool pp_conv_split_enabled();
 bool pp_conv_split_f16_default();
diff --git a/posepipeline_amd/program.py b/posepipeline_amd/program.py
--- a/posepipeline_amd/program.py
+++ b/posepipeline_amd/program.py
@@ -247,6 +247,26 @@
                 need[op["in_"]] = max(need[op["in_"]], over)
         return [need[v] if ok[v] and 0 < need[v] <= 2 else 0 for v in range(n_v)]
 
+    def folded_shortcuts(self):
+        pairs = []
+        for ia, A in enumerate(self.vops):
+            if not (A["type"] == L.PP_OP_CONV and A["kh"] == 1 and A["kw"] == 1 and A["pad_h"] == 0 and A["pad_w"] == 0
+                    and A["pad_end"] == 0 and A["relu"] == L.PP_RELU_NONE and A["res1"] < 0 and A["res2"] < 0 and A["up_log2"] == 0
+                    and not A["out_nchw"] and A["out_c_off"] == 0 and self.vbufs[A["out"]].c == A["cout"] and A["cin"] % 16 == 0):
+                continue
+            o = A["out"]
+            uses = [(j, k) for j, op in enumerate(self.vops) for k in ("in_", "res1", "res2", "in2", "in3", "out")
+                    if j != ia and op.get(k, -1) == o]
+            if len(uses) != 1 or uses[0][1] != "res1" or uses[0][0] < ia or self.vbufs[o].pinned:
+                continue
+            ib = uses[0][0]
+            B = self.vops[ib]
+            if (B["type"] == L.PP_OP_CONV and B["kh"] == 1 and B["kw"] == 1 and B["res1_shift"] == 0 and B["res1_off_w"] == 0
+                    and B["cout"] == A["cout"] and self.dims(B["out"])[:2] == self.dims(o)[:2]
+                    and all(self.vops[j]["out"] != A["in_"] for j in range(ia + 1, ib + 1))):
+                pairs.append((ia, ib))
+        return pairs
+
     def build(self) -> Program:
         n_v = len(self.vbufs)
         last_use = [-1] * n_v
@@ -258,6 +278,9 @@
                     last_use[v] = i
             if first_def[op["out"]] is None:
                 first_def[op["out"]] = i
+        for ia, ib in self.folded_shortcuts():
+            x = self.vops[ia]["in_"]
+            last_use[x] = max(last_use[x], ib)
         vpad = self._halo_plan()
         phys_dims: list[tuple] = []
         phys_pad: list[int] = []
```

Result: no change. 604.8 (-0.4%).
